# johnomotani/SharedMemSparseLU.jl

Hardware: AMD Instinct MI355X
Metric: nnz(L+U)/s + achieved HBM GB/s, 3D Poisson 128³ numeric LU, 1/2/4/8 GPU (higher is better)
Workload: dtype f64

## Files before the change

sharedmemsparselu.jl_amd/csrc/device.hpp:

```cpp
#pragma once
#include <cstdint>

namespace smlu {

struct SNode {
  int64_t first;
  int64_t Loff, Uoff, Foff;
  int64_t rowptr;
  int64_t voff;
  int32_t ns, nu;
  int32_t parent, nb;
  int32_t mode;
  int32_t chbeg, chend;
  int32_t level;
  int32_t cpair;
};

struct GemmTask {
  const double* A;
  const double* B;
  double* C;
  int32_t m, n, k;
  int32_t lda, ldb, ldc;
  int32_t tiles_m;
  int32_t gsid = -1;
  int64_t tile0;
};

constexpr int kUrowsCols = 32;
struct URowTask {
  int32_t s;
  int32_t ob0, ob1;
  int32_t slot0;
  int32_t ld;
  int32_t ncols;
  int64_t coff;
};

struct FrontTile {
  int32_t s;
  int32_t pad;
  int64_t wg0;
};

struct XContrib {
  int32_t child, pad;
  int64_t src;
};

struct alignas(8) AEnt {
  int32_t x, y;
};

struct SegDesc {
  uint64_t src, dst;
  int64_t n4;
};

struct XCol {
  int32_t p, tj;
  int64_t off;
  int32_t cnt, acnt;
  int64_t aoff;
};

struct SwapTask {
  int32_t s, kb0, nsub, slot0;
  int32_t a, b, c_lo, c_hi;
  int64_t wg0;
};

struct Rhs {
  int32_t n;
  int64_t ldx, ldv;
};
constexpr int kMultiRhs = 16;
#ifndef SMLU_SWEEP_WK
#define SMLU_SWEEP_WK 4
#endif
constexpr int kSweepWK = SMLU_SWEEP_WK;
constexpr int kSweepXB = 64;
struct ChunkDesc {
  int64_t c0, s, r0, nr, tri, rect;
};

}
```

sharedmemsparselu.jl_amd/csrc/factor.cpp:

```cpp
#include "handle.hpp"

static hipError_t run_launch(smlu_handle* h, const Launch& L, double diag_tol, double piv_tol, hipStream_t st) {
  switch (L.kind) {
    case K_EXTADD:
      return launch_assemble(st, L.cnt, h->xcols.p + L.off, h->xtasks.p, h->aents.p, h->sn.p, h->relmap.p,
                             h->A.p, h->Arow.p, h->Rs.p, h->store.p, h->scratch.p);
    case K_FRONT_LDS:
      return launch_front_small(st, (int)L.cnt, (int)L.aux, h->ilist.p + L.off, h->sn.p, h->chlist.p,
                                h->relmap.p, h->aents.p, h->A.p, h->Arow.p, h->Rs.p, h->store.p, h->scratch.p,
                                h->rowperm.p, h->info.p, h->growth.p, diag_tol, piv_tol);
    case K_STEPTRSM:
      return launch_step_trsm(st, (int)L.aux, h->ftiles.p + L.off, (int)L.cnt, L.nwg, h->ftiles.p + L.off2,
                              (int)L.cnt2, L.nwg2, L.step, h->sch.ob, h->sn.p, h->store.p, h->scratch.p, h->info.p,
                              h->growth.p, piv_tol);
    case K_LASWP:
      return launch_laswp(st, L.nwg, h->stasks.p + L.off, (int)L.cnt, h->sn.p, h->store.p, h->scratch.p,
                          h->swaps.p, kSwapStride);
    case K_PANEL:
      return launch_panel1(st, (int)L.cnt, (int)L.aux, (int)L.nwg, (int)L.aux2, L.step,
                           h->ilist.p + L.off, h->sn.p,
                          h->store.p, h->scratch.p, h->rowperm.p, h->swaps.p, kSwapStride, h->info.p,
                          h->growth.p, diag_tol, (int)L.cnt2, h->tinv.p, (int)h->sch.ob);
    case K_TRSMU:
      return launch_trsm_u(st, L.nwg, h->ftiles.p + L.off, (int)L.cnt, h->sch.ob, (int)L.aux, h->sn.p,
                           h->store.p, h->scratch.p, h->swaps.p, kSwapStride);
    case K_GEMM:
    case K_GEMMU:
    case K_GEMMO:
    case K_GEMM22:
      return launch_gemm(st, L.nwg, h->gtasks.p + L.off, (int)L.cnt, (int)L.aux, 0);
    case K_TRSML:
      return launch_gemm_g(st, L.nwg, h->gtasks.p + L.off, (int)L.cnt, (int)L.aux, 0, h->info.p,
                           h->growth.p, piv_tol);
    case K_UROWS:
      return launch_urows(st, (int)L.cnt, h->urtasks.p + L.off, h->sn.p, h->store.p, h->tinv.p);
    case K_TRIINV:
      return launch_tri_inv(st, (int)L.cnt, L.step, h->ilist.p + L.off, h->sn.p, h->store.p, h->scratch.p,
                            h->tinv.p);
  }
  return hipErrorInvalidValue;
}

static int enqueue_factor(smlu_handle* h, Timer& tm, bool dbg, int seg) {
  Plan& P = h->plan;
  hipStream_t st = h->stream;
  const size_t lo = h->sch.fac_seg[seg];
  const size_t hi = (size_t)seg + 1 < h->sch.fac_seg.size() ? h->sch.fac_seg[seg + 1] : h->sch.fac.size();
  double diag_tol = P.given_order ? 0.0 : h->opts.diag_pivot_tol;
  double piv_tol = h->opts.pivot_tol;
  if (seg > 0) goto launches;
  HIPCHK(launch_factor_reset(st, h->sch.nnodes, h->info.p, h->growth.p, P.n, h->rowperm.p, h->rowperm0.p));
  if (!h->given_Rs) {
    if (h->opts.scale) HIPCHK(launch_rowscale(st, P.n, h->Arowptr.p, h->Arow_ent.p, h->A.p, h->Rs.p));
    else HIPCHK(launch_fill(st, P.n, h->Rs.p, 1.0));
  }
launches:
  auto group = [&](size_t i) { return h->sch.fac[i].kind == K_FRONT_LDS ? h->sch.fac[i].aux2 : 0; };
  int gi = 0;
  hipEvent_t gstop = nullptr;
  for (size_t li = lo; li < hi; ++li) {
    const Launch& L = h->sch.fac[li];
    const int64_t g = group(li);
    const bool cont = g > 0 && li > lo && group(li - 1) == g;
    const bool more = g > 0 && li + 1 < hi && group(li + 1) == g;
    gi = cont ? gi + 1 : 0;
    const bool grouped = cont || more;
    if (gi == 0 && more) {
      HIPCHK(tm.begin(L.kind, &gstop, st));
      HIPCHK(hipEventRecord(h->fork_ev, st));
    }
    if (gi == 1) HIPCHK(hipStreamWaitEvent(h->side, h->fork_ev, 0));
    hipStream_t ls = (gi & 1) ? h->side : st;
    hipEvent_t stop = nullptr;
    if (!grouped) HIPCHK(tm.begin(L.kind, &stop, ls));
    hipError_t e = run_launch(h, L, diag_tol, piv_tol, ls);
    if (e == hipSuccess && dbg) e = hipStreamSynchronize(ls);
    if (e != hipSuccess) {
      if (gi >= 1) {
        (void)hipEventRecord(h->join_ev, h->side);
        (void)hipStreamWaitEvent(st, h->join_ev, 0);
      }
      char buf[256];
      std::snprintf(buf, sizeof buf, "HIP error '%s' in launch kind=%d step=%d off=%lld cnt=%lld nwg=%lld aux=%lld aux2=%lld",
                    hipGetErrorString(e), L.kind, L.step, (long long)L.off, (long long)L.cnt,
                    (long long)L.nwg, (long long)L.aux, (long long)L.aux2);
      return fail(h, SMLU_ERR_HIP, buf);
    }
    if (!grouped) HIPCHK(tm.end(stop));
    if (gi >= 1 && !more) {
      HIPCHK(hipEventRecord(h->join_ev, h->side));
      HIPCHK(hipStreamWaitEvent(st, h->join_ev, 0));
      tm.st = st;
      HIPCHK(tm.end(gstop));
      gstop = nullptr;
    }
  }
  return SMLU_OK;
}

static int factor_segment(smlu_handle* h, Timer& tm, int seg) {
  hipStream_t st = h->stream;
  const Tune tn = tune();
  const bool dbg = tn.debug_sync, nograph = tn.no_graph;
  const int prof = h->opts.profile ? 1 : 0;
  const size_t nseg = h->sch.fac_seg.size();
  if (h->fac_execs.size() != nseg || (seg == 0 && h->fac_exec_profile != prof)) {
    for (auto& g : h->fac_execs)
      if (g) (void)hipGraphExecDestroy(g);
    h->fac_execs.assign(nseg, nullptr);
    h->seg_events.assign(nseg, {0, 0});
  }
  bool use_graph = !dbg && !nograph && !h->graph_failed && h->have_numeric;
  if (use_graph && !h->fac_execs[seg]) {
    hipGraph_t g = nullptr;
    const size_t ev0 = tm.used;
    HIPCHK(hipStreamBeginCapture(st, hipStreamCaptureModeRelaxed));
    int rc = enqueue_factor(h, tm, false, seg);
    hipError_t ec = hipStreamEndCapture(st, &g);
    if (rc == SMLU_OK && ec == hipSuccess && g) ec = hipGraphInstantiate(&h->fac_execs[seg], g, nullptr, nullptr, 0);
    if (g) (void)hipGraphDestroy(g);
    if (rc != SMLU_OK || ec != hipSuccess || !h->fac_execs[seg]) {
      (void)hipGetLastError();
      h->graph_failed = true;
      h->fac_execs[seg] = nullptr;
      use_graph = false;
      tm.used = ev0;
    } else {
      h->fac_exec_profile = prof;
      h->seg_events[seg] = {ev0, tm.used - ev0};
    }
  }
  if (use_graph) {
    tm.used = h->seg_events[seg].first + h->seg_events[seg].second;
    HIPCHK(hipGraphLaunch(h->fac_execs[seg], st));
    return SMLU_OK;
  }
  return enqueue_factor(h, tm, dbg, seg);
}

int read_status(smlu_handle* h, const int32_t* info, int64_t nnodes, const int32_t* words, int nwords,
                long long out[16]) {
  hipStream_t st = h->stream;
  const long long seq = ++h->rb_seq;
  HIPCHK(launch_status(st, info, nnodes, info ? h->sn.p : nullptr, words, nwords, h->rb.p, seq));
  HIPCHK(hipStreamSynchronize(st));
  for (int attempt = 0; attempt < 4; ++attempt) {
    HIPCHK(hipMemcpy(out, h->rb.p, 16 * sizeof(long long), hipMemcpyDeviceToHost));
    if (out[0] == seq && out[15] == seq) return SMLU_OK;
    ++h->status_copy_retries;
  }
  return fail(h, SMLU_ERR_HIP, "status record read back with a wrong sequence stamp (device-to-host copy)");
}

static int finish_factor(smlu_handle* h, Timer& tm, std::chrono::steady_clock::time_point t0) {
  Plan& P = h->plan;
  long long rec[16];
  int rs = read_status(h, h->info.p, h->sch.nnodes, reinterpret_cast<const int32_t*>(h->growth.p), 4, rec);
  if (rs != SMLU_OK) return rs;
  h->dom_words = rec[7];
  if (rec[10] > 0) {
    h->bad_info_node = rec[8];
    h->bad_info_word = (int32_t)rec[9];
    h->bad_info_count += rec[10];
    return fail(h, SMLU_ERR_STATE, "factorization status: " + std::to_string(rec[10]) +
                " front info words outside the legal code set (first: node " + std::to_string(rec[8]) +
                ", word " + std::to_string(rec[9]) + ")");
  }
  tm.collect();
  h->refactor_ms = std::chrono::duration<double, std::milli>(std::chrono::steady_clock::now() - t0).count();
  double g;
  std::memcpy(&g, &rec[6], sizeof g);
  h->growth_max = g;
  h->have_numeric = true;
  ++h->nfactor;
  h->weak = rec[1];
  h->errcol = -1;
  h->flag_node = rec[4];
  h->flag_info = (int32_t)rec[5];
  int rc = SMLU_OK;
  if (rec[2] >= 0) {
    const int32_t v = (int32_t)rec[3];
    rc = SMLU_SINGULAR;
    h->errcol = P.s_first[h->sch.node_front[rec[2]]] + ((v >> 2) > 0 ? (v >> 2) - 1 : 0);
  }
  if (h->nranks > 1) {
    double red[3] = {rc == SMLU_SINGULAR ? 1.0 : 0.0, (double)h->errcol, (double)h->weak};
    if (h->tr.allreduce_max(h->tr.ctx, red, 3) != 0) return fail(h, SMLU_ERR_HIP, "transport allreduce failed");
    rc = red[0] > 0 ? SMLU_SINGULAR : SMLU_OK;
    h->errcol = (int64_t)red[1];
    h->weak = (int64_t)red[2];
  }
  if (rc == SMLU_SINGULAR) h->err = "matrix is singular (zero pivot column)";
  return rc;
}

static int run_factor_once(smlu_handle* h) {
  HIPCHK(hipSetDevice(h->device));
  auto t0 = std::chrono::steady_clock::now();
  for (auto& v : h->kind_ms) v = 0;
  h->comm_sent_fac = h->comm_recv_fac = 0;
  Timer tm(h);
  for (size_t seg = 0; seg < h->sch.fac_seg.size(); ++seg) {
    if (seg > 0) {
      int rc = exec_comm(h, h->sch.fac_comm[seg - 1]);
      if (rc != SMLU_OK) return rc;
    }
    int rc = factor_segment(h, tm, (int)seg);
    if (rc != SMLU_OK) return rc;
  }
  return finish_factor(h, tm, t0);
}

static int apply_dominance(smlu_handle* h, bool dom, bool* rebuilt);
static int launch_device_dominance(smlu_handle* h);

int run_factor(smlu_handle* h, bool redecide) {
  if (redecide) {
    int rc = launch_device_dominance(h);
    if (rc != SMLU_OK) return rc;
  }
  int rc = run_factor_once(h);
  if (rc < 0) return rc;
  if (redecide) {
    const bool dom = (h->dom_words & 0xffffffffll) != 0 || (h->dom_words >> 32) != 0;
    bool rebuilt = false;
    int r2 = apply_dominance(h, dom, &rebuilt);
    if (r2 != SMLU_OK) return r2;
    if (rebuilt) {
      ++h->mode_refactors;
      return run_factor(h, false);
    }
  }
  const bool off = tune().no_repivot;
  if ((rc == SMLU_SINGULAR || h->weak > 0) && h->pivmode == 0 && !off && has_tile_fronts(h) &&
      h->opts.pivot_tol > 0 && !h->plan.given_order && h->nranks == 1) {
    h->repivot_node = h->flag_node;
    h->repivot_info = h->flag_info;
    h->repivot_sn = h->flag_node >= 0 && h->flag_node < (int64_t)h->sch.hsn.size() ? h->sch.hsn[h->flag_node] : SNode{};
    h->repivot_growth = h->growth_max;
    h->pivmode = 1;
    int r2 = rebuild_schedule(h);
    if (r2 != SMLU_OK) return r2;
    ++h->repivots;
    rc = run_factor_once(h);
  }
  return rc;
}


static int apply_dominance(smlu_handle* h, bool dom, bool* rebuilt) {
  *rebuilt = false;
  if (h->nranks > 1) {
    double nd = dom ? 0.0 : 1.0;
    if (h->tr.allreduce_max(h->tr.ctx, &nd, 1) != 0) return fail(h, SMLU_ERR_HIP, "transport allreduce failed (dominance)");
    dom = nd == 0.0;
  }
  bool changed = false;
  if (dom != h->dominant) {
    h->dominant = dom;
    changed = h->pivmode == 0;
  }
  if (dom && h->pivmode == 1) {
    h->pivmode = 0;
    changed = true;
  }
  *rebuilt = changed;
  return changed ? rebuild_schedule(h) : SMLU_OK;
}

static int launch_device_dominance(smlu_handle* h) {
  const Plan& P = h->plan;
  hipStream_t st = h->stream;
  if (!h->Acolp.p) HIPCHK(h->Acolp.upload(P.Acolptr.data(), P.Acolptr.size(), st));
  int rc = ensure_residual(h);
  if (rc != SMLU_OK) return rc;
  HIPCHK(launch_dominance(st, P.n, h->Acolp.p, h->Arow.p, h->Arowptr.p, h->Arow_ent.p, h->Acol.p, h->A.p,
                          reinterpret_cast<int32_t*>(h->growth.p + 1)));
  return SMLU_OK;
}

int refactor_resident(smlu_handle* h) {
  return run_factor(h, !h->plan.given_order && !h->plan.matched);
}

int smlu_refactor(smlu_handle* h, const double* nzval) {
  if (!h || !nzval) return fail(h, SMLU_ERR_ARG, "NULL argument");
  HIPCHK(hipSetDevice(h->device));
  HIPCHK(hipMemcpyAsync(h->A.p, nzval, sizeof(double) * h->plan.nnzA, hipMemcpyHostToDevice, h->stream));
  return refactor_resident(h);
}

hipError_t after_caller(smlu_handle* h) {
  if (!h->ev_caller) {
    hipError_t e = hipEventCreateWithFlags(&h->ev_caller, hipEventDisableTiming);
    if (e != hipSuccess) return e;
  }
  hipError_t e = hipEventRecord(h->ev_caller, h->caller);
  return e != hipSuccess ? e : hipStreamWaitEvent(h->stream, h->ev_caller, 0);
}

int smlu_dev_front_hash(smlu_handle* h, unsigned long long* out) {
  if (!h || !out) return fail(h, SMLU_ERR_ARG, "NULL argument");
  if (h->nranks > 1) return fail(h, SMLU_ERR_STATE, "one-GPU handles only");
  const int64_t ns = h->plan.nsup;
  DBuf<unsigned long long> d;
  HIPCHK(d.alloc((size_t)std::max<int64_t>(2 * ns, 1)));
  HIPCHK(launch_front_hash(h->stream, ns, h->sn.p, h->store.p, h->rowperm.p, d.p));
  HIPCHK(hipStreamSynchronize(h->stream));
  hipError_t e = hipMemcpy(out, d.p, sizeof(unsigned long long) * 2 * ns, hipMemcpyDeviceToHost);
  d.free();
  HIPCHK(e);
  return SMLU_OK;
}

int smlu_dev_front_values(smlu_handle* h, int64_t s, double* out) {
  if (!h || !out || s < 0 || s >= h->plan.nsup) return fail(h, SMLU_ERR_ARG, "invalid arguments");
  if (h->nranks > 1) return fail(h, SMLU_ERR_STATE, "one-GPU handles only");
  const SNode& r = h->sch.hsn[s];
  const int64_t M = (int64_t)r.ns + r.nu;
  HIPCHK(hipStreamSynchronize(h->stream));
  HIPCHK(hipMemcpy(out, h->store.p + r.Loff, sizeof(double) * M * r.ns, hipMemcpyDeviceToHost));
  if (r.nu > 0)
    HIPCHK(hipMemcpy(out + M * r.ns, h->store.p + r.Uoff, sizeof(double) * r.ns * r.nu, hipMemcpyDeviceToHost));
  return SMLU_OK;
}

int smlu_dev_copy(smlu_handle* h, int which, int64_t off, int64_t cnt, double* out, int64_t* len) {
  if (!h || which < 0 || which > 1) return fail(h, SMLU_ERR_ARG, "invalid arguments");
  const DBuf<double>& b = which == 0 ? h->store : h->scratch;
  if (cnt < 0) {
    if (len) *len = (int64_t)b.n;
    return SMLU_OK;
// ... 83 lines not shown
```

sharedmemsparselu.jl_amd/csrc/handle.hpp:

```cpp
#pragma once
#include <dlfcn.h>
#include <hip/hip_runtime.h>
#include <rccl/rccl.h>

#include <algorithm>
#include <chrono>
#include <cmath>
#include <cstdio>
#include <cstdlib>
#include <cstring>
#include <limits>
#include <map>
#include <memory>
#include <unordered_map>
#include <string>
#include <vector>

#include "../../include/smlu.h"
#include "device.hpp"
#include "plan.hpp"
#include "schedule.hpp"

namespace smlu {
hipError_t launch_rowscale(hipStream_t, int64_t, const int64_t*, const int32_t*, const double*, double*);
hipError_t launch_fill(hipStream_t, int64_t, double*, double);
hipError_t launch_factor_reset(hipStream_t, int64_t, int32_t*, double*, int64_t, int32_t*, const int32_t*);
hipError_t launch_assemble(hipStream_t, int64_t, const XCol*, const XContrib*, const int2*, const SNode*,
                           const int32_t*, const double*, const int32_t*, const double*, double*, double*);
hipError_t launch_front_small(hipStream_t, int, int, const int32_t*, const SNode*, const int32_t*, const int32_t*,
                              const int2*, const double*, const int32_t*, const double*, double*, double*,
                            int32_t*, int32_t*, double*, double, double);
hipError_t init_kernel_attributes();
hipError_t launch_panel1(hipStream_t, int, int, int, int, int, const int32_t*, const SNode*, double*, double*,
                         int32_t*, int32_t*, int64_t, int32_t*, double*, double, int, double*, int);
hipError_t launch_step_trsm(hipStream_t, int, const FrontTile*, int, int64_t, const FrontTile*, int, int64_t,
                            int, int, const SNode*, double*, double*, int32_t*, double*, double);
hipError_t launch_laswp(hipStream_t, int64_t, const SwapTask*, int, const SNode*, double*, double*, const int32_t*,
                        int64_t);
hipError_t launch_trsm_u(hipStream_t, int64_t, const FrontTile*, int, int, int, const SNode*, double*,
                         double*, const int32_t*, int64_t);
hipError_t launch_gemm(hipStream_t, int64_t, const GemmTask*, int, int, int64_t);
hipError_t launch_gemm_g(hipStream_t, int64_t, const GemmTask*, int, int, int64_t, int32_t*, double*, double);
hipError_t launch_tri_inv(hipStream_t, int, int, const int32_t*, const SNode*, double*, double*, double*);
hipError_t launch_urows(hipStream_t, int, const URowTask*, const SNode*, double*, const double*);
hipError_t launch_fwd_tiny(hipStream_t, int, const int32_t*, const SNode*, const int32_t*, const int32_t*,
                           const int32_t*, const double*, double*, double*, Rhs, int);
hipError_t launch_bwd_tiny(hipStream_t, int, const int32_t*, const SNode*, const int32_t*, const double*, double*,
                           double*, Rhs, int);
hipError_t launch_fwd_pull(hipStream_t, int64_t, const FrontTile*, int, const SNode*, const int32_t*,
                           const int32_t*, const int32_t*, const double*, double*, Rhs);
hipError_t launch_fwd_gather(hipStream_t, int, const int32_t*, const SNode*, const int32_t*, const int32_t*,
                             const int32_t*, double*, double*, Rhs);
hipError_t launch_tri_block(hipStream_t, bool, int64_t, const FrontTile*, int, int, const SNode*,
                            const double*, double*, double*, Rhs);
hipError_t launch_bwd_u12(hipStream_t, int64_t, const FrontTile*, int, const SNode*, const int32_t*,
                          const double*, const double*, double*, Rhs);
hipError_t launch_tri_sweep(hipStream_t, bool, int64_t, const FrontTile*, int, unsigned long long*, int32_t*, double*,
                            int32_t*, const SNode*, const double*, double*, double*, Rhs, int);
hipError_t launch_fwd(hipStream_t, int, const int32_t*, const SNode*, const int32_t*, const int32_t*,
                      const int32_t*, const double*, double*, double*, Rhs);
hipError_t launch_bwd(hipStream_t, int, const int32_t*, const SNode*, const int32_t*, const double*,
                      double*, double*, Rhs);
hipError_t launch_residual(hipStream_t, int64_t, const int64_t*, const int32_t*, const int32_t*,
                           const double*, const double*, const double*, double*, double*);
hipError_t launch_axpy1(hipStream_t, int64_t, const double*, double*);
hipError_t launch_dominance(hipStream_t, int64_t, const int64_t*, const int32_t*, const int64_t*, const int32_t*,
                            const int32_t*, const double*, int32_t*);
hipError_t launch_status(hipStream_t, const int32_t*, int64_t, const SNode*, const int32_t*, int, long long*, long long);
hipError_t launch_front_hash(hipStream_t, int64_t, const SNode*, const double*, const int32_t*, unsigned long long*);
hipError_t launch_expand_z(hipStream_t, int64_t, const double*, const int64_t*, const int32_t*, double*);
hipError_t launch_perm_in(hipStream_t, int64_t, const int64_t*, const double*, const double*, double*, int,
                          int64_t, int64_t);
hipError_t launch_perm_out(hipStream_t, int64_t, const int64_t*, const double*, double*, int, int64_t, int64_t);
hipError_t launch_chunked_solve(hipStream_t, bool, int64_t, const ChunkDesc*, const double*, double*);
hipError_t launch_segcopy(hipStream_t, const SegDesc*, int64_t);
hipError_t launch_bwd_u12_cols(hipStream_t, const SNode*, int, int64_t, int64_t, int64_t, int, const int32_t*,
                               const double*, const double*, double*);
hipError_t launch_vcopy(hipStream_t, const SNode*, int, int64_t, const double*, double*);
hipError_t launch_unswap(hipStream_t, int64_t, const int64_t*, const int32_t*, const double*, double*);
hipError_t launch_ut_tiny(hipStream_t, int, const int32_t*, const SNode*, const int32_t*, const int32_t*, const double*,
                          double*, double*, int);
hipError_t launch_lt_tiny(hipStream_t, int, const int32_t*, const SNode*, const int32_t*, const int32_t*, const double*,
                          double*, int);
hipError_t launch_ut_front(hipStream_t, int, const int32_t*, const SNode*, const int32_t*, const int32_t*,
                           const double*, double*, double*);
hipError_t launch_lt_front(hipStream_t, int, const int32_t*, const SNode*, const int32_t*, const int32_t*,
                           const double*, double*, double*);
hipError_t launch_pull_t(hipStream_t, int64_t, const FrontTile*, int, const SNode*, const int32_t*, const int32_t*,
                         const double*, double*);
hipError_t launch_tri_t(hipStream_t, bool, int64_t, const FrontTile*, int, int, const SNode*, const int32_t*,
                        const double*, double*, double*);
hipError_t launch_bwdu_t(hipStream_t, int64_t, const FrontTile*, int, const SNode*, const int32_t*, const double*,
                         const double*, double*);
hipError_t launch_perm_in_t(hipStream_t, int64_t, const int64_t*, const double*, double*, int);
hipError_t launch_perm_out_t(hipStream_t, int64_t, const int64_t*, const double*, const double*, double*, int);
hipError_t launch_residual_t(hipStream_t, int64_t, const int64_t*, const int32_t*, const double*, const double*,
                             const double*, double*, double*, int);
}

using namespace smlu;

namespace smlu {

extern thread_local std::string g_last_error;

template <class T>
struct DBuf {
  T* p = nullptr;
  size_t n = 0;
  hipError_t alloc(size_t cnt) {
    n = cnt;
    if (cnt == 0) return hipSuccess;
    return hipMalloc((void**)&p, cnt * sizeof(T));
  }
  hipError_t upload(const T* h, size_t cnt, hipStream_t st) {
    hipError_t e = alloc(cnt);
    if (e != hipSuccess || cnt == 0) return e;
    return hipMemcpyAsync(p, h, cnt * sizeof(T), hipMemcpyHostToDevice, st);
  }
  void free() {
    if (p) (void)hipFree(p);
    p = nullptr;
    n = 0;
  }
};

struct RcclApi {
  void* lib = nullptr;
  ncclResult_t (*GetUniqueId)(ncclUniqueId*);
  ncclResult_t (*CommInitRank)(ncclComm_t*, int, ncclUniqueId, int);
  ncclResult_t (*CommDestroy)(ncclComm_t);
  ncclResult_t (*Send)(const void*, size_t, ncclDataType_t, int, ncclComm_t, hipStream_t);
  ncclResult_t (*Recv)(void*, size_t, ncclDataType_t, int, ncclComm_t, hipStream_t);
  ncclResult_t (*GroupStart)();
  ncclResult_t (*GroupEnd)();
  ncclResult_t (*AllReduce)(const void*, void*, size_t, ncclDataType_t, ncclRedOp_t, ncclComm_t, hipStream_t);
  ncclResult_t (*CommCount)(const ncclComm_t, int*);
};

RcclApi* rccl_api();

struct RcclState {
  ncclComm_t comm = nullptr;
  int rank = 0;
  int comm_count = 0;
  hipStream_t stream = nullptr;
  double* dbuf = nullptr;
};

int rccl_exchange(void* ctx, int32_t npeer, const int32_t* peer, void* const* sbuf, const int64_t* sbytes,
                  void* const* rbuf, const int64_t* rbytes, void* stream);
int rccl_bcast(void* ctx, void* buf, int64_t bytes, int32_t root, int32_t gsize, const int32_t* group, void* stream);
int rccl_allreduce_max(void* ctx, double* buf, int32_t count);

}

struct smlu_plan {
  Plan plan;
};

struct smlu_handle {
  smlu_opts opts{};
  Plan plan;
  int device = 0;
  hipStream_t stream = nullptr;
  hipStream_t side = nullptr;
  hipEvent_t fork_ev = nullptr, join_ev = nullptr;
  std::string err;
  int64_t errcol = -1;
  bool have_numeric = false;
  bool given_Rs = false;
  DBuf<double> A, Rs, store, scratch, wrk, wrk2, vbuf, growth;
  DBuf<double> vbufm, wrkm, wrk2m;
  DBuf<double> tinv;
  DBuf<double> ch_data;
  DBuf<ChunkDesc> ch_desc;
  DBuf<int64_t> ch_p, ch_q;
  int64_t ch_T = 0, ch_size = 0, ch_version = -1;
  int64_t nfactor = 0;
  DBuf<double> ref_b, ref_r, ref_d, ref_nrm;
  DBuf<int32_t> Acol;
  DBuf<int64_t> Acolp;
  int refine_steps = 0;
  double refine_berr = -1;
  double refine_resid = -1;
  DBuf<int64_t> Arowptr, p0, q, posfirst;
  DBuf<int32_t> Arow_ent, Arow, rows, relmap, chlist, ilist, rowperm, rowperm0, info, swaps;
  DBuf<SNode> sn;
  DBuf<XContrib> xtasks;
  DBuf<int2> aents;
  DBuf<FrontTile> ftiles;
  DBuf<int32_t> gptr, gent;
  DBuf<int32_t> ssync, sstatus;
  DBuf<unsigned long long> stick;
  DBuf<double> sxh;
  DBuf<GemmTask> gtasks;
  DBuf<SwapTask> stasks;
  DBuf<URowTask> urtasks;
  DBuf<XCol> xcols;
  Schedule sch;
  double refactor_ms = 0, solve_ms = 0, growth_max = 0;
  int64_t weak = 0;
  double kind_ms[K_NKIND] = {0};
  std::vector<std::pair<hipEvent_t, hipEvent_t>> ev_pool;
  std::vector<int> ev_kind;
  hipStream_t caller = nullptr;
  hipEvent_t ev_caller = nullptr;
  DBuf<long long> rb;
  std::vector<int64_t> gLp, gLi, gUp, gUi;
  bool given_pattern = false;
  int64_t pattern_dropped = 0;
  long long rb_seq = 0;
  int64_t status_copy_retries = 0;
  int64_t bad_info_node = -1, bad_info_count = 0;
  int32_t bad_info_word = 0;
  int64_t sweep_timeouts = 0;
  int sweep_spin = 1 << 22;
  DBuf<double> bstash;
  std::vector<std::pair<int, hipGraphExec_t>> sol_execs;
  std::vector<hipGraphExec_t> fac_execs;
  int fac_exec_profile = -1;
  std::vector<std::pair<size_t, size_t>> seg_events;
  int rank = 0, nranks = 1;
  RankLayout lay;
  smlu_transport tr{};
  void* rccl = nullptr;
  DBuf<double> stage_s, stage_r, bcbuf, d_red;
  DBuf<SegDesc> segdesc;
  char* hstage_s = nullptr;
  char* hstage_r = nullptr;
  int64_t stage_bytes_s = 0, stage_bytes_r = 0;
  double comm_sent = 0, comm_recv = 0, comm_sent_fac = 0, comm_recv_fac = 0;
  int64_t comm_calls = 0;
  size_t fac_graph_events = 0;
  bool graph_failed = false;
  bool dominant = false;
  int pivmode = 0;
  int64_t repivots = 0;
  int64_t mode_refactors = 0;
  long long dom_words = 0;
  int64_t flag_node = -1;
  int32_t flag_info = 0;
  int64_t repivot_node = -1;
  int32_t repivot_info = 0;
  double repivot_growth = 0;
  SNode repivot_sn{};
  bool zc = false;
  bool cpair = false;
  int64_t zn = 0, znnz = 0;
  std::vector<int64_t> zdst;
  std::vector<int32_t> zoff;
  std::vector<int64_t> zcolptr, zrowval;
  DBuf<int64_t> d_zdst;
  DBuf<int32_t> d_zoff;
  ~smlu_handle() { release_all(); }
  void release_buffers() {
    if (stream) (void)hipSetDevice(device);
    release_graphs();
    DBuf<double>* d[] = {&A, &Rs, &store, &scratch, &wrk, &wrk2, &vbuf, &vbufm, &wrkm, &wrk2m, &growth, &ref_b, &ref_r, &ref_d, &ref_nrm,
                         &tinv, &ch_data, &bstash};
    ch_desc.free();
    ch_p.free();
    ch_q.free();
    ch_version = -1;
    Acol.free();
    Acolp.free();
    for (auto* b : d) b->free();
    DBuf<int64_t>* l[] = {&Arowptr, &p0, &q, &posfirst};
    for (auto* b : l) b->free();
    DBuf<int32_t>* i[] = {&Arow_ent, &Arow, &rows, &relmap, &chlist, &ilist, &rowperm, &rowperm0, &info, &swaps};
    for (auto* b : i) b->free();
    sn.free();
    d_zdst.free();
    d_zoff.free();
    xtasks.free();
    aents.free();
    ftiles.free();
    gptr.free();
    gent.free();
    ssync.free();
    sstatus.free();
    stick.free();
    sxh.free();
    gtasks.free();
    stasks.free();
    urtasks.free();
    xcols.free();
    stage_s.free();
    stage_r.free();
    bcbuf.free();
    segdesc.free();
    d_red.free();
    if (hstage_s) (void)hipHostFree(hstage_s);
    if (hstage_r) (void)hipHostFree(hstage_r);
    hstage_s = hstage_r = nullptr;
  }
  void release_graphs() {
    for (auto& g : fac_execs)
      if (g) (void)hipGraphExecDestroy(g);
    fac_execs.clear();
    for (auto& g : sol_execs)
      if (g.second) (void)hipGraphExecDestroy(g.second);
    sol_execs.clear();
    fac_exec_profile = -1;
  }
  void release_all() {
    release_graphs();
    release_buffers();
    if (rccl) {
      if (RcclApi* R = rccl_api()) (void)R->CommDestroy(static_cast<RcclState*>(rccl)->comm);
      delete static_cast<RcclState*>(rccl);
      rccl = nullptr;
    }
    for (auto& e : ev_pool) {
      (void)hipEventDestroy(e.first);
      (void)hipEventDestroy(e.second);
    }
    ev_pool.clear();
    ev_kind.clear();
    rb.free();
    if (ev_caller) (void)hipEventDestroy(ev_caller);
    if (fork_ev) (void)hipEventDestroy(fork_ev);
    if (join_ev) (void)hipEventDestroy(join_ev);
    fork_ev = join_ev = nullptr;
    if (side) (void)hipStreamDestroy(side);
    side = nullptr;
    if (stream) (void)hipStreamDestroy(stream);
    stream = nullptr;
  }
};

#define HIPCHK2(hh, expr)                                                            \
  do {                                                                               \
    hipError_t _e = (expr);                                                          \
    if (_e != hipSuccess) {                                                          \
      (hh)->err = std::string("HIP error: ") + hipGetErrorString(_e) + " at " #expr; \
      g_last_error = (hh)->err;                                                      \
      return SMLU_ERR_HIP;                                                           \
    }                                                                                \
  } while (0)

#define HIPCHK(expr)                                                                 \
  do {                                                                               \
    hipError_t _e = (expr);                                                          \
    if (_e != hipSuccess) {                                                          \
      h->err = std::string("HIP error: ") + hipGetErrorString(_e) + " at " #expr;    \
      g_last_error = h->err;                                                         \
      return SMLU_ERR_HIP;                                                           \
    }                                                                                \
  } while (0)

inline int fail(smlu_handle* h, int code, const std::string& msg) {
  if (h) h->err = msg;
  g_last_error = msg;
  return code;
}

inline PlanOptions plan_opts(const smlu_opts& o) {
  PlanOptions p;
  p.ordering = o.ordering;
  for (int i = 0; i < 3; ++i) p.grid[i] = o.grid[i];
  p.relax = o.relax;
  p.leaf_size = o.leaf_size > 0 ? o.leaf_size : 64;
  return p;
}

inline bool valid_opts(const smlu_opts* o) { return o && (o->index_base == 0 || o->index_base == 1); }

template <class RI>
bool diagonally_dominant(int64_t n, const int64_t* colptr, const RI* rowval, const double* a,
                                int64_t base) {
  std::vector<double> rdiag(n, 0.0), roff(n, 0.0);
  bool col_dom = true;
  for (int64_t j = 0; j < n; ++j) {
    double d = 0.0, off = 0.0;
    for (int64_t e = colptr[j] - base; e < colptr[j + 1] - base; ++e) {
      const int64_t i = rowval[e] - base;
      const double v = std::fabs(a[e]);
      if (i == j) { d += v; rdiag[i] += v; }
      else { off += v; roff[i] += v; }
    }
    if (!(d > 0.0 && d >= off)) col_dom = false;
  }
  if (col_dom) return true;
  for (int64_t i = 0; i < n; ++i)
    if (!(rdiag[i] > 0.0 && rdiag[i] >= roff[i])) return false;
  return true;
}

struct Timer {
  smlu_handle* h;
  size_t used = 0;
  explicit Timer(smlu_handle* hh) : h(hh) {}
  hipStream_t st = nullptr;
  hipError_t begin(int kind, hipEvent_t* stop, hipStream_t s) {
    st = s;
    if (!h->opts.profile) { *stop = nullptr; return hipSuccess; }
    if (used == h->ev_pool.size()) {
      hipEvent_t a, b;
      hipError_t e = hipEventCreate(&a);
      if (e != hipSuccess) return e;
      e = hipEventCreate(&b);
      if (e != hipSuccess) return e;
      h->ev_pool.push_back({a, b});
      h->ev_kind.push_back(kind);
    }
    h->ev_kind[used] = kind;
    *stop = h->ev_pool[used].second;
    hipError_t e = hipEventRecord(h->ev_pool[used].first, st);
    ++used;
    return e;
  }
  hipError_t end(hipEvent_t stop) { return stop ? hipEventRecord(stop, st) : hipSuccess; }
  void collect() {
    for (size_t i = 0; i < used; ++i) {
      float ms = 0;
      if (hipEventElapsedTime(&ms, h->ev_pool[i].first, h->ev_pool[i].second) == hipSuccess)
        h->kind_ms[h->ev_kind[i]] += ms;
      else
        (void)hipGetLastError();
    }
  }
};

int create_impl(int64_t n, const int64_t* colptr, const int64_t* rowval, const double* nzval, const int64_t* p,
                const int64_t* q, const double* Rs, const smlu_opts* opts, smlu_handle** out, int rank = 0,
                int nranks = 1, const smlu_transport* tr = nullptr, RcclState* rccl = nullptr,
                const std::vector<int64_t>* preorder = nullptr);
std::vector<int64_t> diagonal_match(int64_t n, const int64_t* colptr, const int64_t* rowval, const double* a,
                                    int64_t base);
int setup_device(smlu_handle* h);
void schedule_bytes(const Plan& P, const RankLayout& lay, const Schedule& S, int rank, int nranks, double out[5]);
int rebuild_schedule(smlu_handle* h);
bool has_tile_fronts(const smlu_handle* h);
int run_factor(smlu_handle* h, bool redecide = false);
int read_status(smlu_handle* h, const int32_t* info, int64_t nnodes, const int32_t* words, int nwords,
                long long out[16]);
hipError_t after_caller(smlu_handle* h);
int refactor_resident(smlu_handle* h);
int refactor_csc_impl(smlu_handle* h, int64_t n, const int64_t* colptr, const int64_t* rowval,
                      const double* nzval, const std::vector<int64_t>* preorder);
int exec_comm(smlu_handle* h, int id);
int ensure_residual(smlu_handle* h);


struct Exported {
  std::vector<int64_t> Lp, Li, Up, Ui, p, q;
  std::vector<double> Lx, Ux;
};

int export_factors(smlu_handle* h, Exported& X, bool values);
```

sharedmemsparselu.jl_amd/csrc/kernels_front.hip:

```cpp
#include "kernels_common.hpp"

namespace smlu {

__global__ void k_rowscale(int64_t n, const int64_t* __restrict__ rowptr,
                           const int32_t* __restrict__ ent, const double* __restrict__ a,
                           double* __restrict__ Rs) {
  int64_t i = (int64_t)blockIdx.x * blockDim.x + threadIdx.x;
  if (i >= n) return;
  double s = 0.0;
  const int64_t e1 = rowptr[i + 1];
  for (int64_t e0 = rowptr[i]; e0 < e1; e0 += 8) {
    int32_t id[8];
#pragma unroll
    for (int k = 0; k < 8; ++k) id[k] = e0 + k < e1 ? ent[e0 + k] : -1;
    double v[8];
#pragma unroll
    for (int k = 0; k < 8; ++k) v[k] = id[k] >= 0 ? a[id[k]] : 0.0;
#pragma unroll
    for (int k = 0; k < 8; ++k)
      if (id[k] >= 0) s += fabs(v[k]);
  }
  Rs[i] = s > 0.0 ? 1.0 / s : 1.0;
}

__global__ void k_fill(int64_t n, double* __restrict__ x, double v) {
  int64_t i = (int64_t)blockIdx.x * blockDim.x + threadIdx.x;
  if (i < n) x[i] = v;
}

__global__ void k_factor_reset(int64_t nnodes, int32_t* __restrict__ info, double* __restrict__ growth, int64_t n,
                               int32_t* __restrict__ rowperm, const int32_t* __restrict__ rowperm0) {
  const int64_t i = (int64_t)blockIdx.x * blockDim.x + threadIdx.x;
  if (i < nnodes) info[i] = 0;
  if (i < n) rowperm[i] = rowperm0[i];
  if (i == 0) growth[0] = 0.0;
}

__global__ __launch_bounds__(256) void k_assemble(int64_t ntasks, const XCol* __restrict__ cols,
                                                  const XContrib* __restrict__ contrib,
                                                  const int2* __restrict__ aents,
                                                  const SNode* __restrict__ sn,
                                                  const int32_t* __restrict__ relmap,
                                                  const double* __restrict__ a,
                                                  const int32_t* __restrict__ arow,
                                                  const double* __restrict__ Rs,
                                                  double* __restrict__ store, double* __restrict__ scratch) {
  __shared__ double sbuf[4][256];
  const int64_t w = ((int64_t)blockIdx.x * blockDim.x + threadIdx.x) >> 6;
  const int lane = threadIdx.x & 63;
  if (w >= ntasks) return;
  double* b = sbuf[threadIdx.x >> 6];
  const XCol t = cols[w];
  const SNode p = sn[t.p];
  FrontPtrs P = front_ptrs(p, store, scratch);
  const int64_t len = P.M;
  const int64_t tj = t.tj;
  gdbl* colL = tj < P.ns ? P.L + tj * P.M : nullptr;
  gdbl* colU = tj < P.ns ? nullptr : P.U + (tj - P.ns) * P.ns;
  gdbl* colF = (tj < P.ns || P.nu == 0) ? nullptr : P.F + (tj - P.ns) * P.nu - P.ns;
  int cur = 0;
  int64_t q_src = 0, q_rm = 0;
  int q_nu = 0;
  if (lane < t.cnt) {
    const XContrib ck = contrib[t.off + lane];
    const SNode c = sn[ck.child];
    q_src = ck.src;
    q_rm = c.rowptr;
    q_nu = c.nu;
  }
  int64_t ap = 0;
  for (int64_t r0 = 0; r0 < len; r0 += 256) {
    const int64_t r1 = min<int64_t>(len, r0 + 256);
#pragma unroll
    for (int u = 0; u < 4; ++u) b[lane + 64 * u] = 0.0;
    wave_lds_sync();
    while (ap < t.acnt) {
      const int64_t i = ap + lane;
      int2 en = make_int2(0, 0x7fffffff);
      if (i < t.acnt) en = aents[t.aoff + i];
      const bool take = en.y < r1;
      const unsigned long long m = __ballot(take);
      if (take) b[en.y - r0] = Rs[arow[en.x]] * a[en.x];
      const int c = __popcll(m);
      ap += c;
      if (c < 64) break;
    }
    wave_lds_sync();
    for (int q = 0; q < t.cnt; ++q) {
      int64_t srco, rmo, nuc, pos;
      if (q < 64) {
        srco = ((int64_t)__builtin_amdgcn_readlane((int)(q_src >> 32), q) << 32) |
               (uint32_t)__builtin_amdgcn_readlane((int)(q_src & 0xffffffff), q);
        rmo = ((int64_t)__builtin_amdgcn_readlane((int)(q_rm >> 32), q) << 32) |
              (uint32_t)__builtin_amdgcn_readlane((int)(q_rm & 0xffffffff), q);
        nuc = __builtin_amdgcn_readlane(q_nu, q);
        pos = __builtin_amdgcn_readlane(cur, q);
      } else {
        const XContrib ck = contrib[t.off + q];
        const SNode c = sn[ck.child];
        srco = ck.src;
        rmo = c.rowptr;
        nuc = c.nu;
        const int32_t* rmq = relmap + rmo;
        int64_t lo = 0, hi = nuc;
        while (lo < hi) {
          const int64_t mid = (lo + hi) >> 1;
          if (rmq[mid] < r0) lo = mid + 1;
          else hi = mid;
        }
        pos = lo;
      }
      const double* src = srco >= 0 ? scratch + srco : store + (-1 - srco);
      const int32_t* rm = relmap + rmo;
      int32_t rv[4];
      double sv[4];
#pragma unroll
      for (int k = 0; k < 4; ++k) {
        const int64_t i = pos + lane + 64 * k;
        rv[k] = i < nuc ? rm[i] : 0x7fffffff;
        sv[k] = i < nuc ? src[i] : 0.0;
      }
      int cn = 0;
#pragma unroll
      for (int k = 0; k < 4; ++k) {
        const bool take = rv[k] < r1;
        if (take) b[rv[k] - r0] += sv[k];
        cn += __popcll(__ballot(take));
      }
      pos += cn;
      if (q < 64 && lane == q) cur = (int)pos;
      wave_lds_sync();
    }
#pragma unroll
    for (int u = 0; u < 4; ++u) {
      const int64_t r = r0 + lane + 64 * u;
      if (r < r1) {
        const double v = b[lane + 64 * u];
        if (colL) colL[r] = v;
        else if (r < P.ns) colU[r] = v;
        else colF[r] = v;
      }
    }
    wave_lds_sync();
  }
}

__device__ __forceinline__ int choose_pivot(double akk, double amax, int arg, int k,
                                            double diag_tol) {
  if (amax == 0.0) return k;
  if (fabs(akk) >= diag_tol * amax && akk != 0.0) return k;
  return arg;
}

typedef double f64x4 __attribute__((ext_vector_type(4)));
template <int NW>
__global__ __launch_bounds__(64 * NW) void k_front_small(const int32_t* __restrict__ list,
                                                         const SNode* __restrict__ sn,
                                                         const int32_t* __restrict__ chlist,
                                                         const int32_t* __restrict__ relmap,
                                                         const int2* __restrict__ aents,
                                                         const double* __restrict__ a,
                                                         const int32_t* __restrict__ arow,
                                                         const double* __restrict__ Rs,
                                                         double* __restrict__ store,
                                                         double* __restrict__ scratch,
                                                         int32_t* __restrict__ rowperm,
                                                         int32_t* __restrict__ info,
                                                         double* __restrict__ growth, double diag_tol,
                                                         double piv_tol) {
  constexpr int NT = 64 * NW;
  extern __shared__ __attribute__((aligned(16))) double lds[];
  __shared__ int s_perm[128];
  __shared__ int s_piv;
  const int sid = list[3 * blockIdx.x];
  const int64_t a0 = list[3 * blockIdx.x + 1];
  const int acnt = list[3 * blockIdx.x + 2];
  const SNode s = sn[sid];
  FrontPtrs f = front_ptrs(s, store, scratch);
  const int M = (int)f.M, ns = (int)f.ns;
  const int ld = M | 1;
  const int tid = threadIdx.x, lane = tid & 63, wv = tid >> 6;
  for (int e = tid; e < M * ld; e += NT) lds[e] = 0.0;
  for (int i = tid; i < ns; i += NT) s_perm[i] = i;
  __syncthreads();
  for (int e = tid; e < acnt; e += NT) {
    const int2 en = aents[a0 + e];
    lds[(en.y >> 16) * ld + (en.y & 0xffff)] = Rs[arow[en.x]] * a[en.x];
  }
  __syncthreads();
  for (int q = s.chbeg; q < s.chend; ++q) {
    const SNode c = sn[chlist[q]];
    const int nuc = c.nu;
    if (nuc == 0) continue;
    const int32_t* rm = relmap + c.rowptr;
    const gdbl* src = gbl(scratch + c.Foff);
    const bool h0 = lane < nuc, h1 = lane + 64 < nuc;
    const int ri0 = h0 ? rm[lane] : 0, ri1 = h1 ? rm[lane + 64] : 0;
    for (int jc0 = wv; jc0 < nuc; jc0 += 8 * NW) {
      int cj[8];
      double v0[8], v1[8];
#pragma unroll
      for (int u = 0; u < 8; ++u) {
        const int jc = jc0 + u * NW;
        const bool on = jc < nuc;
        cj[u] = on ? rm[jc] : 0;
        v0[u] = (on && h0) ? src[(int64_t)jc * nuc + lane] : 0.0;
        v1[u] = (on && h1) ? src[(int64_t)jc * nuc + lane + 64] : 0.0;
      }
#pragma unroll
      for (int u = 0; u < 8; ++u) {
        if (jc0 + u * NW >= nuc) break;
        double* col = lds + cj[u] * ld;
        if (h0) col[ri0] += v0[u];
        if (h1) col[ri1] += v1[u];
      }
    }
    __syncthreads();
  }
  int flag = 0, err = -1;
  double gmax = 0.0, glane = 0.0;
  __shared__ int s_second;
  for (int k = 0; k < ns; ++k) {
    if (s.cpair && wv == 0) {
      if ((k & 1) == 0) {
        double am = -1.0, amo = 0.0;
        int ai = k;
        for (int e = k + 2 * lane; e < M; e += 128) {
          const double x = lds[k * ld + e], y = lds[k * ld + e + 1];
          const double v = fma(x, x, y * y);
          if (e < ns) {
            if (v > am) { am = v; ai = e; }
          } else if (v > amo) {
            amo = v;
          }
        }
        am = wave_max_idx(am, ai);
        amo = wave_max(amo);
        if (lane == 0) {
          const double x = lds[k * ld + k], y = lds[k * ld + k + 1];
          const double d2 = fma(x, x, y * y);
          int pc = k;
          if (am <= 0.0) {
            flag |= 1;
            if (err < 0) err = k;
          } else if (!(d2 >= diag_tol * diag_tol * am && d2 != 0.0)) {
            pc = ai;
          }
          const int r1 = fabs(lds[k * ld + pc + 1]) > fabs(lds[k * ld + pc]) ? pc + 1 : pc;
          const int r2 = 2 * pc + 1 - r1;
          if (am > 0.0) {
            const double a = lds[k * ld + pc], b = lds[k * ld + pc + 1];
            const double pm = fma(a, a, b * b);
            if (pm < piv_tol * piv_tol * fmax(am, amo)) flag |= 2;
            gmax = fmax(gmax, sqrt(fmax(am, amo) / pm));
          }
          s_piv = r1;
          s_second = r2 == k ? r1 : r2;
        }
      } else if (lane == 0) {
        s_piv = s_second;
        if (lds[k * ld + s_second] == 0.0) {
          flag |= 1;
          if (err < 0) err = k;
        }
      }
    } else if (wv == 0) {
      double am = -1.0, amo = 0.0;
      int ai = k;
      bool beats = false, weak = false;
      const double akk = lds[k * ld + k], pk = fabs(akk);
      for (int i = k + lane; i < M; i += 64) {
        double v = fabs(lds[k * ld + i]);
        if (i < ns) {
          if (v > am) { am = v; ai = i; }
          beats |= diag_tol * v > pk;
        } else if (v > amo) {
          amo = v;
        }
        weak |= piv_tol * v > pk;
      }
      if (akk != 0.0 && __ballot(beats) == 0ull) {
        const double ml = fmax(am, amo);
        if (ml > 0.0) glane = fmax(glane, ml / pk);
        const bool anyweak = __ballot(weak) != 0ull;
        if (lane == 0) {
          if (anyweak) flag |= 2;
          s_piv = k;
        }
        goto searched;
      }
      am = wave_max_idx(am, ai);
      amo = wave_max(amo);
      if (lane == 0) {
        int piv = choose_pivot(lds[k * ld + k], am, ai, k, diag_tol);
        double pv = fabs(lds[k * ld + piv]);
        if (am <= 0.0) {
          flag |= 1;
          if (err < 0) err = k;
        } else {
          if (pv < piv_tol * fmax(am, amo)) flag |= 2;
          gmax = fmax(gmax, fmax(am, amo) / pv);
        }
        s_piv = piv;
      }
    }
  searched:
    __syncthreads();
    const int piv = s_piv;
    if (piv != k) {
      for (int j = tid; j < M; j += NT) {
        double t = lds[j * ld + k];
        lds[j * ld + k] = lds[j * ld + piv];
        lds[j * ld + piv] = t;
      }
      if (tid == 0) {
        int t = s_perm[k];
        s_perm[k] = s_perm[piv];
        s_perm[piv] = t;
      }
      __syncthreads();
    }
    const double pinv = recip(lds[k * ld + k]);
    for (int i = k + 1 + tid; i < M; i += NT) lds[k * ld + i] = lds[k * ld + i] * pinv;
    __syncthreads();
    const int nb = (M - ns + 63) / 64, nl = ns - k - 1;
    for (int q = wv; q < nb + nl; q += NW) {
      if (q < nb) {
        const int j = ns + 64 * q + lane;
        if (j < M) {
          double* cj = lds + j * ld;
          const double u = cj[k];
          if (u != 0.0) {
            int i = k + 1;
            for (; i + 4 <= ns; i += 4) {
              const double a0 = cj[i], a1 = cj[i + 1], a2 = cj[i + 2], a3 = cj[i + 3];
              const double l0 = lds[k * ld + i], l1 = lds[k * ld + i + 1], l2 = lds[k * ld + i + 2],
                           l3 = lds[k * ld + i + 3];
              cj[i] = fma(-l0, u, a0);
              cj[i + 1] = fma(-l1, u, a1);
              cj[i + 2] = fma(-l2, u, a2);
              cj[i + 3] = fma(-l3, u, a3);
            }
            for (; i < ns; ++i) cj[i] = fma(-lds[k * ld + i], u, cj[i]);
          }
        }
      } else {
        const int j = k + 1 + (q - nb);
        const double u = lds[j * ld + k];
        if (u != 0.0)
          for (int i = k + 1 + lane; i < M; i += 64)
            lds[j * ld + i] = fma(-lds[k * ld + i], u, lds[j * ld + i]);
      }
    }
    __syncthreads();
  }
  if (M > ns) {
    const int nu = M - ns, nt = (nu + 15) / 16;
    const int li = lane & 15, lg = lane >> 4;
    for (int t = wv; t < nt * nt; t += NW) {
// ... 1269 lines not shown
```

sharedmemsparselu.jl_amd/csrc/kernels_gemm.hip:

```cpp
#include "kernels_common.hpp"

namespace smlu {

__device__ __forceinline__ int find_gemm_task(const GemmTask* __restrict__ t, int cnt, int64_t b) {
  int lo = 0, hi = cnt - 1;
  while (lo < hi) {
    int mid = (lo + hi + 1) >> 1;
    if (t[mid].tile0 <= b) lo = mid;
    else hi = mid - 1;
  }
  return lo;
}


__device__ __forceinline__ int64_t xcd_remap(int64_t b, int64_t nwg) {
  const int64_t q = nwg >> 3, r = nwg & 7, x = b & 7;
  return (x < r ? x * (q + 1) : r * (q + 1) + (x - r) * q) + (b >> 3);
}
__device__ __forceinline__ int64_t xcd_window_remap(int64_t b, int64_t nwg) {
  constexpr int64_t W = 512;
  if (b >= (nwg / W) * W) return b;
  const int64_t w0 = b - b % W, i = b % W;
  return w0 + (i & 7) * (W / 8) + (i >> 3);
}
template <int TS>
__device__ __forceinline__ void tile_rc(const GemmTask& t, int64_t tl, int& tm, int& tn) {
  constexpr int GM = 8;
  const int64_t tiles_n = (t.n + TS - 1) / TS;
  const int64_t g = tl / (GM * tiles_n);
  const int first = (int)(g * GM);
  const int gm = min(GM, t.tiles_m - first);
  const int64_t in = tl - g * GM * tiles_n;
  tm = first + (int)(in % gm);
  tn = (int)(in / gm);
}

struct GrowthArgs {
  int32_t* info;
  double* growth;
  double piv_tol;
};
__device__ __forceinline__ void tile_growth(const GrowthArgs& ga, int sid, double g) {
  g = wave_max(g);
  if ((threadIdx.x & 63) == 0 && g > 0.0) {
    atomic_max_pos(&ga.growth[0], g);
    if (g > 1.0 / ga.piv_tol) atomicOr(&ga.info[sid], 2);
  }
}

#define GBM 64
#define GBN 64
#define GBK 16
template <bool TRSM>
__global__ __launch_bounds__(256) void k_gemm(const GemmTask* __restrict__ tasks, int ntask, GrowthArgs ga) {
  __shared__ double As[2][GBK][GBM + 2];
  __shared__ double Bs[2][GBK][GBN + 2];
  const int64_t b = xcd_remap(blockIdx.x, gridDim.x);
  const GemmTask t = tasks[find_gemm_task(tasks, ntask, b)];
  const gdbl* gA = gbl(t.A);
  const gdbl* gB = gbl(t.B);
  gdbl* gC = gbl(t.C);
  int tm, tn;
  tile_rc<GBM>(t, b - t.tile0, tm, tn);
  const int m0 = tm * GBM, n0 = tn * GBN;
  const int tid = threadIdx.x;
  const int tx = tid & 15, ty = tid >> 4;
  double acc[4][4];
#pragma unroll
  for (int j = 0; j < 4; ++j) {
    const int col = n0 + ty + 16 * j;
#pragma unroll
    for (int i = 0; i < 4; ++i) {
      const int row = m0 + tx + 16 * i;
      acc[i][j] = (col < t.n && row < t.m) ? gC[(int64_t)col * t.ldc + row] : 0.0;
    }
  }
  const int ar = tid & 63, ak = tid >> 6;
  const int bk = tid & 15, bc = tid >> 4;
  double ra[4], rb[4];
  const int K = t.k;
  auto gload = [&](int k0) {
#pragma unroll
    for (int r = 0; r < 4; ++r) {
      int kk = ak + 4 * r;
      int row = m0 + ar;
      ra[r] = (row < t.m && k0 + kk < K) ? gA[(int64_t)(k0 + kk) * t.lda + row] : 0.0;
      int col = n0 + bc + 16 * r;
      rb[r] = (col < t.n && k0 + bk < K) ? gB[(int64_t)col * t.ldb + k0 + bk] : 0.0;
    }
  };
  auto sstore = [&](int buf) {
#pragma unroll
    for (int r = 0; r < 4; ++r) {
      As[buf][ak + 4 * r][ar] = ra[r];
      Bs[buf][bk][bc + 16 * r] = -rb[r];
    }
  };
  int nk = (K + GBK - 1) / GBK;
  gload(0);
  sstore(0);
  __syncthreads();
  for (int kt = 0; kt < nk; ++kt) {
    const int cur = kt & 1;
    if (kt + 1 < nk) gload((kt + 1) * GBK);
#pragma unroll 4
    for (int kk = 0; kk < GBK; ++kk) {
      double a[4], bb[4];
#pragma unroll
      for (int i = 0; i < 4; ++i) a[i] = As[cur][kk][tx + 16 * i];
#pragma unroll
      for (int j = 0; j < 4; ++j) bb[j] = Bs[cur][kk][ty + 16 * j];
#pragma unroll
      for (int i = 0; i < 4; ++i)
#pragma unroll
        for (int j = 0; j < 4; ++j) acc[i][j] = fma(a[i], bb[j], acc[i][j]);
    }
    if (kt + 1 < nk) sstore(cur ^ 1);
    __syncthreads();
  }
  double gmax = 0.0;
#pragma unroll
  for (int j = 0; j < 4; ++j) {
    const int col = n0 + ty + 16 * j;
#pragma unroll
    for (int i = 0; i < 4; ++i) {
      const int row = m0 + tx + 16 * i;
      if (col < t.n && row < t.m) {
        gC[(int64_t)col * t.ldc + row] = acc[i][j];
        gmax = fmax(gmax, fabs(acc[i][j]));
      }
    }
  }
  if (TRSM && t.gsid >= 0) tile_growth(ga, t.gsid, gmax);
}

typedef double v4d __attribute__((ext_vector_type(4)));
template <bool TRSM>
__global__ __launch_bounds__(256) void k_gemm64_mfma(const GemmTask* __restrict__ tasks, int ntask, GrowthArgs ga) {
  __shared__ double As[2][GBK][GBM + 2];
  __shared__ double Bs[2][GBK][GBN + 2];
  const int64_t b = xcd_remap(blockIdx.x, gridDim.x);
  const GemmTask t = tasks[find_gemm_task(tasks, ntask, b)];
  const gdbl* gA = gbl(t.A);
  const gdbl* gB = gbl(t.B);
  gdbl* gC = gbl(t.C);
  int tm, tn;
  tile_rc<GBM>(t, b - t.tile0, tm, tn);
  const int m0 = tm * GBM, n0 = tn * GBN;
  const int tid = threadIdx.x, lane = tid & 63;
  const int wv = __builtin_amdgcn_readfirstlane(tid >> 6);
  const int wr = (wv & 1) * 32, wc = (wv >> 1) * 32;
  const int li = lane & 15, lk = lane >> 4;
  v4d acc[2][2];
#pragma unroll
  for (int i = 0; i < 2; ++i) {
    const int row = m0 + wr + 16 * i + li;
#pragma unroll
    for (int j = 0; j < 2; ++j)
#pragma unroll
      for (int r = 0; r < 4; ++r) {
        const int col = n0 + wc + 16 * j + lk + 4 * r;
        acc[i][j][r] = (col < t.n && row < t.m) ? gC[(int64_t)col * t.ldc + row] : 0.0;
      }
  }
  const int ar = tid & 63, ak = tid >> 6;
  const int bk = tid & 15, bc = tid >> 4;
  double ra[4], rb[4];
  const int K = t.k;
  auto gload = [&](int k0) {
#pragma unroll
    for (int r = 0; r < 4; ++r) {
      const int kk = ak + 4 * r;
      const int row = m0 + ar;
      ra[r] = (row < t.m && k0 + kk < K) ? gA[(int64_t)(k0 + kk) * t.lda + row] : 0.0;
      const int col = n0 + bc + 16 * r;
      rb[r] = (col < t.n && k0 + bk < K) ? gB[(int64_t)col * t.ldb + k0 + bk] : 0.0;
    }
  };
  auto sstore = [&](int buf) {
#pragma unroll
    for (int r = 0; r < 4; ++r) {
      As[buf][ak + 4 * r][ar] = ra[r];
      Bs[buf][bk][bc + 16 * r] = -rb[r];
    }
  };
  const int nk = (K + GBK - 1) / GBK;
  gload(0);
  sstore(0);
  __syncthreads();
  for (int kt = 0; kt < nk; ++kt) {
    const int cur = kt & 1;
    if (kt + 1 < nk) gload((kt + 1) * GBK);
#pragma unroll
    for (int kq = 0; kq < GBK / 4; ++kq) {
      const int k = 4 * kq + lk;
      double fa[2], fb[2];
#pragma unroll
      for (int i = 0; i < 2; ++i) fa[i] = As[cur][k][wr + 16 * i + li];
#pragma unroll
      for (int j = 0; j < 2; ++j) fb[j] = Bs[cur][k][wc + 16 * j + li];
#pragma unroll
      for (int i = 0; i < 2; ++i)
#pragma unroll
        for (int j = 0; j < 2; ++j) acc[i][j] = __builtin_amdgcn_mfma_f64_16x16x4f64(fb[j], fa[i], acc[i][j], 0, 0, 0);
    }
    if (kt + 1 < nk) sstore(cur ^ 1);
    __syncthreads();
  }
  double gmax = 0.0;
#pragma unroll
  for (int i = 0; i < 2; ++i) {
    const int row = m0 + wr + 16 * i + li;
#pragma unroll
    for (int j = 0; j < 2; ++j)
#pragma unroll
      for (int r = 0; r < 4; ++r) {
        const int col = n0 + wc + 16 * j + lk + 4 * r;
        if (col < t.n && row < t.m) {
          gC[(int64_t)col * t.ldc + row] = acc[i][j][r];
          gmax = fmax(gmax, fabs(acc[i][j][r]));
        }
      }
  }
  if (TRSM && t.gsid >= 0) tile_growth(ga, t.gsid, gmax);
}

__device__ __forceinline__ double k64_tile_mfma(const gdbl* gA, int lda, const gdbl* gB, int ldb, gdbl* gC, int ldc,
                                                int m, int n, int K, int m0, int n0,
                                                double (&As)[64][GBM + 2], double (&Bs)[64][GBN + 2]) {
  const int tid = threadIdx.x, lane = tid & 63;
  const int wv = __builtin_amdgcn_readfirstlane(tid >> 6);
  const int wr = (wv & 1) * 32, wc = (wv >> 1) * 32;
  const int li = lane & 15, lk = lane >> 4;
  v4d acc[2][2];
#pragma unroll
  for (int i = 0; i < 2; ++i) {
    const int row = m0 + wr + 16 * i + li;
#pragma unroll
    for (int j = 0; j < 2; ++j)
#pragma unroll
      for (int r = 0; r < 4; ++r) {
        const int col = n0 + wc + 16 * j + lk + 4 * r;
        acc[i][j][r] = (col < n && row < m) ? gC[(int64_t)col * ldc + row] : 0.0;
      }
  }
  const int ar = tid & 63, ak = tid >> 6;
  double ra[16], rb[16];
#pragma unroll
  for (int r = 0; r < 16; ++r) {
    const int kk = ak + 4 * r, row = m0 + ar;
    ra[r] = (row < m && kk < K) ? gA[(int64_t)kk * lda + row] : 0.0;
    const int col = n0 + ak + 4 * r;
    rb[r] = (col < n && ar < K) ? gB[(int64_t)col * ldb + ar] : 0.0;
  }
#pragma unroll
  for (int r = 0; r < 16; ++r) {
    As[ak + 4 * r][ar] = ra[r];
    Bs[ar][ak + 4 * r] = -rb[r];
  }
  __syncthreads();
  auto kquad = [&](int kq) {
    const int k = 4 * kq + lk;
    double fa[2], fb[2];
#pragma unroll
    for (int i = 0; i < 2; ++i) fa[i] = As[k][wr + 16 * i + li];
#pragma unroll
    for (int j = 0; j < 2; ++j) fb[j] = Bs[k][wc + 16 * j + li];
#pragma unroll
    for (int i = 0; i < 2; ++i)
#pragma unroll
      for (int j = 0; j < 2; ++j) acc[i][j] = __builtin_amdgcn_mfma_f64_16x16x4f64(fb[j], fa[i], acc[i][j], 0, 0, 0);
  };
  if (K == 64) {
#pragma unroll
    for (int kq = 0; kq < 16; ++kq) kquad(kq);
  } else {
    const int nkq = (K + 3) >> 2;
    for (int kq = 0; kq < nkq; ++kq) kquad(kq);
  }
  double gmax = 0.0;
#pragma unroll
  for (int i = 0; i < 2; ++i) {
    const int row = m0 + wr + 16 * i + li;
#pragma unroll
    for (int j = 0; j < 2; ++j)
#pragma unroll
      for (int r = 0; r < 4; ++r) {
        const int col = n0 + wc + 16 * j + lk + 4 * r;
        if (col < n && row < m) {
          gC[(int64_t)col * ldc + row] = acc[i][j][r];
          gmax = fmax(gmax, fabs(acc[i][j][r]));
        }
      }
  }
  return gmax;
}

template <bool TRSM>
__global__ __launch_bounds__(256) void k_gemm_k64(const GemmTask* __restrict__ tasks, int ntask, GrowthArgs ga) {
  __shared__ double As[64][GBM + 2];
  __shared__ double Bs[64][GBN + 2];
  const int64_t b = xcd_remap(blockIdx.x, gridDim.x);
  const GemmTask t = tasks[find_gemm_task(tasks, ntask, b)];
  int tm, tn;
  tile_rc<GBM>(t, b - t.tile0, tm, tn);
  const double gmax = k64_tile_mfma(gbl(t.A), t.lda, gbl(t.B), t.ldb, gbl(t.C), t.ldc, t.m, t.n, t.k, tm * GBM,
                                    tn * GBN, As, Bs);
  if (TRSM && t.gsid >= 0) tile_growth(ga, t.gsid, gmax);
}

#define HBM_ 128
#define HBK_ 16
#define HLDB_ (HBM_ + 2)
template <bool TRSM, bool FULL>
__device__ __forceinline__ void gemm128_mfma_body(const GemmTask& t, int m0, int n0,
                                                double (&As)[2][HBK_][HBM_], double (&Bs)[2][HBK_][HLDB_],
                                                const GrowthArgs& ga) {
  const gdbl* gA = gbl(t.A);
  const gdbl* gB = gbl(t.B);
  gdbl* gC = gbl(t.C);
  const int tid = threadIdx.x, lane = tid & 63, wv = tid >> 6;
  const int wr = (wv & 1) * 64, wc = (wv >> 1) * 64;
  const int li = lane & 15, lk = lane >> 4;
  v4d acc[4][4];
#pragma unroll
  for (int i = 0; i < 4; ++i) {
    const int row = m0 + wr + 16 * i + li;
#pragma unroll
    for (int j = 0; j < 4; ++j)
#pragma unroll
      for (int r = 0; r < 4; ++r) {
        const int col = n0 + wc + 16 * j + lk + 4 * r;
        acc[i][j][r] = (FULL || (row < t.m && col < t.n)) ? gC[(int64_t)col * t.ldc + row] : 0.0;
      }
  }
  const int ar = tid & 127, ak = tid >> 7;
  const int bk = tid & 15, bc = tid >> 4;
  const int K = t.k;
  const int arow = m0 + ar;
  const bool arow_ok = FULL || arow < t.m;
  const gdbl* Ap = gA + arow;
  const gdbl* Bp = gB + (int64_t)(n0 + bc) * t.ldb + bk;
  double ra[8], rb[8];
  auto gload = [&](int k0, bool kguard) {
#pragma unroll
    for (int r = 0; r < 8; ++r) {
      const int kk = k0 + ak + 2 * r;
      if (!kguard && FULL) ra[r] = Ap[(int64_t)kk * t.lda];
      else ra[r] = (arow_ok && kk < K) ? Ap[(int64_t)kk * t.lda] : 0.0;
      const int col = n0 + bc + 16 * r;
      if (!kguard && FULL) rb[r] = Bp[(int64_t)16 * r * t.ldb + k0];
      else rb[r] = ((FULL || col < t.n) && k0 + bk < K) ? Bp[(int64_t)16 * r * t.ldb + k0] : 0.0;
    }
  };
  auto sstore = [&](int buf) {
#pragma unroll
    for (int r = 0; r < 8; ++r) {
      As[buf][ak + 2 * r][ar] = ra[r];
      Bs[buf][bk][bc + 16 * r] = -rb[r];
    }
  };
  const int nk = (K + HBK_ - 1) / HBK_;
  const int nfull = K / HBK_;
  gload(0, nfull == 0);
  sstore(0);
  __syncthreads();
  for (int kt = 0; kt < nk; ++kt) {
    const int cur = kt & 1;
    if (kt + 1 < nk) gload((kt + 1) * HBK_, kt + 1 >= nfull);
#pragma unroll
    for (int kq = 0; kq < HBK_ / 4; ++kq) {
      const int k = kq * 4 + lk;
      double fa[4], fb[4];
#pragma unroll
      for (int i = 0; i < 4; ++i) fa[i] = As[cur][k][wr + 16 * i + li];
#pragma unroll
      for (int j = 0; j < 4; ++j) fb[j] = Bs[cur][k][wc + 16 * j + li];
#pragma unroll
      for (int i = 0; i < 4; ++i)
#pragma unroll
        for (int j = 0; j < 4; ++j)
          acc[i][j] = __builtin_amdgcn_mfma_f64_16x16x4f64(fb[j], fa[i], acc[i][j], 0, 0, 0);
    }
    if (kt + 1 < nk) sstore(cur ^ 1);
    __syncthreads();
  }
  double gmax = 0.0;
#pragma unroll
  for (int i = 0; i < 4; ++i) {
    const int row = m0 + wr + 16 * i + li;
#pragma unroll
    for (int j = 0; j < 4; ++j)
#pragma unroll
      for (int r = 0; r < 4; ++r) {
        const int col = n0 + wc + 16 * j + lk + 4 * r;
        if (FULL || (row < t.m && col < t.n)) {
          gC[(int64_t)col * t.ldc + row] = acc[i][j][r];
          if (TRSM) gmax = fmax(gmax, fabs(acc[i][j][r]));
        }
      }
  }
  if (TRSM && t.gsid >= 0) tile_growth(ga, t.gsid, gmax);
}


typedef double v2du __attribute__((ext_vector_type(2), aligned(8)));
typedef double v2d __attribute__((ext_vector_type(2)));
__device__ __forceinline__ v2d ldu2(const char* ubase, uint32_t off) {
  return *(const __attribute__((address_space(1))) v2du*)(ubase + off);
}
__device__ __forceinline__ void stu2(char* ubase, uint32_t off, v2d v) {
  *(__attribute__((address_space(1))) v2du*)(ubase + off) = v;
}

struct Mfma3Lds {
  double A[2][HBK_][HBM_];
  double B[2][HBM_][HBK_];
};
static_assert(sizeof(Mfma3Lds) == 65536, "v3 tile LDS image");
typedef __attribute__((address_space(3))) void lds_void;

__device__ __forceinline__ void glds16(const void* src, void* lds_dst) {
  __builtin_amdgcn_global_load_lds((const __attribute__((address_space(1))) void*)src, (lds_void*)lds_dst, 16, 0, 0);
}


template <bool TRSM, bool EB>
__device__ __forceinline__ void gemm128_mfma3_interior(const GemmTask& t, int m0, int n0, Mfma3Lds& S,
                                                       const GrowthArgs& ga) {
  const int tid = threadIdx.x, lane = tid & 63;
  const int wv = __builtin_amdgcn_readfirstlane(tid >> 6);
  const int wr = (wv & 1) * 64, wc = (wv >> 1) * 64;
  const int li = lane & 15, lk = lane >> 4;
  const int K = t.k;
  const int64_t lda = t.lda, ldb = t.ldb, ldc = t.ldc;
  const uint32_t c_lo = (uint32_t)(((int64_t)lk * ldc + 2 * li) * 8);
  auto cbase = [&](int ip, int j, int r) {
    return reinterpret_cast<char*>(t.C) + ((int64_t)(n0 + wc + 16 * j + 4 * r) * ldc + m0 + wr + 32 * ip) * 8;
  };
  const int bpair = (lane & 7) ^ ((4 * wv + (lane >> 4)) & 7);
  const char* asrc = reinterpret_cast<const char*>(t.A) + ((int64_t)wv * lda + m0 + 2 * lane) * 8;
  const char* bsrc = reinterpret_cast<const char*>(t.B) + ((int64_t)(n0 + 8 * wv + (lane >> 3)) * ldb + 2 * bpair) * 8;
  auto issue = [&](int k0, int buf) {
#pragma unroll
    for (int q = 0; q < 4; ++q) {
      glds16(asrc + ((int64_t)(k0 + 4 * q) * lda) * 8, &S.A[buf][wv + 4 * q][0]);
      glds16(bsrc + ((int64_t)32 * q * ldb + k0) * 8, &S.B[buf][8 * (wv + 4 * q)][0]);
    }
  };
  auto stage_tail = [&](int k0, int buf) {
#pragma unroll
    for (int q = 0; q < 4; ++q) {
      const int ka = k0 + wv + 4 * q;
      const v2d a = ka < K ? ldu2(asrc + ((int64_t)(k0 + 4 * q) * lda) * 8, 0) : v2d{0.0, 0.0};
      *reinterpret_cast<v2d*>(&S.A[buf][wv + 4 * q][2 * lane]) = a;
      const gdbl* bp = gbl(reinterpret_cast<const double*>(bsrc + ((int64_t)32 * q * ldb + k0) * 8));
      const int kb = k0 + 2 * bpair;
      v2d b;
      b.x = kb < K ? bp[0] : 0.0;
      b.y = kb + 1 < K ? bp[1] : 0.0;
      *reinterpret_cast<v2d*>(&S.B[buf][8 * (wv + 4 * q)][2 * lane]) = b;
    }
  };
  v4d acc[4][4];
#pragma unroll
  for (int ip = 0; ip < 2; ++ip)
#pragma unroll
    for (int j = 0; j < 4; ++j)
#pragma unroll
      for (int r = 0; r < 4; ++r) {
        const v2d c = ldu2(cbase(ip, j, r), c_lo);
        acc[2 * ip][j][r] = c.x;
        acc[2 * ip + 1][j][r] = c.y;
      }
  const int a_off = (lk * HBM_ + wr + 2 * li);
  int b_off[4];
#pragma unroll
  for (int kq = 0; kq < 4; ++kq) b_off[kq] = (wc + li) * HBK_ + (((2 * kq + (lk >> 1)) ^ (li >> 1)) << 1) + (lk & 1);
  auto frags = [&](int cur, int kq, v2d (&fa)[2], double (&fb)[4]) {
    const double* As = &S.A[cur][0][0] + a_off + kq * 4 * HBM_;
    const double* Bs = &S.B[cur][0][0] + b_off[kq];
#pragma unroll
    for (int ip = 0; ip < 2; ++ip) fa[ip] = *reinterpret_cast<const v2d*>(As + 32 * ip);
#pragma unroll
    for (int j = 0; j < 4; ++j) fb[j] = Bs[16 * HBK_ * j];
  };
  auto quad = [&](const v2d (&fa)[2], const double (&fb)[4]) {
#pragma unroll
    for (int ip = 0; ip < 2; ++ip)
#pragma unroll
      for (int j = 0; j < 4; ++j) {
        acc[2 * ip][j] = __builtin_amdgcn_mfma_f64_16x16x4f64(fb[j], fa[ip].x, acc[2 * ip][j], 0, 0, 1);
        acc[2 * ip + 1][j] = __builtin_amdgcn_mfma_f64_16x16x4f64(fb[j], fa[ip].y, acc[2 * ip + 1][j], 0, 0, 1);
      }
  };
  auto slice = [&](int cur) {
    v2d fa0[2], fa1[2];
    double fb0[4], fb1[4];
    frags(cur, 0, fa0, fb0);
    frags(cur, 1, fa1, fb1);
    quad(fa0, fb0);
    frags(cur, 2, fa0, fb0);
    quad(fa1, fb1);
    frags(cur, 3, fa1, fb1);
    quad(fa0, fb0);
    quad(fa1, fb1);
  };
  const int nk = (K + HBK_ - 1) / HBK_;
  const int nfull = K / HBK_;
  if (nfull > 0) issue(0, 0);
  else stage_tail(0, 0);
  __syncthreads();
  if (!EB) {
    for (int kt = 0; kt < nk; ++kt) {
      const int cur = kt & 1;
      const bool next = kt + 1 < nk;
      const bool next_full = kt + 1 < nfull;
      if (next_full) issue((kt + 1) * HBK_, cur ^ 1);
      if (next && !next_full) stage_tail((kt + 1) * HBK_, cur ^ 1);
      slice(cur);
      if (next) __syncthreads();
    }
  } else {
    v2d fa0[2], fa1[2];
    double fb0[4], fb1[4];
    frags(0, 0, fa0, fb0);
    for (int kt = 0; kt < nk; ++kt) {
      const int cur = kt & 1;
      const bool next = kt + 1 < nk;
      const bool next_full = kt + 1 < nfull;
      if (next_full) issue((kt + 1) * HBK_, cur ^ 1);
      if (next && !next_full) stage_tail((kt + 1) * HBK_, cur ^ 1);
      frags(cur, 1, fa1, fb1);
      quad(fa0, fb0);
      frags(cur, 2, fa0, fb0);
      quad(fa1, fb1);
      frags(cur, 3, fa1, fb1);
      quad(fa0, fb0);
      if (next) {
        __syncthreads();
        frags(cur ^ 1, 0, fa0, fb0);
      }
      quad(fa1, fb1);
    }
  }
  double gmax = 0.0;
#pragma unroll
  for (int ip = 0; ip < 2; ++ip)
#pragma unroll
    for (int j = 0; j < 4; ++j)
#pragma unroll
      for (int r = 0; r < 4; ++r) {
        const v2d c = v2d{acc[2 * ip][j][r], acc[2 * ip + 1][j][r]};
        stu2(cbase(ip, j, r), c_lo, c);
        if (TRSM) gmax = fmax(gmax, fmax(fabs(c.x), fabs(c.y)));
      }
  if (TRSM && t.gsid >= 0) tile_growth(ga, t.gsid, gmax);
}

#ifdef SMLU_CLOCK_PROBE
__device__ unsigned long long* g_clock_probe = nullptr;
struct ClockMark {
  unsigned long long t0, r0;
  __device__ __forceinline__ ClockMark() : t0(__builtin_amdgcn_s_memtime()), r0(__builtin_amdgcn_s_memrealtime()) {}
  __device__ __forceinline__ void done(int form) const {
    const unsigned long long t1 = __builtin_amdgcn_s_memtime(), r1 = __builtin_amdgcn_s_memrealtime();
    unsigned long long* p = g_clock_probe;
    if (p && threadIdx.x == 0) {
      atomicAdd(p + 4 * form, t1 - t0);
      atomicAdd(p + 4 * form + 1, r1 - r0);
      atomicAdd(p + 4 * form + 2, 1ull);
    }
  }
};
#endif
template <bool TRSM, bool EB = false>
__global__ __launch_bounds__(256, 2) void k_gemm128_mfma3(const GemmTask* __restrict__ tasks, int ntask,
                                                          GrowthArgs ga) {
#ifdef SMLU_CLOCK_PROBE
  const ClockMark mark;
#endif
  __shared__ __attribute__((aligned(16))) double lds[sizeof(Mfma3Lds) / sizeof(double)];
  const int64_t b = xcd_window_remap(blockIdx.x, gridDim.x);
  const GemmTask t = tasks[find_gemm_task(tasks, ntask, b)];
  int tm, tn;
  tile_rc<HBM_>(t, b - t.tile0, tm, tn);
  const int m0 = tm * HBM_, n0 = tn * HBM_;
  if (m0 + HBM_ <= t.m && n0 + HBM_ <= t.n) {
    gemm128_mfma3_interior<TRSM, EB>(t, m0, n0, *reinterpret_cast<Mfma3Lds*>(lds), ga);
  } else {
    auto& As = *reinterpret_cast<double(*)[2][HBK_][HBM_]>(lds);
    auto& Bs = *reinterpret_cast<double(*)[2][HBK_][HLDB_]>(lds + 2 * HBK_ * HBM_);
    gemm128_mfma_body<TRSM, false>(t, m0, n0, As, Bs, ga);
  }
#ifdef SMLU_CLOCK_PROBE
  mark.done(EB ? 0 : 1);
#endif
}

#define UR_NC 32
#define UR_RB 6
#define UR_LD 36
__device__ __forceinline__ double sel0(bool c, double x) {
  return __longlong_as_double(__double_as_longlong(x) & (c ? -1LL : 0LL));
}
__global__ __launch_bounds__(256, 2) void k_urows(const URowTask* __restrict__ tasks, const SNode* __restrict__ sn,
                                                  double* __restrict__ store, const double* __restrict__ tinv) {
  __shared__ double Bs[64 * UR_LD];
  const URowTask t = tasks[blockIdx.x];
  const SNode s = sn[t.s];
  const int64_t M = (int64_t)s.ns + s.nu;
  const int64_t ld = t.ld;
  const int nc = t.ncols;
  const int nrows = t.ob1 - t.ob0;
  const int tid = threadIdx.x, lane = tid & 63, li = lane & 15, lk = lane >> 4;
  const int wv = __builtin_amdgcn_readfirstlane(tid >> 6);
  gdbl* const C = gbl(store + t.coff);
  const gdbl* const Lp = gbl(store + s.Loff);
  v4d acc[UR_RB][2];
#pragma unroll
  for (int i = 0; i < UR_RB; ++i) {
    const int lr = 16 * (wv + 4 * i) + li;
    const bool rin = lr < nrows;
    const int row = t.ob0 + (rin ? lr : 0);
#pragma unroll
    for (int cb = 0; cb < 2; ++cb)
#pragma unroll
      for (int r = 0; r < 4; ++r) {
        const int col = 16 * cb + lk + 4 * r;
        const bool in = rin && col < nc;
        acc[i][cb][r] = sel0(in, C[(int64_t)(in ? col : 0) * ld + row]);
      }
  }
  auto publish = [&](int i) {
#pragma unroll
    for (int cb = 0; cb < 2; ++cb)
#pragma unroll
      for (int r = 0; r < 4; ++r) Bs[(16 * wv + li) * UR_LD + 16 * cb + lk + 4 * r] = -acc[i][cb][r];
  };
  const int nsub = (nrows + 63) >> 6;
#pragma unroll 1
  for (int u = 0; u < nsub; ++u) {
    const int kbu = t.ob0 + 64 * u;
    const int wu = min(64, t.ob1 - kbu);
    const int nkq = (wu + 3) >> 2;
    v4d tc[2];
#pragma unroll
    for (int i = 0; i < UR_RB; ++i)
      if (i == u) {
        publish(i);
        tc[0] = acc[i][0];
        tc[1] = acc[i][1];
      }
    double na[16];
    {
      const gdbl* pn = gbl(tinv + (int64_t)(t.slot0 + u) * 8192) + lk * 64 + 16 * wv + li;
#pragma unroll
      for (int kq = 0; kq < 16; ++kq) na[kq] = sel0(16 * wv + li < wu && 4 * kq + lk < wu, pn[256 * kq]);
    }
    __syncthreads();
#pragma unroll
    for (int kq = 0; kq < 16; ++kq) {
      if (kq >= nkq) continue;
      const int k = 4 * kq + lk;
#pragma unroll
      for (int cb = 0; cb < 2; ++cb)
        tc[cb] = __builtin_amdgcn_mfma_f64_16x16x4f64(Bs[k * UR_LD + 16 * cb + li], na[kq], tc[cb], 0, 0, 0);
    }
    __syncthreads();
#pragma unroll
    for (int i = 0; i < UR_RB; ++i)
      if (i == u) {
        acc[i][0] = tc[0];
        acc[i][1] = tc[1];
        publish(i);
      }
    __syncthreads();
    double fa[16], fn[16];
    auto lfrag = [&](int i, double (&f)[16]) {
      const int lr = 16 * (wv + 4 * i) + li;
      const bool rin = lr < nrows;
      const gdbl* pa = Lp + (int64_t)(kbu + lk) * M + t.ob0 + (rin ? lr : 0);
#pragma unroll
      for (int kq = 0; kq < 16; ++kq) {
        const bool kin = 4 * kq + lk < wu;
        f[kq] = sel0(rin && kin, pa[kin ? (int64_t)4 * kq * M : 0]);
      }
    };
    if (u + 1 < UR_RB && 16 * (wv + 4 * (u + 1)) < nrows) lfrag(u + 1, fa);
#pragma unroll
    for (int i = 1; i < UR_RB; ++i) {
      if (i <= u || 16 * (wv + 4 * i) >= nrows) continue;
      const bool more = i + 1 < UR_RB && 16 * (wv + 4 * (i + 1)) < nrows;
      if (more) lfrag(i + 1, fn);
#pragma unroll
      for (int kq = 0; kq < 16; ++kq) {
        if (kq >= nkq) continue;
        const int k = 4 * kq + lk;
#pragma unroll
        for (int cb = 0; cb < 2; ++cb)
          acc[i][cb] = __builtin_amdgcn_mfma_f64_16x16x4f64(Bs[k * UR_LD + 16 * cb + li], fa[kq], acc[i][cb], 0, 0, 0);
      }
      if (more)
#pragma unroll
        for (int kq = 0; kq < 16; ++kq) fa[kq] = fn[kq];
    }
    __syncthreads();
  }
#pragma unroll
  for (int i = 0; i < UR_RB; ++i) {
    const int lr = 16 * (wv + 4 * i) + li;
    if (16 * (wv + 4 * i) >= nrows) continue;
#pragma unroll
    for (int cb = 0; cb < 2; ++cb)
#pragma unroll
      for (int r = 0; r < 4; ++r) {
        const int col = 16 * cb + lk + 4 * r;
        if (lr < nrows && col < nc) C[(int64_t)col * ld + t.ob0 + lr] = acc[i][cb][r];
      }
  }
}

__global__ __launch_bounds__(256) void k_tri_inv(const int32_t* __restrict__ list, int step,
                                                 const SNode* __restrict__ sn,
                                                 double* __restrict__ store,
                                                 double* __restrict__ scratch,
                                                 double* __restrict__ tinv) {
  __shared__ double sD[64 * 65];
  const int item = blockIdx.x >> 3, part = blockIdx.x & 7;
  const int sid = list[2 * item];
  const int64_t slot = list[2 * item + 1];
  const SNode s = sn[sid];
  FrontPtrs f = front_ptrs(s, store, scratch);
  const int64_t M = f.M;
  const int kb = step * s.nb;
  const int w = min(s.nb, (int)f.ns - kb);
  const gdbl* D = f.L + (int64_t)kb * M + kb;
  {
    double v[16];
#pragma unroll
    for (int u = 0; u < 16; ++u) {
      const int idx = threadIdx.x + 256 * u, i = idx & 63, j = idx >> 6;
      v[u] = (i < w && j < w) ? D[(int64_t)j * M + i] : (i == j ? 1.0 : 0.0);
    }
#pragma unroll
    for (int u = 0; u < 16; ++u) {
      const int idx = threadIdx.x + 256 * u, i = idx & 63, j = idx >> 6;
      sD[j * 65 + i] = v[u];
    }
  }
  __syncthreads();
  const int lane = threadIdx.x & 63, wv = threadIdx.x >> 6;
  const bool upper = part >= 4;
  const int c0 = ((part & 3) * 4 + wv) * 4;
  double z[4];
#pragma unroll
  for (int r = 0; r < 4; ++r) z[r] = lane == c0 + r ? 1.0 : 0.0;
  double* out = tinv + slot * 8192 + (upper ? 4096 : 0);
  if (!upper) {
#pragma unroll 4
    for (int j = 0; j < 63; ++j) {
      const double lij = sD[j * 65 + lane];
#pragma unroll
      for (int r = 0; r < 4; ++r) {
        const double zj = readlane_f64(z[r], j);
        if (lane > j) z[r] = fma(-lij, zj, z[r]);
      }
    }
#pragma unroll
    for (int r = 0; r < 4; ++r) out[(int64_t)(c0 + r) * 64 + lane] = lane > c0 + r ? -z[r] : 0.0;
  } else {
    const double rd = recip(sD[lane * 65 + lane]);
#pragma unroll 4
    for (int j = 63; j >= 0; --j) {
      const double uij = sD[j * 65 + lane];
#pragma unroll
      for (int r = 0; r < 4; ++r) {
        if (lane == j) z[r] *= rd;
        const double yj = readlane_f64(z[r], j);
        if (lane < j) z[r] = fma(-uij, yj, z[r]);
      }
    }
#pragma unroll
    for (int r = 0; r < 4; ++r) {
      const int c = c0 + r;
      out[(int64_t)c * 64 + lane] = lane == c ? 1.0 - z[r] : (lane < c ? -z[r] : 0.0);
    }
  }
}

#ifdef SMLU_CLOCK_PROBE
extern "C" int smlu_dev_gemm_clock(int arm, unsigned long long* out) {
  static unsigned long long* buf = nullptr;
  if (!buf && hipMalloc(&buf, 8 * sizeof(unsigned long long)) != hipSuccess) return -1;
  unsigned long long* p = nullptr;
  if (arm) {
    if (hipMemset(buf, 0, 8 * sizeof(unsigned long long)) != hipSuccess) return -1;
    p = buf;
  } else {
    if (hipDeviceSynchronize() != hipSuccess) return -1;
    if (out && hipMemcpy(out, buf, 8 * sizeof(unsigned long long), hipMemcpyDeviceToHost) != hipSuccess) return -1;
  }
  return hipMemcpyToSymbol(HIP_SYMBOL(g_clock_probe), &p, sizeof p) == hipSuccess ? 0 : -1;
}
#endif

hipError_t launch_gemm_g(hipStream_t st, int64_t ntiles, const GemmTask* tasks, int ntask, int tile,
                         int64_t maxwg, int32_t* info, double* growth, double piv_tol) {
  if (ntiles <= 0) return hipSuccess;
  const GrowthArgs ga{info, growth, piv_tol};
  const bool trsm = info != nullptr;
  if (tile == 135 && trsm) k_gemm128_mfma3<true, true><<<(unsigned)ntiles, 256, 0, st>>>(tasks, ntask, ga);
  else if (tile == 135) k_gemm128_mfma3<false, true><<<(unsigned)ntiles, 256, 0, st>>>(tasks, ntask, ga);
  else if (tile == 131 && trsm) k_gemm128_mfma3<true><<<(unsigned)ntiles, 256, 0, st>>>(tasks, ntask, ga);
  else if (tile == 131) k_gemm128_mfma3<false><<<(unsigned)ntiles, 256, 0, st>>>(tasks, ntask, ga);
  else if (tile == 65 && trsm) k_gemm_k64<true><<<(unsigned)ntiles, 256, 0, st>>>(tasks, ntask, ga);
  else if (tile == 65) k_gemm_k64<false><<<(unsigned)ntiles, 256, 0, st>>>(tasks, ntask, ga);
  else if (tile == 66 && trsm) k_gemm64_mfma<true><<<(unsigned)ntiles, 256, 0, st>>>(tasks, ntask, ga);
  else if (tile == 66) k_gemm64_mfma<false><<<(unsigned)ntiles, 256, 0, st>>>(tasks, ntask, ga);
  else if (trsm) k_gemm<true><<<(unsigned)ntiles, 256, 0, st>>>(tasks, ntask, ga);
  else k_gemm<false><<<(unsigned)ntiles, 256, 0, st>>>(tasks, ntask, ga);
  return hipGetLastError();
}
hipError_t launch_gemm(hipStream_t st, int64_t ntiles, const GemmTask* tasks, int ntask, int tile,
                       int64_t maxwg) {
  return launch_gemm_g(st, ntiles, tasks, ntask, tile, maxwg, nullptr, nullptr, 1.0);
}
hipError_t launch_urows(hipStream_t st, int cnt, const URowTask* tasks, const SNode* sn, double* store,
                        const double* tinv) {
  if (cnt <= 0) return hipSuccess;
  k_urows<<<(unsigned)cnt, 256, 0, st>>>(tasks, sn, store, tinv);
  return hipGetLastError();
}
hipError_t launch_tri_inv(hipStream_t st, int cnt, int step, const int32_t* list, const SNode* sn,
                          double* store, double* scratch, double* tinv) {
  if (cnt <= 0) return hipSuccess;
  k_tri_inv<<<(unsigned)cnt * 8, 256, 0, st>>>(list, step, sn, store, scratch, tinv);
  return hipGetLastError();
}

}
```

sharedmemsparselu.jl_amd/csrc/plan.hpp:

```cpp
#pragma once
#include <algorithm>
#include <cstdint>
#include <string>
#include <vector>

namespace smlu {

struct Tune {
  int ob = 0;
  int64_t t128_min = 512;
  bool small_k = true;
  int64_t fullpiv_ns = -1;
  int sweep_spin = 1 << 22;
  bool solve_steps = false;
  bool no_graph = false;
  bool debug_sync = false;
  bool no_repivot = false;
  int host_threads = 0;
};
Tune tune();


struct PlanOptions {
  int ordering = 0;
  int64_t grid[3] = {0, 0, 0};
  int relax = 1;
  int64_t leaf_size = 64;
  std::vector<int64_t> preorder;
};

struct Graph {
  int64_t n = 0;
  std::vector<int64_t> ptr;
  std::vector<int32_t> adj;
};

Graph build_sym_graph(int64_t n, const int64_t* colptr, const int32_t* rowval);
std::vector<int64_t> order_geometric_nd(int64_t nx, int64_t ny, int64_t nz, int64_t leaf);
std::vector<int64_t> order_graph_nd(const Graph& g, int64_t leaf);
std::vector<int64_t> order_amd(const Graph& g);
std::vector<int64_t> compute_order(int64_t n, const int64_t* colptr, const int32_t* rowval,
                                   const PlanOptions& opt, std::string& err);
std::vector<int64_t> zero_free_diagonal(int64_t n, const int64_t* colptr, const int32_t* rowval,
                                        const double* a);

struct Plan {
  int64_t n = 0, nnzA = 0;
  std::vector<int64_t> Acolptr;
  std::vector<int32_t> Arow;
  bool sym_pattern = false;

  std::vector<int64_t> q, qinv;
  std::vector<int64_t> p0, p0inv;
  bool given_order = false;
  bool matched = false;

  int64_t ntsup = 0;
  std::vector<int64_t> t_first;
  std::vector<int64_t> t_rowptr;
  std::vector<int32_t> t_rows;
  std::vector<int32_t> col2t;

  int64_t nsup = 0;
  std::vector<int64_t> s_first;
  std::vector<int64_t> s_parent;
  std::vector<int64_t> s_rowptr;
  std::vector<int32_t> s_rows;
  std::vector<int32_t> col2s;
  std::vector<int32_t> s_level;
  std::vector<int64_t> ch_ptr;
  std::vector<int32_t> ch_list;
  std::vector<int32_t> child_rank;
  std::vector<int32_t> relmap;
  int nlevels = 0;
  std::vector<int64_t> lev_ptr;
  std::vector<int32_t> lev_sup;

  std::vector<int64_t> Loff, Uoff;
  std::vector<int64_t> lev_foff;
  int64_t factor_size = 0;
  std::vector<int64_t> Foff;
  std::vector<int64_t> lev_soff, lev_ssize;
  int64_t scratch_size = 0;

  std::vector<int64_t> Adest;
  std::vector<int32_t> A_s, A_li, A_lj;
  std::vector<int64_t> Alev_ptr;
  std::vector<int32_t> Alev_ent;
  std::vector<int64_t> Arowptr;
  std::vector<int32_t> Arow_ent;

  double nnzL = 0, nnzU = 0;
  double upd = 0;
  double flops = 0;
  double stored = 0;
  int64_t front_max = 0, ns_max = 0, nu_max = 0;
  double analysis_ms = 0;
  double phase_ms[12] = {0};

  int nparts = 1;
  int64_t dob = 384;
  std::vector<int32_t> owner;
  std::vector<std::vector<int32_t>> group;
  std::vector<double> front_flops;
  void compute_owners(int nparts, int64_t block = 384);
  bool dist(int64_t s) const { return !group.empty() && group[s].size() > 1; }
  int64_t npblk(int64_t s) const { return (ns(s) + dob - 1) / dob; }
  int64_t nublk(int64_t s) const { return (nu(s) + dob - 1) / dob; }
  int32_t blk_owner(int64_t s, int64_t b) const { return group[s][b % group[s].size()]; }
  int64_t blk_c0(int64_t s, int64_t b) const {
    const int64_t np = npblk(s);
    return b < np ? b * dob : ns(s) + (b - np) * dob;
  }
  int64_t blk_c1(int64_t s, int64_t b) const {
    const int64_t np = npblk(s);
    return b < np ? std::min(ns(s), (b + 1) * dob) : std::min(M(s), ns(s) + (b - np + 1) * dob);
  }
  int32_t col_owner(int64_t s, int64_t c) const {
    if (!dist(s)) return owner[s];
    return c < ns(s) ? blk_owner(s, c / dob) : blk_owner(s, npblk(s) + (c - ns(s)) / dob);
  }

  std::string build(int64_t n, const int64_t* colptr, const int64_t* rowval, int index_base,
                    const PlanOptions& opt, const int64_t* pgiven = nullptr,
                    const int64_t* qgiven = nullptr, const int64_t* rowmatch = nullptr);

  int64_t ns(int64_t s) const { return s_first[s + 1] - s_first[s]; }
  int64_t nu(int64_t s) const { return s_rowptr[s + 1] - s_rowptr[s]; }
  int64_t M(int64_t s) const { return ns(s) + nu(s); }
  int64_t local_index(int64_t s, int64_t g) const;
};

struct RankLayout {
  int rank = 0;
  std::vector<int64_t> Loff, Uoff, Foff;
  struct Blk {
    int32_t s;
    int32_t b;
    int64_t c0, c1;
    int64_t loff;
    int64_t foff;
  };
  std::vector<Blk> blocks;
  std::vector<int64_t> recv_off, recv_size;
  int64_t store_size = 0, scratch_size = 0;
  int64_t stage_size = 0;
};
void rank_layout(const Plan& P, int rank, RankLayout& out);
double project_partition(const Plan& P, double tflops, double gbs, double lat_us, double* t1);

}
```

sharedmemsparselu.jl_amd/csrc/schedule.cpp:

```cpp
#include <cstddef>

#include "handle.hpp"

static void stage_sizes(const Schedule& S, int64_t& ss, int64_t& rs, int64_t& hs, int64_t& hr) {
  ss = rs = hs = hr = 0;
  for (const CommOp& op : S.comm) {
    int64_t a = 0, b = 0, sa = 0, sb = 0;
    for (size_t i = 0; i < op.peer.size(); ++i) {
      if (op.sbase[i] == 4) a = std::max(a, op.soff[i] + op.sbytes[i]);
      if (op.rbase[i] == 5) b = std::max(b, op.roff[i] + op.rbytes[i]);
      sa += op.sbytes[i];
      sb += op.rbytes[i];
    }
    if (op.type == 1 && op.bbase == 4) a = std::max(a, op.bytes);
    ss = std::max(ss, a);
    rs = std::max(rs, b);
    hs = std::max(hs, std::max(sa, op.type == 1 ? op.bytes : 0));
    hr = std::max(hr, std::max(sb, op.type == 1 ? op.bytes : 0));
  }
}

struct Sizes {
  int64_t store, scratch, bcbuf;
};
static Sizes sizes_of(const Plan& P, const RankLayout& lay, int rank, int nranks) {
  Sizes z{};
  int64_t maxM = 1;
  for (int64_t s = 0; s < P.nsup; ++s) maxM = std::max<int64_t>(maxM, P.M(s));
  z.store = std::max<int64_t>(lay.store_size, 1) + 64 * maxM + 4096;
  z.scratch = std::max<int64_t>(lay.scratch_size, 1);
  z.bcbuf = 0;
  if (nranks > 1) {
    z.bcbuf = 1;
    for (int64_t s = 0; s < P.nsup; ++s)
      if (P.dist(s) && std::binary_search(P.group[s].begin(), P.group[s].end(), rank))
        z.bcbuf = std::max<int64_t>(z.bcbuf, P.M(s) * P.dob + (P.dob / 64) * 8192 + (P.dob / 64) * kSwapStride / 2 + P.dob / 2 + 64);
  }
  return z;
}

static int upload_schedule(smlu_handle* h) {
  Schedule& S = h->sch;
  hipStream_t st = h->stream;
  static_assert(sizeof(AEnt) == sizeof(int2) && alignof(AEnt) == alignof(int2) && offsetof(AEnt, y) == offsetof(int2, y),
                "the kernels read the A-entry lists as int2");
  HIPCHK(h->sn.upload(S.hsn.data(), S.hsn.size(), st));
  HIPCHK(h->ilist.upload(S.ilist.data(), S.ilist.size(), st));
  HIPCHK(h->xtasks.upload(S.xt.data(), S.xt.size(), st));
  HIPCHK(h->aents.upload(reinterpret_cast<const int2*>(S.ae.data()), S.ae.size(), st));
  HIPCHK(h->ftiles.upload(S.ft.data(), S.ft.size(), st));
  if (!S.gptr.empty()) {
    HIPCHK(h->gptr.upload(S.gptr.data(), S.gptr.size(), st));
    HIPCHK(h->gent.upload(S.gent.data(), S.gent.size(), st));
  }
  if (S.ssync_n > 0) {
    HIPCHK(h->ssync.alloc((size_t)S.ssync_n));
    HIPCHK(h->stick.alloc((size_t)S.ntick));
    HIPCHK(h->sxh.alloc((size_t)S.ssync_n * 64 * kMultiRhs));
    {
      const long long sent = 0x7ff4dead5eed0001ll;
      double sv;
      std::memcpy(&sv, &sent, sizeof sv);
      HIPCHK(launch_fill(st, S.ssync_n * 64 * kMultiRhs, h->sxh.p, sv));
    }
    HIPCHK(hipMemsetAsync(h->ssync.p, 0, sizeof(int32_t) * S.ssync_n, st));
    HIPCHK(hipMemsetAsync(h->stick.p, 0, sizeof(unsigned long long) * S.ntick, st));
    HIPCHK(hipStreamSynchronize(st));
  }
  if (!h->sstatus.p) {
    HIPCHK(h->sstatus.alloc(1));
    HIPCHK(hipMemsetAsync(h->sstatus.p, 0, sizeof(int32_t), st));
  }
  h->sweep_spin = tune().sweep_spin;
  if (S.uses_tinv || h->nranks > 1) HIPCHK(h->tinv.alloc((size_t)S.max_list * 8192));
  std::vector<GemmTask> gt(S.gt.size());
  {
    double* base[8] = {h->store.p, h->scratch.p, nullptr, nullptr, nullptr, nullptr, h->bcbuf.p, h->tinv.p};
    auto addr = [&](const Operand& o) { return o.buf < 0 ? nullptr : base[o.buf] + o.off; };
    for (size_t i = 0; i < gt.size(); ++i) {
      const GemmRec& r = S.gt[i];
      gt[i] = GemmTask{addr(r.A), addr(r.B), addr(r.C), r.m, r.n, r.k, r.lda, r.ldb, r.ldc, r.tiles_m, r.gsid, r.tile0};
    }
  }
  HIPCHK(h->gtasks.upload(gt.data(), gt.size(), st));
  HIPCHK(h->stasks.upload(S.st_tasks.data(), S.st_tasks.size(), st));
  HIPCHK(h->urtasks.upload(S.ur_tasks.data(), S.ur_tasks.size(), st));
  HIPCHK(h->xcols.upload(S.xc.data(), S.xc.size(), st));
  HIPCHK(h->swaps.alloc((size_t)S.max_list * kSwapStride));
  HIPCHK(h->vbuf.alloc((size_t)std::max<int64_t>(S.voff, 1)));
  if (!S.comm.empty()) {
    int64_t ss, rs, hs, hr;
    stage_sizes(S, ss, rs, hs, hr);
    h->stage_bytes_s = ss;
    h->stage_bytes_r = rs;
    HIPCHK(h->stage_s.alloc((size_t)(ss + 7) / 8 + 1));
    HIPCHK(h->stage_r.alloc((size_t)(rs + 7) / 8 + 1));
    if (!h->tr.device_memory) {
      HIPCHK(hipHostMalloc((void**)&h->hstage_s, (size_t)std::max<int64_t>(hs, 8), 0));
      HIPCHK(hipHostMalloc((void**)&h->hstage_r, (size_t)std::max<int64_t>(hr, 8), 0));
    }
    char* base[10] = {(char*)h->store.p, (char*)h->scratch.p, (char*)h->vbuf.p, (char*)h->wrk.p,
                      (char*)h->stage_s.p, (char*)h->stage_r.p, (char*)h->bcbuf.p, (char*)h->tinv.p,
                      (char*)h->swaps.p, (char*)h->rowperm.p};
    std::vector<SegDesc> d;
    for (CommOp& op : S.comm) {
      auto emit = [&](const std::vector<HSeg>& v, int64_t& at) {
        at = (int64_t)d.size();
        for (const HSeg& g : v)
          d.push_back(SegDesc{(uint64_t)(base[g.sb] + g.so), (uint64_t)(base[g.db] + g.dof), g.bytes / 4});
      };
      emit(op.pack, op.pack0);
      emit(op.unpack, op.unpack0);
    }
    HIPCHK(h->segdesc.upload(d.data(), d.size(), st));
  }
  HIPCHK(hipStreamSynchronize(st));
  S.ilist = {}; S.xt = {}; S.ae = {}; S.xc = {}; S.ft = {}; S.gptr = {}; S.gent = {};
  S.gt = {}; S.st_tasks = {}; S.ur_tasks = {};
  return SMLU_OK;
}

void schedule_bytes(const Plan& P, const RankLayout& lay, const Schedule& S, int rank, int nranks, double out[5]) {
  const Sizes z = sizes_of(P, lay, rank, nranks);
  const double n = (double)P.n, nnzA = (double)P.nnzA;
  const int64_t nnodes = P.nsup + (int64_t)lay.blocks.size();
  int64_t ss, rs, hs, hr;
  stage_sizes(S, ss, rs, hs, hr);
  int64_t nseg = 0;
  for (const CommOp& op : S.comm) nseg += (int64_t)(op.pack.size() + op.unpack.size());
  out[1] = 8.0 * z.store;
  out[2] = 8.0 * z.scratch;
  out[3] = 8.0 * z.bcbuf + (nranks > 1 ? 64.0 : 0.0) + 8.0 * ((ss + 7) / 8 + 1) + 8.0 * ((rs + 7) / 8 + 1);
  out[4] = (double)hs + (double)hr;
  out[0] = out[1] + out[2] + 8.0 * nnzA + 8.0 * n * 3 + 8.0 + 8.0 * (n + 1) + 4.0 * nnzA * 2 + 8.0 * n * 3 +
           4.0 * (double)(P.s_rows.size() + P.relmap.size() + P.ch_list.size()) + 4.0 * n * 2 + 4.0 * (double)nnodes +
           8.0 * (16 + 5 * 512) + out[3];
  out[0] += sizeof(SNode) * (double)S.hsn.size() + 4.0 * S.ilist.size() + sizeof(XContrib) * (double)S.xt.size() +
            sizeof(AEnt) * (double)S.ae.size() + sizeof(FrontTile) * (double)S.ft.size() +
            4.0 * (S.gptr.size() + S.gent.size()) + 4.0 * S.ssync_n + 8.0 * S.ntick +
            8.0 * 64 * kMultiRhs * S.ssync_n + 4.0 + ((S.uses_tinv || nranks > 1) ? 8.0 * 8192 * S.max_list : 0.0) +
            sizeof(GemmTask) * (double)S.gt.size() + sizeof(SwapTask) * (double)S.st_tasks.size() +
            sizeof(URowTask) * (double)S.ur_tasks.size() + sizeof(XCol) * (double)S.xc.size() +
            4.0 * kSwapStride * S.max_list + 8.0 * std::max<int64_t>(S.voff, 1) + sizeof(SegDesc) * (double)nseg;
}

static int build_and_upload(smlu_handle* h) {
  ScheduleInput in;
  in.plan = &h->plan;
  in.lay = &h->lay;
  in.tn = tune();
  in.rank = h->rank;
  in.nranks = h->nranks;
  in.dominant = h->dominant;
  in.pivmode = h->pivmode;
  in.cpair = h->cpair;
  in.use_mfma = h->opts.use_mfma != 0;
  in.ob = h->sch.ob;
  const std::string e = build_schedule(in, h->sch);
  static_assert(kSchedErrArg == SMLU_ERR_ARG && kSchedErrAlloc == SMLU_ERR_ALLOC && kSchedErrState == SMLU_ERR_STATE,
                "the builder's error codes are smlu.h's");
  if (!e.empty()) return fail(h, h->sch.err_code, e);
  return upload_schedule(h);
}

int setup_device(smlu_handle* h) {
  Plan& P = h->plan;
  HIPCHK(hipSetDevice(h->device));
  int prio_lo = 0, prio_hi = 0;
  HIPCHK(hipDeviceGetStreamPriorityRange(&prio_lo, &prio_hi));
  if (!h->stream) HIPCHK(hipStreamCreateWithPriority(&h->stream, hipStreamNonBlocking, prio_hi));
  if (!h->side) HIPCHK(hipStreamCreateWithPriority(&h->side, hipStreamNonBlocking, prio_hi));
  if (!h->fork_ev) HIPCHK(hipEventCreateWithFlags(&h->fork_ev, hipEventDisableTiming));
  if (!h->join_ev) HIPCHK(hipEventCreateWithFlags(&h->join_ev, hipEventDisableTiming));
  hipStream_t st = h->stream;
  rank_layout_of(P, h->rank, h->nranks, h->lay);
  const Sizes z = sizes_of(P, h->lay, h->rank, h->nranks);
  HIPCHK(h->A.alloc((size_t)std::max<int64_t>(P.nnzA, 1)));
  HIPCHK(h->Rs.alloc((size_t)P.n));
  HIPCHK(h->store.alloc((size_t)z.store));
  HIPCHK(h->scratch.alloc((size_t)z.scratch));
  if (h->nranks > 1) {
    HIPCHK(h->bcbuf.alloc((size_t)z.bcbuf));
    HIPCHK(h->d_red.alloc(8));
  }
  HIPCHK(h->wrk.alloc((size_t)P.n));
  HIPCHK(h->wrk2.alloc((size_t)P.n));
  HIPCHK(h->growth.alloc(2));
  HIPCHK(h->Arowptr.upload(P.Arowptr.data(), P.Arowptr.size(), st));
  HIPCHK(h->Arow_ent.upload(P.Arow_ent.data(), P.Arow_ent.size(), st));
  HIPCHK(h->Arow.upload(P.Arow.data(), P.Arow.size(), st));
  HIPCHK(h->p0.upload(P.p0.data(), P.p0.size(), st));
  HIPCHK(h->q.upload(P.q.data(), P.q.size(), st));
  HIPCHK(h->rows.upload(P.s_rows.data(), P.s_rows.size(), st));
  HIPCHK(h->relmap.upload(P.relmap.data(), P.relmap.size(), st));
  HIPCHK(h->chlist.upload(P.ch_list.data(), P.ch_list.size(), st));
  std::vector<int64_t> pf(P.n);
  for (int64_t s = 0; s < P.nsup; ++s)
    for (int64_t j = P.s_first[s]; j < P.s_first[s + 1]; ++j) pf[j] = P.s_first[s];
  HIPCHK(h->posfirst.upload(pf.data(), pf.size(), st));
  HIPCHK(h->rowperm.alloc((size_t)P.n));
  {
    std::vector<int32_t> id(P.n);
    for (int64_t j = 0; j < P.n; ++j) id[j] = (int32_t)(j - pf[j]);
    HIPCHK(h->rowperm0.upload(id.data(), id.size(), st));
  }
  const int64_t nnodes = P.nsup + (int64_t)h->lay.blocks.size();
  HIPCHK(h->info.alloc((size_t)std::max<int64_t>(nnodes, 1)));
  HIPCHK(init_kernel_attributes());
  if (!h->rb.p) HIPCHK(h->rb.alloc(16 + 5 * 512));
  return build_and_upload(h);
}

static void release_schedule(smlu_handle* h) {
  h->release_graphs();
  h->sn.free();
  h->ilist.free();
  h->xtasks.free();
  h->aents.free();
  h->ftiles.free();
  h->gptr.free();
  h->gent.free();
  h->ssync.free();
  h->stick.free();
  h->sxh.free();
  h->gtasks.free();
  h->stasks.free();
  h->urtasks.free();
  h->xcols.free();
  h->swaps.free();
  h->vbuf.free();
  h->vbufm.free();
  h->tinv.free();
  h->stage_s.free();
  h->stage_r.free();
  h->segdesc.free();
  if (h->hstage_s) (void)hipHostFree(h->hstage_s);
  if (h->hstage_r) (void)hipHostFree(h->hstage_r);
  h->hstage_s = h->hstage_r = nullptr;
}

int rebuild_schedule(smlu_handle* h) {
  HIPCHK(hipSetDevice(h->device));
  HIPCHK(hipStreamSynchronize(h->stream));
  release_schedule(h);
  return build_and_upload(h);
}

bool has_tile_fronts(const smlu_handle* h) {
  for (const SNode& r : h->sch.hsn)
    if (r.mode == 2) return true;
  return false;
}
```

sharedmemsparselu.jl_amd/csrc/schedule.hpp:

```cpp
#pragma once
#include <algorithm>
#include <cstdint>
#include <string>
#include <vector>

#include "device.hpp"
#include "plan.hpp"

namespace smlu {

constexpr int kSmallM = 128;
constexpr int kFullPivNs = 512;
constexpr int kNbFull = 32;
constexpr int kNbTile = 64;
constexpr int kSwapStride = 1 + 2 * 64;
constexpr int kOBDefault = 384;

enum Kind : int {
  K_EXTADD, K_FRONT_LDS, K_PANEL, K_TRSMU, K_TRSML,
  K_GEMM, K_FWD, K_BWD, K_FWDG, K_TRIF, K_BWDU, K_TRIB, K_GEMM22, K_LASWP, K_STEPTRSM, K_GEMMU,
  K_GEMMO, K_TRIINV, K_BWDU12C, K_VCOPY, K_FWDT, K_BWDT, K_SWEEPF, K_SWEEPB, K_UROWS, K_FWDP, K_NKIND
};
inline const char* const kKindName[] = {"assemble", "small", "panel",
                                  "trsm", "trsm", "gemm", "solve", "solve", "solve", "solve",
                                  "solve", "solve", "gemm22", "trsm", "trsm", "gemmu", "gemmo", "trsm", "solve", "solve",
                                  "solve", "solve", "solve", "solve", "urows", "solve"};
static_assert(sizeof(kKindName) / sizeof(kKindName[0]) == K_NKIND, "one kKindName entry per launch kind");
constexpr int kSolveBigNs = 256;
constexpr int64_t kSolveBigWork = 1 << 16;
constexpr int kSolveMicroM = 8;
constexpr int kSolveTinyM = 128;

struct Launch {
  int kind = 0;
  int node = 0;
  int step = 0;
  int64_t off = 0, cnt = 0, nwg = 0, aux = 0, aux2 = 0;
  int64_t off2 = 0, cnt2 = 0, nwg2 = 0;
  double flops = 0;
  int grp = 0;
  bool side = false;
};

struct HSeg {
  int sb;
  int64_t so;
  int db;
  int64_t dof;
  int64_t bytes;
};

struct CommOp {
  int type = 0;
  std::vector<int32_t> peer;
  std::vector<int> sbase, rbase;
  std::vector<int64_t> soff, roff, sbytes, rbytes;
  int32_t root = -1;
  std::vector<int32_t> grp;
  int bbase = 4;
  int64_t bytes = 0;
  std::vector<HSeg> pack, unpack;
  int64_t pack0 = 0, unpack0 = 0;
  int at(int32_t p) {
    for (size_t i = 0; i < peer.size(); ++i)
      if (peer[i] == p) return (int)i;
    peer.push_back(p);
    sbase.push_back(4);
    rbase.push_back(5);
    soff.push_back(0);
    roff.push_back(0);
    sbytes.push_back(0);
    rbytes.push_back(0);
    return (int)peer.size() - 1;
  }
};

struct Operand {
  int buf = -1;
  int64_t off = 0;
  Operand operator+(int64_t d) const { return Operand{buf, off + d}; }
};
struct GemmRec {
  Operand A, B, C;
  int32_t m, n, k;
  int32_t lda, ldb, ldc;
  int32_t tiles_m = 0;
  int32_t gsid = -1;
  int64_t tile0 = 0;
};

struct ScheduleInput {
  const Plan* plan = nullptr;
  const RankLayout* lay = nullptr;
  Tune tn;
  int rank = 0, nranks = 1;
  bool dominant = false;
  int pivmode = 0;
  bool cpair = false;
  bool use_mfma = true;
  int ob = kOBDefault;
};

struct Schedule {
  std::vector<SNode> hsn;
  std::vector<int32_t> node_front;
  int64_t nnodes = 0;
  std::vector<Launch> fac, fwd, bwd;
  std::vector<Launch> fwdm, bwdm;
  std::vector<size_t> fac_seg, fwd_seg, bwd_seg;
  std::vector<size_t> fwdm_seg, bwdm_seg;
  std::vector<int> fac_comm, fwd_comm, bwd_comm;
  std::vector<CommOp> comm;
  std::vector<int32_t> ilist;
  std::vector<XContrib> xt;
  std::vector<AEnt> ae;
  std::vector<XCol> xc;
  std::vector<FrontTile> ft;
  std::vector<int32_t> gptr, gent;
  std::vector<GemmRec> gt;
  std::vector<SwapTask> st_tasks;
  std::vector<URowTask> ur_tasks;
  double gemm_flops = 0, gemm22_flops = 0;
  double gemm_bytes = 0;
  int64_t gemm_launches = 0, gemm128_launches = 0;
  int64_t nlaunch = 0;
  int64_t max_list = 1;
  int64_t ssync_n = 0, ntick = 0;
  int64_t voff = 0;
  bool uses_tinv = false;
  int ob = kOBDefault;
  int64_t t128_min = 512;
  bool small_k = true;
  bool trsm_gemm = true;
  int err_code = 0;
};
constexpr int kSchedErrArg = -1, kSchedErrAlloc = -3, kSchedErrState = -6;

std::string build_schedule(const ScheduleInput& in, Schedule& out);
void rank_layout_of(const Plan& P, int rank, int nranks, RankLayout& Y);
void schedule_digest(const Schedule& S, const double bytes[5], std::vector<uint64_t>& out);

}
```

sharedmemsparselu.jl_amd/csrc/schedule_build.cpp:

```cpp
#include "schedule.hpp"

#include <limits>
#include <unordered_map>
#include <utility>

namespace smlu {
namespace {

const Operand kStore{0, 0}, kScratch{1, 0}, kBlockBuf{6, 0}, kTinv{7, 0};

GemmRec gemm_task(Operand A, Operand B, Operand C, int64_t m, int64_t n, int64_t k, int64_t lda, int64_t ldb,
                  int64_t ldc, int32_t gsid = -1) {
  GemmRec g;
  g.A = A; g.B = B; g.C = C;
  g.m = (int32_t)m; g.n = (int32_t)n; g.k = (int32_t)k;
  g.lda = (int32_t)lda; g.ldb = (int32_t)ldb; g.ldc = (int32_t)ldc;
  g.gsid = gsid;
  return g;
}
void update(std::vector<GemmRec>& cand, double& fl, Operand A, Operand B, Operand C, int64_t m, int64_t n, int64_t k,
            int64_t lda, int64_t ldb, int64_t ldc) {
  if (m <= 0 || n <= 0 || k <= 0) return;
  cand.push_back(gemm_task(A, B, C, m, n, k, lda, ldb, ldc));
  fl += 2.0 * (double)m * (double)n * (double)k;
}
Operand tinv_at(int64_t slot, bool upper) { return kTinv + (slot * 8192 + (upper ? 4096 : 0)); }

int64_t tri_wg(bool upper, int64_t M, int64_t ns, int64_t jb) {
  if (upper) return std::max<int64_t>(1, (jb + 255) / 256);
  const int64_t bw = std::min<int64_t>(64, ns - jb);
  return std::max<int64_t>(1, (M - jb - bw + 255) / 256);
}

constexpr int kMfmaTile = 131;
constexpr bool kDistLookahead = false;

struct Builder {
  const ScheduleInput& in;
  const Plan& P;
  const RankLayout& Y;
  Schedule& S;
  const int rank, nranks;
  std::string err;
  std::vector<int32_t> blknode;
  std::unordered_map<int64_t, int32_t> blkmap;
  std::vector<int64_t> fr_ptr;
  std::vector<int32_t> fr_ent;
  std::vector<int64_t> LP;
  std::vector<int32_t> LS;
  std::vector<std::vector<int32_t>> dfront;
  std::vector<char> dlevel;
  int64_t dist_slots = 0;
  int64_t spf = 0;
  int fuse_mode = 0;
  bool fuse_panel = false, fuse_inv = false, fuse_urows = false;
  std::vector<int64_t> bidx;
  std::vector<int32_t> col_cnt, col_pos;
  std::vector<std::vector<Launch>> bwd_levels;

  Builder(const ScheduleInput& i, Schedule& s)
      : in(i), P(*i.plan), Y(*i.lay), S(s), rank(i.rank), nranks(i.nranks) {}

  static Launch launch(int kind, int step, size_t off) {
    Launch L;
    L.kind = kind;
    L.step = step;
    L.off = (int64_t)off;
    return L;
  }
  void fail(int code, const char* msg) {
    S.err_code = code;
    err = msg;
  }
  void add_comm(std::vector<Launch>& seq, std::vector<size_t>& seg, std::vector<int>& cm, CommOp&& op) {
    seg.push_back(seq.size());
    cm.push_back((int)S.comm.size());
    S.comm.push_back(std::move(op));
  }
  int32_t child_col(int64_t c, int64_t jc, int64_t* src) const {
    const int64_t nuc = P.nu(c);
    if (!P.dist(c)) {
      if (src && P.owner[c] == rank) *src = Y.Foff[c] + jc * nuc;
      return P.owner[c];
    }
    const int64_t b = P.npblk(c) + jc / P.dob;
    const int32_t o = P.blk_owner(c, b);
    if (src && o == rank) {
      const RankLayout::Blk& B = Y.blocks[blkmap.at((int64_t)c * 1048576 + b)];
      *src = B.foff + (P.ns(c) + jc - B.c0) * nuc;
    }
    return o;
  }
  int32_t node_of(int64_t s, int64_t b) const { return blknode[blkmap.at(s * 1048576 + b)]; }
  int32_t holder(int64_t c) const { return P.dist(c) ? P.blk_owner(c, P.npblk(c) - 1) : P.owner[c]; }
  bool gform(int64_t s) const { return S.trsm_gemm && S.hsn[s].nb == kNbTile; }
  int64_t slot_of(int64_t s, int64_t u) const { return dist_slots + bidx[s] * spf + u; }
  struct Step {
    int64_t kb, w, ostart, oend, R, M, slot;
  };
  Step geom(int64_t s, int64_t t) const {
    const SNode& r = S.hsn[s];
    Step g;
    g.M = (int64_t)r.ns + r.nu;
    g.kb = t * r.nb;
    g.w = std::min<int64_t>(r.nb, r.ns - g.kb);
    g.ostart = (g.kb / S.ob) * S.ob;
    g.oend = std::min<int64_t>(r.ns, g.ostart + S.ob);
    g.R = r.mode == 1 ? r.ns - g.kb : g.w;
    g.slot = slot_of(s, t % (S.ob / r.nb));
    return g;
  }
  void add_gemm_launch(std::vector<GemmRec>& cand, double fl, int step, int kind = K_GEMM) {
    if (cand.empty()) return;
    const bool count = kind != K_TRSML;
    int64_t t128 = 0;
    for (auto& g : cand) t128 += (int64_t)((g.m + 127) / 128) * ((g.n + 127) / 128);
    int tile = t128 >= S.t128_min && !(kind == K_TRSML && S.small_k) ? 128 : 64;
    if (tile == 128) tile = in.use_mfma ? kMfmaTile : 64;
    if (tile == 131 && step < 0) tile = 135;
    if (tile == 64 && S.small_k) {
      int kmax = 0;
      for (auto& g : cand) kmax = std::max(kmax, g.k);
      tile = kmax <= 64 ? 65 : in.use_mfma ? 66 : 64;
    }
    if (step < 0)
      std::stable_sort(cand.begin(), cand.end(), [](const GemmRec& a, const GemmRec& b) { return a.k > b.k; });
    Launch L = launch(step < 0 ? K_GEMM22 : kind, step, S.gt.size());
    L.aux = tile;
    int64_t tiles = 0;
    const int ts = tile >= 128 ? 128 : 64;
    for (GemmRec& g : cand) {
      if (count) S.gemm_bytes += 8.0 * ((double)g.m * g.k + (double)g.k * g.n + 2.0 * g.m * g.n);
      if (g.A.buf == kTinv.buf || g.B.buf == kTinv.buf) S.uses_tinv = true;
      g.tiles_m = (g.m + ts - 1) / ts;
      g.tile0 = tiles;
      tiles += (int64_t)g.tiles_m * ((g.n + ts - 1) / ts);
      S.gt.push_back(g);
    }
    L.cnt = (int64_t)cand.size();
    L.nwg = tiles;
    L.flops = fl;
    S.fac.push_back(L);
    if (!count) return;
    S.gemm_flops += fl;
    ++S.gemm_launches;
    if (tile >= 128) ++S.gemm128_launches;
    if (step < 0) S.gemm22_flops += fl;
  }

  void nodes() {
    const int64_t nsup = P.nsup;
    const int64_t full_piv_ns = (in.pivmode == 1 || in.cpair) ? std::numeric_limits<int64_t>::max()
                                : in.tn.fullpiv_ns >= 0 ? in.tn.fullpiv_ns
                                : in.dominant ? (int64_t)0 : (int64_t)kFullPivNs;
    S.hsn.resize(nsup);
    for (int64_t s = 0; s < nsup; ++s) {
      SNode r{};
      r.first = P.s_first[s];
      r.Loff = Y.Loff[s] >= 0 ? Y.Loff[s] : 0;
      r.Uoff = Y.Uoff[s] >= 0 ? Y.Uoff[s] : 0;
      r.Foff = Y.Foff[s];
      r.rowptr = P.s_rowptr[s];
      r.voff = S.voff;
      r.ns = (int32_t)P.ns(s);
      r.nu = (int32_t)P.nu(s);
      S.voff += P.M(s);
      r.parent = (int32_t)P.s_parent[s];
      if (P.M(s) <= kSmallM) { r.mode = 0; r.nb = 0; }
      else if (r.ns <= full_piv_ns) { r.mode = 1; r.nb = kNbFull; }
      else { r.mode = 2; r.nb = kNbTile; }
      r.chbeg = (int32_t)P.ch_ptr[s];
      r.chend = (int32_t)P.ch_ptr[s + 1];
      r.level = P.s_level[s];
      r.cpair = in.cpair ? 1 : 0;
      if (nranks > 1 && P.dist(s)) { r.mode = 2; r.nb = kNbTile; }
      S.hsn[s] = r;
    }
    S.node_front.resize(nsup);
    for (int64_t s = 0; s < nsup; ++s) S.node_front[s] = (int32_t)s;
    blknode.resize(Y.blocks.size());
    for (size_t i = 0; i < Y.blocks.size(); ++i) {
      const RankLayout::Blk& B = Y.blocks[i];
      SNode r = S.hsn[B.s];
      const int64_t ns = r.ns, nu = r.nu, M = ns + nu;
      if (B.c0 < ns) {
        r.Loff = B.loff - B.c0 * M;
      } else {
        r.Uoff = B.loff - (B.c0 - ns) * ns;
        r.Foff = B.foff - (B.c0 - ns) * nu;
      }
      blknode[i] = (int32_t)S.hsn.size();
      blkmap[(int64_t)B.s * 1048576 + B.b] = (int32_t)i;
      S.hsn.push_back(r);
      S.node_front.push_back(B.s);
    }
    S.nnodes = (int64_t)S.hsn.size();
  }

  void group_entries() {
    const int64_t nsup = P.nsup;
    fr_ptr.assign(nsup + 1, 0);
    fr_ent.resize((size_t)P.nnzA);
    for (int64_t e = 0; e < P.nnzA; ++e) ++fr_ptr[P.A_s[e] + 1];
    for (int64_t s = 0; s < nsup; ++s) fr_ptr[s + 1] += fr_ptr[s];
    std::vector<int64_t> fp(fr_ptr.begin(), fr_ptr.end() - 1);
    for (int64_t e = 0; e < P.nnzA; ++e) fr_ent[fp[P.A_s[e]]++] = (int32_t)e;
    for (int64_t s = 0; s < nsup; ++s) {
      if (nranks > 1 && !(P.dist(s) ? std::binary_search(P.group[s].begin(), P.group[s].end(), rank)
                                    : P.owner[s] == rank))
        continue;
      std::sort(fr_ent.begin() + fr_ptr[s], fr_ent.begin() + fr_ptr[s + 1], [&](int32_t a, int32_t b) {
        return P.A_lj[a] != P.A_lj[b] ? P.A_lj[a] < P.A_lj[b] : P.A_li[a] < P.A_li[b];
      });
    }
  }

  void levels() {
    LP.assign(P.nlevels + 1, 0);
    dfront.assign(P.nlevels, {});
    dlevel.assign(P.nlevels, 0);
    for (int l = 0; l < P.nlevels; ++l) {
      for (int64_t k = P.lev_ptr[l]; k < P.lev_ptr[l + 1]; ++k) {
        const int64_t s = P.lev_sup[k];
        if (nranks == 1) { LS.push_back((int32_t)s); continue; }
        if (!P.dist(s)) {
          if (P.owner[s] == rank) LS.push_back((int32_t)s);
          continue;
        }
        dlevel[l] = 1;
        if (std::binary_search(P.group[s].begin(), P.group[s].end(), rank)) dfront[l].push_back((int32_t)s);
      }
      LP[l + 1] = (int64_t)LS.size();
    }
    S.fac_seg.assign(1, 0);
    S.fwd_seg.assign(1, 0);
    S.bwd_seg.assign(1, 0);
    bidx.assign(P.nsup, 0);
    dist_slots = nranks > 1 ? S.ob / 32 : 0;
    spf = S.ob / 32;
    fuse_mode = !(S.trsm_gemm && S.ob <= 64 + 16 * 20) ? 0 : 2;
    fuse_panel = fuse_mode > 0;
    fuse_inv = fuse_mode == 2;
    fuse_urows = S.ob <= 384;
  }

  using RecvAt = std::unordered_map<int64_t, int64_t>;
  RecvAt f22_exchange(int l) {
    RecvAt recv_at;
    for (const int32_t t : dfront[l]) {
      CommOp op;
      std::vector<std::vector<std::pair<int64_t, int64_t>>> from(nranks);
      for (int64_t e = P.ch_ptr[t]; e < P.ch_ptr[t + 1]; ++e) {
        const int64_t c = P.ch_list[e];
        const int32_t* rm = P.relmap.data() + P.s_rowptr[c];
        const int64_t nuc = P.nu(c);
        for (int64_t jc = 0; jc < nuc; ++jc) {
          const int32_t dst = P.col_owner(t, rm[jc]);
          int64_t src = -1;
          const int32_t o = child_col(c, jc, &src);
          if (o == dst) continue;
          if (o == rank) {
            const int pi = op.at(dst);
            op.pack.push_back(HSeg{1, 8 * src, 4, 0, 8 * nuc});
            op.pack.back().db = 1000 + pi;
            op.sbytes[pi] += 8 * nuc;
          } else if (dst == rank) {
            from[o].push_back({c, jc});
          }
        }
      }
      int64_t ro = Y.recv_off[t];
      for (int32_t o = 0; o < nranks; ++o) {
        if (from[o].empty()) continue;
        const int pi = op.at(o);
        op.rbase[pi] = 1;
        op.roff[pi] = 8 * ro;
        for (auto& cj : from[o]) {
          recv_at[cj.first * 1048576 + cj.second] = ro;
          ro += P.nu(cj.first);
          op.rbytes[pi] += 8 * P.nu(cj.first);
        }
      }
      std::vector<int64_t> base(op.peer.size(), 0);
      int64_t acc = 0;
      for (size_t i = 0; i < op.peer.size(); ++i) {
        op.soff[i] = acc;
        base[i] = acc;
        acc += op.sbytes[i];
      }
      for (auto& g : op.pack) {
        const int pi = g.db - 1000;
        g.db = 4;
        g.dof = base[pi];
        base[pi] += g.bytes;
      }
      add_comm(S.fac, S.fac_seg, S.fac_comm, std::move(op));
    }
    return recv_at;
  }

  void front_columns(int64_t s, const std::vector<std::pair<int64_t, int64_t>>& ranges,
                     const std::vector<int32_t>& nodes, const RecvAt& recv_at) {
    std::vector<int32_t>&cnt = col_cnt, &pos = col_pos;
    const int64_t M = P.M(s);
    cnt.assign(M + 1, 0);
    for (int64_t ci = P.ch_ptr[s]; ci < P.ch_ptr[s + 1]; ++ci) {
      const int64_t c = P.ch_list[ci];
      const int32_t* rm = P.relmap.data() + S.hsn[c].rowptr;
      for (int64_t jc = 0; jc < P.nu(c); ++jc) ++cnt[rm[jc] + 1];
    }
    for (int64_t tj = 0; tj < M; ++tj) cnt[tj + 1] += cnt[tj];
    const int64_t base = (int64_t)S.xt.size();
    S.xt.resize(base + cnt[M]);
    pos.assign(cnt.begin(), cnt.end() - 1);
    for (int64_t ci = P.ch_ptr[s]; ci < P.ch_ptr[s + 1]; ++ci) {
      const int64_t c = P.ch_list[ci];
      const int32_t* rm = P.relmap.data() + S.hsn[c].rowptr;
      for (int64_t jc = 0; jc < P.nu(c); ++jc) {
        int64_t src = -1;
        if (nranks == 1) src = S.hsn[c].Foff + jc * P.nu(c);
        else if (P.col_owner(s, rm[jc]) == rank) {
          if (child_col(c, jc, &src) != rank) src = recv_at.at(c * 1048576 + jc);
        }
        S.xt[base + pos[rm[jc]]++] = XContrib{(int32_t)c, 0, src};
      }
    }
    int64_t ea = fr_ptr[s];
    const int64_t eb = fr_ptr[s + 1];
    for (size_t ri = 0; ri < ranges.size(); ++ri)
      for (int64_t tj = ranges[ri].first; tj < ranges[ri].second; ++tj) {
        while (ea < eb && P.A_lj[fr_ent[ea]] < tj) ++ea;
        const int64_t a0 = (int64_t)S.ae.size();
        while (ea < eb && P.A_lj[fr_ent[ea]] == tj) {
          S.ae.push_back(AEnt{fr_ent[ea], P.A_li[fr_ent[ea]]});
          ++ea;
        }
        S.xc.push_back(XCol{nodes[ri], (int32_t)tj, base + cnt[tj], cnt[tj + 1] - cnt[tj],
                            (int32_t)((int64_t)S.ae.size() - a0), a0});
      }
  }
  void assembly(int l, const RecvAt& recv_at) {
    Launch L = launch(K_EXTADD, 0, S.xc.size());
    for (int64_t k = LP[l]; k < LP[l + 1]; ++k) {
      const int64_t s = LS[k];
      if (S.hsn[s].mode != 0) front_columns(s, {{0, P.M(s)}}, {(int32_t)s}, recv_at);
    }
    for (const int32_t t : dfront[l]) {
      std::vector<std::pair<int64_t, int64_t>> ranges;
      std::vector<int32_t> nodes;
      for (size_t i = 0; i < Y.blocks.size(); ++i)
        if (Y.blocks[i].s == t) {
          ranges.push_back({Y.blocks[i].c0, Y.blocks[i].c1});
          nodes.push_back(blknode[i]);
        }
      front_columns(t, ranges, nodes, recv_at);
    }
    L.cnt = (int64_t)S.xc.size() - L.off;
    if (L.cnt > 0) S.fac.push_back(L);
  }

  void small_fronts(int l) {
    const int64_t cls[6] = {16, 32, 48, 64, 96, kSmallM};
    for (int c = 0; c < 6; ++c) {
      Launch L = launch(K_FRONT_LDS, 0, S.ilist.size());
      int64_t Mmax = 0;
      for (int64_t k = LP[l]; k < LP[l + 1]; ++k) {
        int64_t s = LS[k];
        if (S.hsn[s].mode != 0) continue;
        int64_t M = P.M(s);
        if (M > cls[c] || (c > 0 && M <= cls[c - 1])) continue;
        S.ilist.push_back((int32_t)s);
        S.ilist.push_back((int32_t)S.ae.size());
        S.ilist.push_back((int32_t)(fr_ptr[s + 1] - fr_ptr[s]));
        for (int64_t e = fr_ptr[s]; e < fr_ptr[s + 1]; ++e) {
          const int32_t id = fr_ent[e];
          S.ae.push_back(AEnt{id, (int32_t)((P.A_lj[id] << 16) | P.A_li[id])});
        }
        Mmax = std::max(Mmax, M);
      }
      L.cnt = ((int64_t)S.ilist.size() - L.off) / 3;
      L.aux = Mmax;
      L.aux2 = l + 1;
      if (L.cnt > 0) S.fac.push_back(L);
    }
    std::vector<std::pair<int64_t, int64_t>> wr, rd;
    for (int64_t k = LP[l]; k < LP[l + 1]; ++k) {
      const int64_t s = LS[k];
      if (S.hsn[s].mode != 0) continue;
      const int64_t nu = P.nu(s);
      if (nu > 0 && S.hsn[s].Foff >= 0) wr.push_back({S.hsn[s].Foff, S.hsn[s].Foff + nu * nu});
      for (int64_t e = P.ch_ptr[s]; e < P.ch_ptr[s + 1]; ++e) {
        const int64_t c = P.ch_list[e], nuc = P.nu(c);
        if (nuc > 0 && S.hsn[c].Foff >= 0) rd.push_back({S.hsn[c].Foff, S.hsn[c].Foff + nuc * nuc});
      }
    }
    std::sort(wr.begin(), wr.end());
    for (size_t i = 1; i < wr.size(); ++i)
      if (wr[i].first < wr[i - 1].second) {
        fail(kSchedErrState, "internal: overlapping F22 blocks in one level");
        return;
      }
    for (const auto& r : rd) {
      auto it = std::upper_bound(wr.begin(), wr.end(), std::make_pair(r.second, (int64_t)-1));
      if (it != wr.begin() && std::prev(it)->second > r.first) {
        fail(kSchedErrState, "internal: a level's F22 block overlaps a child's F22 it reads");
        return;
      }
    }
  }

  void blocked_fronts(int l) {
    std::vector<int64_t> big;
    int64_t maxsteps = 0;
    for (int64_t k = LP[l]; k < LP[l + 1]; ++k) {
      int64_t s = LS[k];
      const SNode& r = S.hsn[s];
      if (r.mode == 0) continue;
      bidx[s] = (int64_t)big.size();
      big.push_back(s);
      maxsteps = std::max<int64_t>(maxsteps, (r.ns + r.nb - 1) / r.nb);
    }
    S.max_list = std::max<int64_t>(S.max_list, dist_slots + (int64_t)big.size() * spf);
    for (int64_t t = 0; t < maxsteps; ++t) {
      std::vector<int64_t> act;
      for (auto s : big) {
        const SNode& r = S.hsn[s];
        if (t * r.nb < r.ns) act.push_back(s);
      }
      if (act.empty()) continue;
      step_panels(t, act);
      if (!err.empty()) return;
      step_solves(t, act);
      std::vector<int64_t> fin_all;
      for (auto s : act) {
        const Step g = geom(s, t);
        if (g.kb + g.w == g.oend) fin_all.push_back(s);
      }
      if (!fin_all.empty()) outer_block_end(t, fin_all);
    }
    std::vector<GemmRec> cand;
    double fl = 0;
    for (auto s : big) {
      const SNode& r = S.hsn[s];
      update(cand, fl, kStore + r.Loff + r.ns, kStore + r.Uoff, kScratch + r.Foff, r.nu, r.nu, r.ns,
             (int64_t)r.ns + r.nu, r.ns, r.nu);
    }
    add_gemm_launch(cand, fl, -1);
  }
  int pclass(int64_t s, int64_t t) const {
    const SNode& r = S.hsn[s];
    if (r.nb > 32) return 0;
    const int64_t R = r.mode == 1 ? r.ns - t * r.nb : std::min<int64_t>(r.nb, r.ns - t * r.nb);
    return R <= 64 ? 1 : R <= 128 ? 2 : R <= 256 ? 3 : R <= 512 ? 4 : 5;
  }
  void step_panels(int64_t t, std::vector<int64_t>& act) {
    std::stable_sort(act.begin(), act.end(), [&](int64_t a, int64_t b) { return pclass(a, t) < pclass(b, t); });
    size_t pos = 0;
    for (int c = 0; c < 6 && pos < act.size(); ++c) {
      Launch L = launch(K_PANEL, (int)t, S.ilist.size());
      int64_t rmax = 1, wmax = 1, cnt = 0;
      while (pos < act.size() && pclass(act[pos], t) == c) {
        const Step g = geom(act[pos], t);
        rmax = std::max(rmax, g.R);
        wmax = std::max<int64_t>(wmax, S.hsn[act[pos]].nb);
        S.ilist.push_back((int32_t)act[pos]);
        S.ilist.push_back((int32_t)g.slot);
        ++pos;
        ++cnt;
      }
      L.cnt = cnt;
      L.aux = 0;
      L.nwg = rmax;
      L.aux2 = wmax;
      L.cnt2 = c == 0 ? fuse_mode : 0;
      if (L.cnt > 0) S.fac.push_back(L);
    }
    if (pos != act.size()) fail(kSchedErrArg, "internal: panel classes");
  }
  void step_solves(int64_t t, const std::vector<int64_t>& act) {
    Launch L;
    L.kind = K_TRIINV;
    L.step = (int)t;
    L.off = (int64_t)S.ilist.size();
    for (auto s : act) {
      if (!gform(s) || fuse_inv) continue;
      S.ilist.push_back((int32_t)s);
      S.ilist.push_back((int32_t)geom(s, t).slot);
    }
    L.cnt = ((int64_t)S.ilist.size() - L.off) / 2;
    if (L.cnt > 0) S.fac.push_back(L);
    L = launch(K_LASWP, (int)t, S.st_tasks.size());
    int64_t wg = 0;
    for (auto s : act) {
      const Step g = geom(s, t);
      const int64_t ncol = g.oend - g.ostart - g.w;
      if (ncol <= 0 || (fuse_panel && gform(s))) continue;
      S.st_tasks.push_back(SwapTask{(int32_t)s, (int32_t)g.kb, 1, (int32_t)g.slot, (int32_t)g.ostart,
                                    (int32_t)g.oend, (int32_t)g.kb, (int32_t)(g.kb + g.w), wg});
      wg += (ncol + 63) / 64;
    }
    L.cnt = (int64_t)S.st_tasks.size() - L.off;
    L.nwg = wg;
    if (wg > 0) S.fac.push_back(L);
    Launch T = launch(K_STEPTRSM, (int)t, S.ft.size());
    int64_t wgU = 0, W = 32, ntri = 0;
    for (auto s : act) {
      if (gform(s)) continue;
      ++ntri;
      const Step g = geom(s, t);
      S.ft.push_back(FrontTile{(int32_t)s, (int32_t)g.kb, wgU});
      wgU += (g.oend - g.kb - g.w + 255) / 256;
      W = std::max<int64_t>(W, g.w);
    }
    T.cnt = ntri;
    T.nwg = wgU;
    T.off2 = (int64_t)S.ft.size();
    int64_t wgL = 0;
    for (auto s : act) {
      if (gform(s)) continue;
      const Step g = geom(s, t);
      S.ft.push_back(FrontTile{(int32_t)s, (int32_t)g.kb, wgL});
      wgL += (g.M - g.kb - g.R + 255) / 256;
    }
    T.cnt2 = ntri;
    T.nwg2 = wgL;
    T.aux = W;
    if (wgU + wgL > 0) S.fac.push_back(T);
    std::vector<GemmRec> tri, cand;
    double fl = 0;
    for (auto s : act) {
      const Step g = geom(s, t);
      const Operand F = kStore + S.hsn[s].Loff;
      if (gform(s)) {
        if (g.oend - g.kb - g.w > 0) {
          const Operand X = F + (g.kb + g.w) * g.M + g.kb;
          tri.push_back(gemm_task(tinv_at(g.slot, false), X, X, g.w, g.oend - g.kb - g.w, g.w, 64, g.M, g.M));
        }
        if (g.M - g.kb - g.R > 0) {
          const Operand X = F + g.kb * g.M + g.kb + g.R;
          tri.push_back(gemm_task(X, tinv_at(g.slot, true), X, g.M - g.kb - g.R, g.w, g.w, g.M, 64, g.M, (int32_t)s));
        }
      }
      update(cand, fl, F + g.kb * g.M + g.kb + g.w, F + (g.kb + g.w) * g.M + g.kb,
             F + (g.kb + g.w) * g.M + g.kb + g.w, g.M - g.kb - g.w, g.oend - g.kb - g.w, g.w, g.M, g.M, g.M);
    }
    add_gemm_launch(tri, 0.0, (int)t, K_TRSML);
    add_gemm_launch(cand, fl, (int)t);
  }
  void outer_block_end(int64_t t, const std::vector<int64_t>& fin_all) {
    Launch L = launch(K_LASWP, (int)t, S.st_tasks.size());
    int64_t wg = 0;
    for (auto s : fin_all) {
      const SNode& r = S.hsn[s];
      const Step g = geom(s, t);
      const int64_t ncol = g.M - (g.oend - g.ostart);
      if (ncol <= 0) continue;
      S.st_tasks.push_back(SwapTask{(int32_t)s, (int32_t)g.ostart, (int32_t)((g.oend - g.ostart + r.nb - 1) / r.nb),
                                    (int32_t)slot_of(s, (g.ostart % S.ob) / r.nb), 0, (int32_t)g.M,
                                    (int32_t)g.ostart, (int32_t)g.oend, wg});
      wg += (ncol + 63) / 64;
    }
    L.cnt = (int64_t)S.st_tasks.size() - L.off;
    L.nwg = wg;
    if (wg > 0) S.fac.push_back(L);
    std::vector<URows> items;
    std::vector<GemmRec> c1;
    double fl1 = 0;
    for (auto s : fin_all) {
      const SNode& r = S.hsn[s];
      const Step g = geom(s, t);
      if (g.oend == g.M) continue;
      items.push_back(URows{s, g.ostart, g.oend, g.oend, r.ns, true});
      rank_update(s, g.oend, g.M, g.oend, r.ns, false, g.ostart, g.oend, c1, fl1);
      rank_update(s, g.oend, r.ns, g.oend, g.oend, true, g.ostart, g.oend, c1, fl1);
    }
    urows(t, items);
    add_gemm_launch(c1, fl1, (int)t, K_GEMMO);
  }
  struct URows {
    int64_t s, ob0, ob1, c0, c1;
    bool u12;
  };
  void urows(int64_t t, const std::vector<URows>& all_items) {
    std::vector<URows> items;
    Launch L = launch(K_UROWS, (int)t, S.ur_tasks.size());
    for (auto& it : all_items) {
      const SNode& r = S.hsn[it.s];
      if (!(fuse_urows && gform(it.s))) {
        items.push_back(it);
        continue;
      }
      const int64_t M = (int64_t)r.ns + r.nu;
      const int32_t slot0 = (int32_t)slot_of(it.s, (it.ob0 % S.ob) / r.nb);
      for (int64_t c = it.c0; c < it.c1; c += kUrowsCols)
        S.ur_tasks.push_back(URowTask{(int32_t)it.s, (int32_t)it.ob0, (int32_t)it.ob1, slot0, (int32_t)M,
                                      (int32_t)std::min<int64_t>(kUrowsCols, it.c1 - c), r.Loff + c * M});
      if (it.u12)
        for (int64_t c = 0; c < r.nu; c += kUrowsCols)
          S.ur_tasks.push_back(URowTask{(int32_t)it.s, (int32_t)it.ob0, (int32_t)it.ob1, slot0, r.ns,
                                        (int32_t)std::min<int64_t>(kUrowsCols, r.nu - c), r.Uoff + c * r.ns});
    }
    L.cnt = (int64_t)S.ur_tasks.size() - L.off;
    if (L.cnt > 0) S.fac.push_back(L);
    int64_t nsub = 0;
    for (auto& it : items) nsub = std::max<int64_t>(nsub, (it.ob1 - it.ob0 + S.hsn[it.s].nb - 1) / S.hsn[it.s].nb);
    for (int64_t u = 0; u < nsub; ++u) {
      L = Launch();
      L.kind = K_TRSMU;
      L.step = (int)t;
      L.aux = 1;
      L.off = (int64_t)S.ft.size();
      int64_t wg = 0, cnt = 0;
      std::vector<GemmRec> cand, ctri;
      double fl = 0;
      for (auto& it : items) {
        const int64_t s = it.s;
        const SNode& r = S.hsn[s];
        const int64_t M = (int64_t)r.ns + r.nu;
        const int64_t kbu = it.ob0 + u * r.nb;
        if (kbu >= it.ob1) continue;
        const int64_t wu = std::min<int64_t>(r.nb, it.ob1 - kbu);
        const int64_t n1 = it.c1 - it.c0;
        const Operand F = kStore + r.Loff, U = kStore + r.Uoff;
        const bool u12 = it.u12 && r.nu > 0;
        if (gform(s)) {
          const Operand Ti = tinv_at(slot_of(s, (kbu % S.ob) / r.nb), false);
          if (n1 > 0) ctri.push_back(gemm_task(Ti, F + it.c0 * M + kbu, F + it.c0 * M + kbu, wu, n1, wu, 64, M, M));
          if (u12) ctri.push_back(gemm_task(Ti, U + kbu, U + kbu, wu, r.nu, wu, 64, r.ns, r.ns));
        } else {
          S.ft.push_back(FrontTile{(int32_t)s, (int32_t)kbu, wg});
          wg += (M - it.c0 + 255) / 256;
          ++cnt;
        }
        const int64_t m = it.ob1 - kbu - wu;
        update(cand, fl, F + kbu * M + kbu + wu, F + it.c0 * M + kbu, F + it.c0 * M + kbu + wu, m, n1, wu, M, M, M);
        if (u12) update(cand, fl, F + kbu * M + kbu + wu, U + kbu, U + kbu + wu, m, r.nu, wu, M, r.ns, r.ns);
      }
      L.cnt = cnt;
      L.nwg = wg;
      if (wg > 0) S.fac.push_back(L);
      add_gemm_launch(ctri, 0.0, (int)t, K_TRSML);
      add_gemm_launch(cand, fl, (int)t, K_GEMMU);
    }
  }
  void rank_update(int64_t s, int64_t r0, int64_t r1, int64_t c0, int64_t c1, bool u12, int64_t k0, int64_t k1,
                   std::vector<GemmRec>& cand, double& fl) {
    const SNode& r = S.hsn[s];
    const int64_t M = (int64_t)r.ns + r.nu;
    const Operand F = kStore + r.Loff, U = kStore + r.Uoff;
    update(cand, fl, F + k0 * M + r0, F + c0 * M + k0, F + c0 * M + r0, r1 - r0, c1 - c0, k1 - k0, M, M, M);
    const int64_t ru1 = std::min<int64_t>(r1, r.ns);
    if (u12) update(cand, fl, F + k0 * M + r0, U + k0, U + r0, ru1 - r0, r.nu, k1 - k0, M, r.ns, r.ns);
  }

  void shared_front(int32_t t) {
    const int64_t np = P.npblk(t);
    std::vector<size_t> mine;
    for (size_t i = 0; i < Y.blocks.size(); ++i)
      if (Y.blocks[i].s == t) mine.push_back(i);
    std::vector<Launch> pending;
    for (int64_t b = 0; b < np; ++b) {
      const bool own = P.blk_owner(t, b) == rank;
      const int32_t bn = own ? node_of(t, b) : -1;
      if (own) shared_block_factor(t, b, bn);
      shared_block_bcast(t, b, bn);
      for (auto& q : pending) S.fac.push_back(q);
      pending.clear();
      shared_block_apply(t, b, bn, mine, pending);
    }
    for (auto& q : pending) S.fac.push_back(q);
  }
  void shared_block_factor(int32_t t, int64_t b, int32_t bn) {
    const int64_t M = P.M(t), ob = P.blk_c0(t, b), oe = P.blk_c1(t, b);
    const Operand Lb = kStore + S.hsn[bn].Loff;
    for (int64_t kb = ob; kb < oe; kb += 64) {
      const int64_t wk = std::min<int64_t>(64, oe - kb);
      const int step = (int)(kb / 64);
      const int32_t u = (int32_t)((kb - ob) / 64);
      Launch Q = launch(K_PANEL, step, S.ilist.size());
      S.ilist.push_back(bn);
      S.ilist.push_back(u);
      Q.cnt = 1;
      Q.nwg = wk;
      Q.aux2 = 64;
      S.fac.push_back(Q);
      Q = launch(K_TRIINV, step, S.ilist.size());
      S.ilist.push_back(bn);
      S.ilist.push_back(u);
      Q.cnt = 1;
      S.fac.push_back(Q);
      if (oe - ob - wk > 0) {
        Q = launch(K_LASWP, step, S.st_tasks.size());
        S.st_tasks.push_back(SwapTask{bn, (int32_t)kb, 1, u, (int32_t)ob, (int32_t)oe, (int32_t)kb,
                                      (int32_t)(kb + wk), 0});
        Q.cnt = 1;
        Q.nwg = (oe - ob - wk + 63) / 64;
        S.fac.push_back(Q);
      }
      std::vector<GemmRec> tri, cand;
      double fl = 0;
      if (oe - kb - wk > 0) {
        const Operand X = Lb + (kb + wk) * M + kb;
        tri.push_back(gemm_task(tinv_at(u, false), X, X, wk, oe - kb - wk, wk, 64, M, M));
      }
      if (M - kb - wk > 0) {
        const Operand X = Lb + kb * M + kb + wk;
        tri.push_back(gemm_task(X, tinv_at(u, true), X, M - kb - wk, wk, wk, M, 64, M, bn));
      }
      add_gemm_launch(tri, 0.0, step, K_TRSML);
      update(cand, fl, Lb + kb * M + kb + wk, Lb + (kb + wk) * M + kb, Lb + (kb + wk) * M + kb + wk, M - kb - wk,
             oe - kb - wk, wk, M, M, M);
      add_gemm_launch(cand, fl, step);
    }
  }
  void shared_block_bcast(int32_t t, int64_t b, int32_t bn) {
    const SNode& fr = S.hsn[t];
    const int64_t M = P.M(t), ob = P.blk_c0(t, b), oe = P.blk_c1(t, b), w = oe - ob, nsub = (w + 63) / 64;
    const int64_t lbytes = 8 * (M - ob) * w, tbytes = 8 * nsub * 8192;
    const int64_t swbytes = 4 * nsub * kSwapStride, rpbytes = 4 * w;
    CommOp op;
    op.type = 1;
    op.root = P.blk_owner(t, b);
    op.grp = P.group[t];
    op.bytes = lbytes + tbytes + swbytes + rpbytes;
    if (op.root == rank) {
      op.bbase = 4;
      for (int64_t c = ob; c < oe; ++c)
        op.pack.push_back(HSeg{0, 8 * (S.hsn[bn].Loff + c * M + ob), 4, 8 * (c - ob) * (M - ob), 8 * (M - ob)});
      op.pack.push_back(HSeg{7, 0, 4, lbytes, tbytes});
      op.pack.push_back(HSeg{8, 0, 4, lbytes + tbytes, swbytes});
      op.pack.push_back(HSeg{9, 4 * (fr.first + ob), 4, lbytes + tbytes + swbytes, rpbytes});
    } else {
      op.bbase = 6;
      op.unpack.push_back(HSeg{6, lbytes + tbytes, 8, 0, swbytes});
      op.unpack.push_back(HSeg{6, lbytes + tbytes + swbytes, 9, 4 * (fr.first + ob), rpbytes});
    }
    add_comm(S.fac, S.fac_seg, S.fac_comm, std::move(op));
  }
  void shared_block_apply(int32_t t, int64_t b, int32_t bn, const std::vector<size_t>& mine,
                          std::vector<Launch>& pending) {
    const SNode& fr = S.hsn[t];
    const int64_t ns = fr.ns, nu = fr.nu, M = ns + nu, np = P.npblk(t);
    const int64_t ob = P.blk_c0(t, b), oe = P.blk_c1(t, b), w = oe - ob, nsub = (w + 63) / 64;
    const bool own = bn >= 0;
    const Operand Lb = own ? kStore + S.hsn[bn].Loff : Operand{};
    const int64_t ldL = own ? M : M - ob;
    auto Lsrc = [&](int64_t row, int64_t col) {
      return own ? Lb + col * M + row : kBlockBuf + ((col - ob) * (M - ob) + (row - ob));
// ... 147 lines not shown
    solve_gather(bigs);
    if (!err.empty()) return;
    Launch U = launch(K_BWDU, 0, S.ft.size());
    int64_t wg = 0;
    for (auto s : bigs) {
      S.ft.push_back(FrontTile{(int32_t)s, 0, wg});
      wg += (S.hsn[s].ns + 63) / 64;
    }
    U.cnt = (int64_t)bigs.size();
    U.nwg = wg;
    bl.push_back(U);
    if (!in.tn.solve_steps) {
      for (int upper = 0; upper < 2; ++upper) {
        Launch F = launch(upper ? K_SWEEPB : K_SWEEPF, 0, S.ft.size());
        F.aux = S.ssync_n;
        F.aux2 = S.ntick++;
        int64_t w = 0;
        int32_t fb = 0;
        for (auto s : bigs) {
          const SNode& r = S.hsn[s];
          const int64_t nbs = (r.ns + 63) / 64;
          S.ft.push_back(FrontTile{(int32_t)s, fb, w});
          w += upper ? (nbs + kSweepWK - 1) / kSweepWK
                     : ((int64_t)r.ns + r.nu + 64 * kSweepWK - 1) / (64 * kSweepWK);
          fb += (int32_t)nbs;
        }
        F.cnt = (int64_t)bigs.size();
        F.nwg = w;
        S.ssync_n += fb;
        (upper ? bl : S.fwd).push_back(F);
      }
      return;
    }
    int64_t nb = 0;
    for (auto s : bigs) nb = std::max<int64_t>(nb, (S.hsn[s].ns + 63) / 64);
    for (int64_t t = 0; t < nb; ++t)
      for (int upper = 0; upper < 2; ++upper) {
        Launch F = launch(upper ? K_TRIB : K_TRIF, (int)t, S.ft.size());
        int64_t w = 0, cnt = 0;
        for (auto s : bigs) {
          const SNode& r = S.hsn[s];
          const int64_t nbs = (r.ns + 63) / 64;
          if (t >= nbs) continue;
          S.ft.push_back(FrontTile{(int32_t)s, 0, w});
          w += tri_wg(upper, (int64_t)r.ns + r.nu, r.ns, (upper ? nbs - 1 - t : t) * 64);
          ++cnt;
        }
        F.cnt = cnt;
        F.nwg = w;
        (upper ? bl : S.fwd).push_back(F);
      }
  }
  void tri_steps(bool upper, int32_t node, int64_t ob, int64_t oe, std::vector<Launch>& out) {
    const SNode& r = S.hsn[node];
    const int64_t M = (int64_t)r.ns + r.nu, nbs = (r.ns + 63) / 64;
    std::vector<int64_t> jbs;
    for (int64_t jb = ob; jb < oe; jb += 64) jbs.push_back(jb);
    if (upper) std::reverse(jbs.begin(), jbs.end());
    for (int64_t jb : jbs) {
      Launch F = launch(upper ? K_TRIB : K_TRIF, (int)(upper ? nbs - 1 - jb / 64 : jb / 64), S.ft.size());
      S.ft.push_back(FrontTile{node, 0, 0});
      F.cnt = 1;
      F.nwg = tri_wg(upper, M, r.ns, jb);
      out.push_back(F);
    }
  }
  void vhop(std::vector<Launch>& seq, std::vector<size_t>& seg, std::vector<int>& cm, int32_t a, int32_t b,
            int64_t off, int64_t cnt) {
    if (a == b || cnt <= 0 || (rank != a && rank != b)) return;
    CommOp op;
    const int pi = op.at(rank == a ? b : a);
    if (rank == a) { op.sbase[pi] = 2; op.soff[pi] = 8 * off; op.sbytes[pi] = 8 * cnt; }
    else { op.rbase[pi] = 2; op.roff[pi] = 8 * off; op.rbytes[pi] = 8 * cnt; }
    add_comm(seq, seg, cm, std::move(op));
  }

  void shared_forward(int32_t t) {
    const int64_t np = P.npblk(t), M = P.M(t);
    const int64_t tv = S.hsn[t].voff;
    const int32_t o0 = P.blk_owner(t, 0);
    {
      CommOp op;
      std::vector<std::vector<int64_t>> kids(nranks);
      for (int64_t e = P.ch_ptr[t]; e < P.ch_ptr[t + 1]; ++e) kids[holder(P.ch_list[e])].push_back(P.ch_list[e]);
      for (int32_t q = 0; q < nranks; ++q) {
        if (q == o0 || kids[q].empty()) continue;
        if (rank != q && rank != o0) continue;
        const int pi = op.at(rank == q ? o0 : q);
        int64_t acc = 0;
        for (int64_t c : kids[q]) {
          const int64_t off = 8 * (S.hsn[c].voff + P.ns(c)), nb8 = 8 * P.nu(c);
          if (rank == q) op.pack.push_back(HSeg{2, off, 4, acc, nb8});
          else op.unpack.push_back(HSeg{5, acc, 2, off, nb8});
          acc += nb8;
        }
        if (rank == q) op.sbytes[pi] = acc;
        else op.rbytes[pi] = acc;
      }
      int64_t racc = 0;
      for (size_t i = 0; i < op.peer.size(); ++i) {
        op.roff[i] = racc;
        racc += op.rbytes[i];
      }
      if (rank == o0) {
        size_t k = 0;
        for (int32_t q = 0; q < nranks; ++q) {
          if (q == o0 || kids[q].empty()) continue;
          int64_t shift = 0;
          for (size_t i = 0; i < op.peer.size(); ++i)
            if (op.peer[i] == q) shift = op.roff[i];
          for (size_t j = 0; j < kids[q].size(); ++j) op.unpack[k++].so += shift;
        }
      }
      if (!op.peer.empty()) add_comm(S.fwd, S.fwd_seg, S.fwd_comm, std::move(op));
    }
    if (rank == o0) {
      Launch L = launch(K_FWDG, 0, S.ilist.size());
      S.ilist.push_back(t);
      L.cnt = 1;
      S.fwd.push_back(L);
    }
    for (int64_t b = 0; b < np; ++b) {
      const int32_t o = P.blk_owner(t, b);
      const int64_t ob = P.blk_c0(t, b), oe = P.blk_c1(t, b);
      if (rank == o) tri_steps(false, node_of(t, b), ob, oe, S.fwd);
      if (b + 1 < np) vhop(S.fwd, S.fwd_seg, S.fwd_comm, o, P.blk_owner(t, b + 1), tv + oe, M - oe);
    }
  }

  using Rows = std::vector<std::pair<int64_t, int64_t>>;
  void backward() {
    std::vector<Rows> pending_rows(nranks);
    Rows myrows;
    for (int l = P.nlevels - 1; l >= 0; --l) {
      for (auto& L : bwd_levels[l]) S.bwd.push_back(L);
      if (nranks == 1) continue;
      for (int64_t k = P.lev_ptr[l]; k < P.lev_ptr[l + 1]; ++k) {
        const int64_t s = P.lev_sup[k];
        if (!P.dist(s)) {
          pending_rows[P.owner[s]].push_back({P.s_first[s], P.ns(s)});
          continue;
        }
        for (int64_t b = 0; b < P.npblk(s); ++b)
          pending_rows[P.blk_owner(s, b)].push_back({P.s_first[s] + P.blk_c0(s, b), P.blk_c1(s, b) - P.blk_c0(s, b)});
      }
      for (const int32_t t : dfront[l]) shared_backward(t);
      for (auto& rg : pending_rows[rank]) myrows.push_back(rg);
      pending_rows[rank].clear();
      if (dlevel[l] || l == 0) xbwd(pending_rows, myrows);
    }
  }
  void xbwd(std::vector<Rows>& pending_rows, Rows& myrows) {
    CommOp op;
    int64_t mine = 0;
    for (auto& rg : myrows) {
      op.pack.push_back(HSeg{3, 8 * rg.first, 4, 8 * mine, 8 * rg.second});
      mine += rg.second;
    }
    std::vector<Rows> theirs(nranks);
    theirs.swap(pending_rows);
    int64_t racc = 0;
    for (int32_t q = 0; q < nranks; ++q) {
      if (q == rank) continue;
      const int pi = op.at(q);
      op.soff[pi] = 0;
      op.sbytes[pi] = 8 * mine;
      op.roff[pi] = racc;
      int64_t cnt = 0;
      for (auto& rg : theirs[q]) {
        op.unpack.push_back(HSeg{5, racc + 8 * cnt, 3, 8 * rg.first, 8 * rg.second});
        cnt += rg.second;
      }
      op.rbytes[pi] = 8 * cnt;
      racc += 8 * cnt;
    }
    myrows.clear();
    add_comm(S.bwd, S.bwd_seg, S.bwd_comm, std::move(op));
  }
  void shared_backward(int32_t t) {
    const int64_t np = P.npblk(t), nbk = np + P.nublk(t), ns = P.ns(t);
    const int64_t tv = S.hsn[t].voff;
    const int32_t cs = nbk > np ? P.blk_owner(t, np) : P.blk_owner(t, np - 1);
    {
      CommOp op;
      const int64_t f0 = P.s_first[t];
      for (int32_t q = 0; q < nranks; ++q) {
        if (q == cs || (rank != q && rank != cs)) continue;
        int64_t acc = 0;
        std::vector<HSeg> segs;
        for (int64_t b = 0; b < np; ++b) {
          if (P.blk_owner(t, b) != q) continue;
          const int64_t o8 = 8 * (f0 + P.blk_c0(t, b)), nb8 = 8 * (P.blk_c1(t, b) - P.blk_c0(t, b));
          segs.push_back(rank == q ? HSeg{3, o8, 4, acc, nb8} : HSeg{5, acc, 3, o8, nb8});
          acc += nb8;
        }
        if (acc == 0) continue;
        const int pi = op.at(rank == q ? cs : q);
        if (rank == q) {
          op.sbytes[pi] = acc;
          for (auto& g : segs) op.pack.push_back(g);
        } else {
          op.rbytes[pi] = acc;
          for (auto& g : segs) op.unpack.push_back(g);
        }
      }
      if (rank == cs) {
        int64_t racc = 0;
        size_t k = 0;
        for (size_t i = 0; i < op.peer.size(); ++i) {
          op.roff[i] = racc;
          int64_t left = op.rbytes[i];
          while (left > 0 && k < op.unpack.size()) {
            op.unpack[k].so += racc;
            left -= op.unpack[k].bytes;
            ++k;
          }
          racc += op.rbytes[i];
        }
      }
      if (!op.peer.empty()) add_comm(S.bwd, S.bwd_seg, S.bwd_comm, std::move(op));
    }
    int32_t prev = -1;
    bool first = true;
    for (int64_t ub = np; ub < nbk; ++ub) {
      const int32_t o = P.blk_owner(t, ub);
      if (prev >= 0) vhop(S.bwd, S.bwd_seg, S.bwd_comm, prev, o, tv, ns);
      if (rank == o) {
        Launch L;
        L.kind = K_BWDU12C;
        L.node = node_of(t, ub);
        L.aux = P.blk_c0(t, ub);
        L.aux2 = P.blk_c1(t, ub);
        L.cnt = first ? 1 : 0;
        S.bwd.push_back(L);
      }
      prev = o;
      first = false;
    }
    if (first) {
      prev = P.blk_owner(t, np - 1);
      if (rank == prev) {
        Launch L;
        L.kind = K_VCOPY;
        L.node = t;
        S.bwd.push_back(L);
      }
    }
    for (int64_t b = np - 1; b >= 0; --b) {
      const int32_t o = P.blk_owner(t, b);
      const int64_t ob = P.blk_c0(t, b), oe = P.blk_c1(t, b);
      vhop(S.bwd, S.bwd_seg, S.bwd_comm, prev, o, tv, oe);
      if (rank == o) tri_steps(true, node_of(t, b), ob, oe, S.bwd);
      prev = o;
    }
  }

  void expand(const Launch& Sw, bool upper, std::vector<Launch>& out) {
    std::vector<int32_t> fr;
    for (int64_t i = Sw.off; i < Sw.off + Sw.cnt; ++i) fr.push_back(S.ft[i].s);
    int64_t nb = 0;
    for (auto s : fr) nb = std::max<int64_t>(nb, (S.hsn[s].ns + 63) / 64);
    for (int64_t t = 0; t < nb; ++t) {
      Launch F;
      F.kind = upper ? K_TRIB : K_TRIF;
      F.grp = Sw.grp;
      F.step = (int)t;
      F.off = (int64_t)S.ft.size();
      int64_t w = 0, cnt = 0;
      for (auto s : fr) {
        const SNode& r = S.hsn[s];
        const int64_t nbs = (r.ns + 63) / 64;
        if (t >= nbs) continue;
        S.ft.push_back(FrontTile{s, 0, w});
        w += tri_wg(upper, (int64_t)r.ns + r.nu, r.ns, (upper ? nbs - 1 - t : t) * 64);
        ++cnt;
      }
      F.cnt = cnt;
      F.nwg = w;
      out.push_back(F);
    }
  }
  void expand_all(const std::vector<Launch>& seq, const std::vector<size_t>& seg, bool upper,
                  std::vector<Launch>& out, std::vector<size_t>& oseg) {
    std::vector<size_t> at(seq.size() + 1);
    for (size_t i = 0; i < seq.size(); ++i) {
      at[i] = out.size();
      if (seq[i].kind == (upper ? K_SWEEPB : K_SWEEPF)) expand(seq[i], upper, out);
      else out.push_back(seq[i]);
    }
    at[seq.size()] = out.size();
    oseg.clear();
    for (size_t k : seg) oseg.push_back(at[std::min(k, seq.size())]);
  }

  std::string run() {
    S = Schedule();
    S.ob = in.tn.ob > 0 ? in.tn.ob : in.ob;
    S.t128_min = in.tn.t128_min;
    S.small_k = in.tn.small_k;
    S.trsm_gemm = in.use_mfma;
    nodes();
    group_entries();
    levels();
    for (int l = 0; l < P.nlevels && err.empty(); ++l) {
      assembly(l, f22_exchange(l));
      small_fronts(l);
      if (err.empty()) blocked_fronts(l);
      if (!err.empty()) break;
      for (const int32_t t : dfront[l]) shared_front(t);
    }
    for (int l = 0; l < P.nlevels && err.empty(); ++l) {
      solve_level(l);
      for (const int32_t t : dfront[l]) shared_forward(t);
    }
    if (!err.empty()) return err;
    backward();
    S.nlaunch = (int64_t)S.fac.size();
    expand_all(S.fwd, S.fwd_seg, false, S.fwdm, S.fwdm_seg);
    expand_all(S.bwd, S.bwd_seg, true, S.bwdm, S.bwdm_seg);
    if (nranks > 1) S.max_list = std::max<int64_t>(S.max_list, dist_slots);
    return err;
  }
};

}

std::string build_schedule(const ScheduleInput& in, Schedule& out) { return Builder(in, out).run(); }

void rank_layout_of(const Plan& P, int rank, int nranks, RankLayout& Y) {
  if (nranks > 1) {
    rank_layout(P, rank, Y);
    return;
  }
  Y = RankLayout();
  Y.Loff = P.Loff;
  Y.Uoff = P.Uoff;
  Y.Foff = P.Foff;
  Y.recv_off.assign(P.nsup, -1);
  Y.recv_size.assign(P.nsup, 0);
  Y.store_size = P.factor_size;
  Y.scratch_size = P.scratch_size;
}

}
```

sharedmemsparselu.jl_amd/csrc/smlu.cpp:

```cpp
#include "handle.hpp"

namespace smlu {
thread_local std::string g_last_error;
}

static int check_device(smlu_handle* h) {
  int cnt = 0;
  hipError_t e = hipGetDeviceCount(&cnt);
  if (e != hipSuccess || cnt <= 0)
    return fail(h, SMLU_ERR_NODEVICE, "no HIP device visible (libsmlu has no CPU fallback)");
  if (h->opts.device < 0 || h->opts.device >= cnt)
    return fail(h, SMLU_ERR_NODEVICE, "opts.device out of range");
  hipDeviceProp_t prop;
  if (hipGetDeviceProperties(&prop, h->opts.device) != hipSuccess)
    return fail(h, SMLU_ERR_NODEVICE, "hipGetDeviceProperties failed");
  if (std::strncmp(prop.gcnArchName, "gfx950", 6) != 0)
    return fail(h, SMLU_ERR_NODEVICE, std::string("device is ") + prop.gcnArchName + ", libsmlu is built for gfx950 only");
  h->device = h->opts.device;
  return SMLU_OK;
}

std::vector<int64_t> diagonal_match(int64_t n, const int64_t* colptr, const int64_t* rowval,
                                    const double* a, int64_t base) {
  bool need = false;
  for (int64_t j = 0; j < n && !need; ++j) {
    bool has = false;
    for (int64_t e = colptr[j] - base; e < colptr[j + 1] - base; ++e)
      if (rowval[e] - base == j) has = a[e] != 0.0;
    need = !has;
  }
  if (!need) return {};
  const int64_t nnz = colptr[n] - base;
  std::vector<int64_t> cp(n + 1);
  std::vector<int32_t> ri((size_t)std::max<int64_t>(nnz, 1));
  for (int64_t j = 0; j <= n; ++j) cp[j] = colptr[j] - base;
  for (int64_t e = 0; e < nnz; ++e) ri[e] = (int32_t)(rowval[e] - base);
  std::vector<int64_t> m = zero_free_diagonal(n, cp.data(), ri.data(), a);
  bool ident = true;
  for (int64_t j = 0; j < (int64_t)m.size() && ident; ++j) ident = m[j] == j;
  if (ident) m.clear();
  return m;
}

int create_impl(int64_t n, const int64_t* colptr, const int64_t* rowval, const double* nzval,
                const int64_t* p, const int64_t* q, const double* Rs, const smlu_opts* opts,
                smlu_handle** out, int rank, int nranks, const smlu_transport* tr, RcclState* rccl,
                const std::vector<int64_t>* preorder) {
  std::unique_ptr<RcclState> rccl_own(rccl);
  if (!out) return fail(nullptr, SMLU_ERR_ARG, "out is NULL");
  *out = nullptr;
  if (n <= 0 || !colptr || (!rowval && n > 0) || !nzval)
    return fail(nullptr, SMLU_ERR_ARG, "invalid matrix arguments");
  std::unique_ptr<smlu_handle> h(new (std::nothrow) smlu_handle());
  if (!h) return fail(nullptr, SMLU_ERR_ALLOC, "allocation failed");
  h->rccl = rccl_own.release();
  if (tr) h->tr = *tr;
  if (opts) h->opts = *opts;
  else smlu_default_opts(&h->opts);
  if (!valid_opts(&h->opts)) return fail(nullptr, SMLU_ERR_ARG, "index_base must be 0 or 1");
  if (h->opts.chunk_size <= 0 || h->opts.chunk_size > n) h->opts.chunk_size = std::min<int64_t>(8, n);
  int rc = check_device(h.get());
  if (rc != SMLU_OK) return rc;
  std::string e;
  try {
    std::vector<int64_t> match;
    if (!p && h->opts.ordering != SMLU_ORDER_GIVEN)
      match = diagonal_match(n, colptr, rowval, nzval, h->opts.index_base);
    PlanOptions po = plan_opts(h->opts);
    if (preorder) po.preorder = *preorder;
    e = h->plan.build(n, colptr, rowval, h->opts.index_base, po, p, q,
                      match.empty() ? nullptr : match.data());
  } catch (const std::bad_alloc&) {
    return fail(nullptr, SMLU_ERR_ALLOC, "host allocation failed during analysis");
  }
  if (!e.empty()) return fail(nullptr, SMLU_ERR_ARG, e);
  h->rank = rank;
  h->nranks = nranks;
  h->cpair = preorder != nullptr && !h->plan.matched;
  if (!p && !h->plan.matched) h->dominant = diagonally_dominant(n, colptr, rowval, nzval, h->opts.index_base);
  if (nranks > 1) {
    if (tune().ob > 0) h->sch.ob = tune().ob;
    h->plan.compute_owners(nranks, h->sch.ob);
    h->opts.profile = 0;
  }
  rc = setup_device(h.get());
  if (rc != SMLU_OK) { g_last_error = h->err; return rc; }
  if (h->rccl) {
    static_cast<RcclState*>(h->rccl)->stream = h->stream;
    static_cast<RcclState*>(h->rccl)->dbuf = h->d_red.p;
  }
  hipStream_t st = h->stream;
  {
    smlu_handle* hp = h.get();
    smlu_handle* h = hp;
    HIPCHK(hipMemcpyAsync(h->A.p, nzval, sizeof(double) * h->plan.nnzA, hipMemcpyHostToDevice, st));
    if (Rs) {
      HIPCHK(hipMemcpyAsync(h->Rs.p, Rs, sizeof(double) * n, hipMemcpyHostToDevice, st));
      h->given_Rs = true;
    }
  }
  rc = run_factor(h.get());
  *out = h.release();
  return rc;
}


void smlu_default_opts(smlu_opts* o) {
  if (!o) return;
  std::memset(o, 0, sizeof(*o));
  o->chunk_size = 8;
  o->index_base = 1;
  o->ordering = SMLU_ORDER_AUTO;
  o->scale = 1;
  o->relax = 1;
  o->pivot_tol = 0.1;
  o->diag_pivot_tol = 0.001;
  o->device = 0;
  o->profile = 0;
  o->leaf_size = 64;
  o->use_mfma = 1;
  o->refine = -1;
  o->vendor_gemm = 0;
}

int smlu_create(int64_t n, const int64_t* colptr, const int64_t* rowval, const double* nzval,
                const smlu_opts* opts, smlu_handle** out) {
  return create_impl(n, colptr, rowval, nzval, nullptr, nullptr, nullptr, opts, out);
}

int smlu_create_i32(int64_t n, const int32_t* colptr, const int32_t* rowval, const double* nzval,
                    const smlu_opts* opts, smlu_handle** out) {
  if (!out || !colptr || n <= 0) return fail(nullptr, SMLU_ERR_ARG, "invalid matrix arguments");
  const int64_t base = opts ? opts->index_base : 1;
  const int64_t nnz = (int64_t)colptr[n] - base;
  if (nnz < 0 || (nnz > 0 && !rowval)) return fail(nullptr, SMLU_ERR_ARG, "invalid matrix arguments");
  std::vector<int64_t> cp(colptr, colptr + n + 1), rv(rowval, rowval + nnz);
  return smlu_create(n, cp.data(), rv.data(), nzval, opts, out);
}

void smlu_destroy(smlu_handle* h) { delete h; }

const char* smlu_last_error_string(const smlu_handle* h) {
  if (h) return h->err.c_str();
  return g_last_error.c_str();
}

int64_t smlu_last_error_col(const smlu_handle* h) {
  if (!h) return -1;
  return (h->zc && h->errcol >= 0) ? h->errcol / 2 : h->errcol;
}

static double plan_stat(const Plan& P, const std::string& k) {
  if (k.rfind("phase_ms", 0) == 0) {
    const int i = std::atoi(k.c_str() + 8);
    return i >= 0 && i < 12 ? P.phase_ms[i] : std::numeric_limits<double>::quiet_NaN();
  }
  if (k == "n") return (double)P.n;
  if (k == "nnzA") return (double)P.nnzA;
  if (k == "nsuper") return (double)P.nsup;
  if (k == "ntsuper") return (double)P.ntsup;
  if (k == "nlevels") return (double)P.nlevels;
  if (k == "nnzL") return P.nnzL;
  if (k == "nnzU") return P.nnzU;
  if (k == "nnzLU") return P.nnzL + P.nnzU - (double)P.n;
  if (k == "upd") return P.upd;
  if (k == "dense_flops") return P.flops;
  if (k == "stored") return P.stored;
  if (k == "front_max") return (double)P.front_max;
  if (k == "ns_max") return (double)P.ns_max;
  if (k == "nu_max") return (double)P.nu_max;
  if (k == "factor_bytes") return 8.0 * (double)P.factor_size;
  if (k == "scratch_bytes") return 8.0 * (double)P.scratch_size;
  if (k == "analysis_ms") return P.analysis_ms;
  if (k == "extadd_entries") {
    double t = 0;
    for (int64_t s = 0; s < P.nsup; ++s)
      if (P.s_parent[s] >= 0) t += (double)P.nu(s) * (double)P.nu(s);
    return t;
  }
  return std::numeric_limits<double>::quiet_NaN();
}

double smlu_stat(const smlu_handle* h, const char* key) {
  if (!h || !key) return std::numeric_limits<double>::quiet_NaN();
  std::string k(key);
  if (k == "complex") return h->zc ? 1.0 : 0.0;
  if (k == "cpair") return h->cpair ? 1.0 : 0.0;
  if (k == "launches") return (double)h->sch.nlaunch;
  if (k == "refactor_ms_last") return h->refactor_ms;
  if (k == "solve_ms_last") return h->solve_ms;
  if (k == "growth_max") return h->growth_max;
  if (k == "weak") return (double)h->weak;
  if (k == "dominant") return h->dominant ? 1.0 : 0.0;
  if (k == "pivmode") return (double)h->pivmode;
  if (k == "matched") return h->plan.matched ? 1.0 : 0.0;
  if (k == "nranks") return (double)h->nranks;
  if (k == "owned_blocks") return (double)h->lay.blocks.size();
  if (k == "comm_steps") return (double)h->sch.comm.size();
  if (k == "comm_calls") return (double)h->comm_calls;
  if (k == "comm_bytes_sent") return h->comm_sent;
  if (k == "comm_bytes_recv") return h->comm_recv;
  if (k == "comm_bytes_sent_refactor") return h->comm_sent_fac;
  if (k == "comm_bytes_recv_refactor") return h->comm_recv_fac;
  if (k == "rccl_nranks") return h->rccl ? (double)static_cast<const RcclState*>(h->rccl)->comm_count : 0.0;
  if (k == "store_bytes_rank") return 8.0 * (double)h->lay.store_size;
  if (k == "scratch_bytes_rank") return 8.0 * (double)h->lay.scratch_size;
  if (k == "shared_fronts") {
    double c = 0;
    for (int64_t s = 0; s < h->plan.nsup && h->nranks > 1; ++s)
      if (h->plan.dist(s) && std::binary_search(h->plan.group[s].begin(), h->plan.group[s].end(), h->rank)) ++c;
    return c;
  }
  if (k == "repivots") return (double)h->repivots;
  if (k == "mode_refactors") return (double)h->mode_refactors;
  if (k == "repivot_node") return (double)h->repivot_node;
  if (k == "repivot_info") return (double)h->repivot_info;
  if (k == "repivot_growth") return h->repivot_growth;
  if (k == "repivot_node_mode" || k == "repivot_node_ns" || k == "repivot_node_nu") {
    if (h->repivot_node < 0) return -1;
    const SNode& r = h->repivot_sn;
    return k == "repivot_node_mode" ? r.mode : k == "repivot_node_ns" ? r.ns : r.nu;
  }
  if (k == "pivot_tol") return h->opts.pivot_tol;
  if (k == "diag_pivot_tol") return h->plan.given_order ? 0.0 : h->opts.diag_pivot_tol;
  if (k == "sweep_timeouts") {
    return (double)h->sweep_timeouts;
  }
  if (k == "sweep_status") {
    int32_t v = 0;
    if (h->sstatus.p && hipMemcpy(&v, h->sstatus.p, sizeof v, hipMemcpyDeviceToHost) != hipSuccess) return -1;
    return v;
  }
  if (k == "solve_sweeps") {
    int64_t c = 0;
    for (const Launch& L : h->sch.fwd) c += L.kind == K_SWEEPF;
    for (const Launch& L : h->sch.bwd) c += L.kind == K_SWEEPB;
    return (double)c;
  }
  if (k.rfind("launches_", 0) == 0) {
    const std::string v = k.substr(9);
    double c = 0;
    for (const Launch& L : h->sch.fac) {
      const bool gemm = L.kind == K_GEMM || L.kind == K_GEMMU || L.kind == K_GEMMO || L.kind == K_GEMM22;
      const bool trsm = L.kind == K_TRSML;
      const bool mfma = L.aux == 131 || L.aux == 135;
      if (v == "mfma128" && gemm && mfma) ++c;
      else if (v == "mfma128_trsm" && trsm && mfma) ++c;
      else if (v == "k64" && gemm && L.aux == 65) ++c;
      else if (v == "k64_trsm" && trsm && L.aux == 65) ++c;
      else if (v == "valu64" && gemm && L.aux == 64) ++c;
      else if (v == "mfma64" && gemm && L.aux == 66) ++c;
      else if (v == "valu64_trsm" && trsm && L.aux == 64) ++c;
      else if (v == "tri_inv" && L.kind == K_TRIINV) ++c;
      else if (v == "panel_tall" && L.kind == K_PANEL && L.nwg > 512) ++c;
    }
    return c;
  }
  if (k.rfind("fronts_mode", 0) == 0) {
    const int m = std::atoi(k.c_str() + 11);
    double c = 0;
    for (const SNode& r : h->sch.hsn) c += r.mode == m ? 1 : 0;
    return c;
  }
  if (k == "pattern_dropped") return (double)h->pattern_dropped;
  if (k == "given_pattern") return h->given_pattern ? 1.0 : 0.0;
  if (k == "status_copy_retries") return (double)h->status_copy_retries;
  if (k == "bad_info_count") return (double)h->bad_info_count;
  if (k == "bad_info_node") return (double)h->bad_info_node;
  if (k == "bad_info_word") return (double)h->bad_info_word;
  if (k == "refine_steps") return (double)h->refine_steps;
  if (k == "refine_residual") return h->refine_resid;
  if (k == "refine_berr") return h->refine_berr;
  if (k == "gemm_flops") return h->sch.gemm_flops;
  if (k == "gemm22_flops") return h->sch.gemm22_flops;
  if (k == "gemm_launches") return (double)h->sch.gemm_launches;
  if (k == "gemm_bytes") return h->sch.gemm_bytes;
  if (k == "gemm128_launches") return (double)h->sch.gemm128_launches;
  if (k == "vendor_calls") return 0.0;
  if (k.rfind("ms_", 0) == 0) {
    std::string name = k.substr(3);
    double t = 0;
    bool found = false;
    for (int i = 0; i < K_NKIND; ++i)
      if (name == kKindName[i]) { t += h->kind_ms[i]; found = true; }
    return found ? t : std::numeric_limits<double>::quiet_NaN();
  }
  return plan_stat(h->plan, k);
}

int smlu_plan_create(int64_t n, const int64_t* colptr, const int64_t* rowval, const smlu_opts* opts,
                     smlu_plan** out) {
  if (!out || !colptr || n <= 0) return fail(nullptr, SMLU_ERR_ARG, "invalid arguments");
  smlu_opts o;
  if (opts) o = *opts;
  else smlu_default_opts(&o);
  if (!valid_opts(&o)) return fail(nullptr, SMLU_ERR_ARG, "index_base must be 0 or 1");
  std::unique_ptr<smlu_plan> p(new smlu_plan());
  std::string e = p->plan.build(n, colptr, rowval, o.index_base, plan_opts(o));
  if (!e.empty()) return fail(nullptr, SMLU_ERR_ARG, e);
  *out = p.release();
  return SMLU_OK;
}

double smlu_plan_stat(const smlu_plan* plan, const char* key) {
  if (!plan || !key) return std::numeric_limits<double>::quiet_NaN();
  return plan_stat(plan->plan, key);
}

int smlu_plan_pattern(const smlu_plan* pl, int64_t* q, int64_t* Lcolptr, int64_t* Lrowval) {
  if (!pl) return SMLU_ERR_ARG;
  const Plan& P = pl->plan;
  if (q) for (int64_t i = 0; i < P.n; ++i) q[i] = P.q[i];
  if (Lcolptr || Lrowval) {
    int64_t o = 0;
    if (Lcolptr) Lcolptr[0] = 0;
    for (int64_t j = 0; j < P.n; ++j) {
      int64_t t = P.col2t[j], last = P.t_first[t + 1] - 1;
      if (Lrowval) {
        for (int64_t i = j; i <= last; ++i) Lrowval[o++] = i;
        for (int64_t e = P.t_rowptr[t]; e < P.t_rowptr[t + 1]; ++e) Lrowval[o++] = P.t_rows[e];
      } else {
        o += last - j + 1 + P.t_rowptr[t + 1] - P.t_rowptr[t];
      }
      if (Lcolptr) Lcolptr[j + 1] = o;
    }
  }
  return SMLU_OK;
}

int smlu_plan_supernodes(const smlu_plan* pl, int64_t* first, int64_t* parent, int64_t* level) {
  if (!pl) return SMLU_ERR_ARG;
  const Plan& P = pl->plan;
  for (int64_t s = 0; s <= P.nsup; ++s)
    if (first) first[s] = P.s_first[s];
  for (int64_t s = 0; s < P.nsup; ++s) {
    if (parent) parent[s] = P.s_parent[s];
    if (level) level[s] = P.s_level[s];
  }
  return SMLU_OK;
}

static void fronts_of(const Plan& P, int64_t* first, int64_t* parent, int64_t* rowptr, int64_t* rows,
                      int64_t* p0) {
  for (int64_t s = 0; s <= P.nsup; ++s) {
    if (first) first[s] = P.s_first[s];
    if (rowptr) rowptr[s] = P.s_rowptr[s];
  }
  for (int64_t s = 0; s < P.nsup; ++s)
    if (parent) parent[s] = P.s_parent[s];
  if (rows)
    for (int64_t e = 0; e < P.s_rowptr[P.nsup]; ++e) rows[e] = P.s_rows[e];
  if (p0)
    for (int64_t i = 0; i < P.n; ++i) p0[i] = P.p0[i];
}

int smlu_plan_fronts(const smlu_plan* pl, int64_t* rowptr, int64_t* rows, int64_t* p0) {
  if (!pl) return SMLU_ERR_ARG;
  fronts_of(pl->plan, nullptr, nullptr, rowptr, rows, p0);
  return SMLU_OK;
}

int smlu_get_fronts(smlu_handle* h, int64_t* first, int64_t* parent, int64_t* rowptr, int64_t* rows,
                    int64_t* p0, int32_t* mode) {
  if (!h) return fail(h, SMLU_ERR_ARG, "NULL handle");
  fronts_of(h->plan, first, parent, rowptr, rows, p0);
  if (mode)
    for (int64_t s = 0; s < h->plan.nsup; ++s) mode[s] = h->sch.hsn[s].mode;
  return SMLU_OK;
}

void smlu_plan_destroy(smlu_plan* p) { delete p; }

const char* smlu_version(void) { return "smlu 0.1.0 (gfx950, fp64, multifrontal)"; }
```

sharedmemsparselu.jl_amd/csrc/tune.cpp:

```cpp
#include <algorithm>
#include <cstdlib>

#include "plan.hpp"

namespace smlu {

Tune tune() {
  Tune v;
  {
    if (const char* e = std::getenv("SMLU_OB")) v.ob = std::max(64, (std::atoi(e) / 64) * 64);
    if (const char* e = std::getenv("SMLU_T128MIN")) v.t128_min = std::atoll(e);
    if (const char* e = std::getenv("SMLU_SMALLK")) v.small_k = std::atoi(e) != 0;
    if (const char* e = std::getenv("SMLU_FULLPIV_NS")) v.fullpiv_ns = std::atoll(e);
    if (const char* e = std::getenv("SMLU_SWEEP_SPIN")) v.sweep_spin = std::atoi(e);
    if (const char* e = std::getenv("SMLU_SOLVE_STEPS")) v.solve_steps = std::atoi(e) == 1;
    v.no_graph = std::getenv("SMLU_NO_GRAPH") != nullptr;
    v.debug_sync = std::getenv("SMLU_DEBUG_SYNC") != nullptr;
    v.no_repivot = std::getenv("SMLU_NO_REPIVOT") != nullptr;
    if (const char* e = std::getenv("OMP_NUM_THREADS")) v.host_threads = std::atoi(e);
  }
  return v;
}

}
```

Measured before the change: 6.358 billion.

## Fuse child F22 extend-add gather into Schur-complement GEMM accumulator init

For large blocked fronts with few children, the F22 Schur update GEMM now starts its accumulators by gathering the children's contribution blocks through inverse row maps, instead of loading a C block that an earlier extend-add pass had to write. The extend-add kernel is told to skip the F22 region of those columns and handle only the L/U part. This removes one full write and re-read of the F22 block through HBM. The cost is irregular per-element gathered loads and extra index tables in the GEMM prologue, plus a host-side check that the gather never reads a block the same launch writes. It is enabled by default only on a single rank without cpair and with MFMA.

```diff
diff --git a/sharedmemsparselu.jl_amd/csrc/device.hpp b/sharedmemsparselu.jl_amd/csrc/device.hpp
--- a/sharedmemsparselu.jl_amd/csrc/device.hpp
+++ b/sharedmemsparselu.jl_amd/csrc/device.hpp
@@ -25,6 +25,17 @@
   int32_t tiles_m;
   int32_t gsid = -1;
   int64_t tile0;
+};
+
+struct F22Gather {
+  int32_t beg, cnt;
+};
+struct F22Child {
+  int64_t foff;
+  int64_t inv;
+  int32_t nu;
+  int32_t lo, hi;
+  int32_t pad;
 };
 
 constexpr int kUrowsCols = 32;
@@ -57,6 +68,7 @@
   int64_t n4;
 };
 
+constexpr int32_t kXColNoF22 = 1 << 30;
 struct XCol {
   int32_t p, tj;
   int64_t off;
diff --git a/sharedmemsparselu.jl_amd/csrc/factor.cpp b/sharedmemsparselu.jl_amd/csrc/factor.cpp
--- a/sharedmemsparselu.jl_amd/csrc/factor.cpp
+++ b/sharedmemsparselu.jl_amd/csrc/factor.cpp
@@ -28,6 +28,9 @@
     case K_GEMMU:
     case K_GEMMO:
     case K_GEMM22:
+      if (L.aux == 143)
+        return launch_gemm_gather(st, L.nwg, h->gtasks.p + L.off, (int)L.cnt, h->f22tasks.p + L.off2, h->f22ch.p,
+                                  h->f22inv.p, h->scratch.p);
       return launch_gemm(st, L.nwg, h->gtasks.p + L.off, (int)L.cnt, (int)L.aux, 0);
     case K_TRSML:
       return launch_gemm_g(st, L.nwg, h->gtasks.p + L.off, (int)L.cnt, (int)L.aux, 0, h->info.p,
diff --git a/sharedmemsparselu.jl_amd/csrc/handle.hpp b/sharedmemsparselu.jl_amd/csrc/handle.hpp
--- a/sharedmemsparselu.jl_amd/csrc/handle.hpp
+++ b/sharedmemsparselu.jl_amd/csrc/handle.hpp
@@ -41,6 +41,8 @@
                          double*, const int32_t*, int64_t);
 hipError_t launch_gemm(hipStream_t, int64_t, const GemmTask*, int, int, int64_t);
 hipError_t launch_gemm_g(hipStream_t, int64_t, const GemmTask*, int, int, int64_t, int32_t*, double*, double);
+hipError_t launch_gemm_gather(hipStream_t, int64_t, const GemmTask*, int, const F22Gather*, const F22Child*,
+                              const int32_t*, const double*);
 hipError_t launch_tri_inv(hipStream_t, int, int, const int32_t*, const SNode*, double*, double*, double*);
 hipError_t launch_urows(hipStream_t, int, const URowTask*, const SNode*, double*, const double*);
 hipError_t launch_fwd_tiny(hipStream_t, int, const int32_t*, const SNode*, const int32_t*, const int32_t*,
@@ -195,6 +197,9 @@
   DBuf<unsigned long long> stick;
   DBuf<double> sxh;
   DBuf<GemmTask> gtasks;
+  DBuf<F22Gather> f22tasks;
+  DBuf<F22Child> f22ch;
+  DBuf<int32_t> f22inv;
   DBuf<SwapTask> stasks;
   DBuf<URowTask> urtasks;
   DBuf<XCol> xcols;
@@ -283,6 +288,9 @@
     stick.free();
     sxh.free();
     gtasks.free();
+    f22tasks.free();
+    f22ch.free();
+    f22inv.free();
     stasks.free();
     urtasks.free();
     xcols.free();
diff --git a/sharedmemsparselu.jl_amd/csrc/kernels_front.hip b/sharedmemsparselu.jl_amd/csrc/kernels_front.hip
--- a/sharedmemsparselu.jl_amd/csrc/kernels_front.hip
+++ b/sharedmemsparselu.jl_amd/csrc/kernels_front.hip
@@ -53,8 +53,8 @@
   const XCol t = cols[w];
   const SNode p = sn[t.p];
   FrontPtrs P = front_ptrs(p, store, scratch);
-  const int64_t len = P.M;
-  const int64_t tj = t.tj;
+  const int64_t len = (t.tj & kXColNoF22) ? P.ns : P.M;
+  const int64_t tj = t.tj & ~kXColNoF22;
   gdbl* colL = tj < P.ns ? P.L + tj * P.M : nullptr;
   gdbl* colU = tj < P.ns ? nullptr : P.U + (tj - P.ns) * P.ns;
   gdbl* colF = (tj < P.ns || P.nu == 0) ? nullptr : P.F + (tj - P.ns) * P.nu - P.ns;
diff --git a/sharedmemsparselu.jl_amd/csrc/kernels_gemm.hip b/sharedmemsparselu.jl_amd/csrc/kernels_gemm.hip
--- a/sharedmemsparselu.jl_amd/csrc/kernels_gemm.hip
+++ b/sharedmemsparselu.jl_amd/csrc/kernels_gemm.hip
@@ -312,10 +312,43 @@
 #define HBM_ 128
 #define HBK_ 16
 #define HLDB_ (HBM_ + 2)
-template <bool TRSM, bool FULL>
+__device__ __forceinline__ double sel0(bool c, double x) {
+  return __longlong_as_double(__double_as_longlong(x) & (c ? -1LL : 0LL));
+}
+struct GatherArgs {
+  const F22Gather* tg;
+  const F22Child* ch;
+  const int32_t* inv;
+  const double* scratch;
+};
+struct F22Tile {
+  const F22Child* ch;
+  const int32_t* inv;
+  const double* scratch;
+  int cnt;
+};
+__device__ __forceinline__ double f22_child_val(const char* src, int nuc, int ri, int cj) {
+  const bool ok = (ri | cj) >= 0;
+  const uint32_t off = ok ? ((uint32_t)cj * (uint32_t)nuc + (uint32_t)ri) * 8u : 0u;
+  return sel0(ok, *(const gdbl*)(src + off));
+}
+__device__ __forceinline__ void f22_child_add(v4d (&acc)[4][4], int j, const char* src, int nuc, const int (&ri)[4],
+                                              const int (&cj)[4]) {
+  double v[4][4];
+#pragma unroll
+  for (int r = 0; r < 4; ++r)
+#pragma unroll
+    for (int i = 0; i < 4; ++i) v[i][r] = f22_child_val(src, nuc, ri[i], cj[r]);
+#pragma unroll
+  for (int r = 0; r < 4; ++r)
+#pragma unroll
+    for (int i = 0; i < 4; ++i) acc[i][j][r] += v[i][r];
+  __builtin_amdgcn_sched_barrier(0);
+}
+template <bool TRSM, bool FULL, bool GATHER = false>
 __device__ __forceinline__ void gemm128_mfma_body(const GemmTask& t, int m0, int n0,
                                                 double (&As)[2][HBK_][HBM_], double (&Bs)[2][HBK_][HLDB_],
-                                                const GrowthArgs& ga) {
+                                                const GrowthArgs& ga, const F22Tile& fg = F22Tile{}) {
   const gdbl* gA = gbl(t.A);
   const gdbl* gB = gbl(t.B);
   gdbl* gC = gbl(t.C);
@@ -323,16 +356,48 @@
   const int wr = (wv & 1) * 64, wc = (wv >> 1) * 64;
   const int li = lane & 15, lk = lane >> 4;
   v4d acc[4][4];
-#pragma unroll
-  for (int i = 0; i < 4; ++i) {
-    const int row = m0 + wr + 16 * i + li;
-#pragma unroll
-    for (int j = 0; j < 4; ++j)
-#pragma unroll
-      for (int r = 0; r < 4; ++r) {
-        const int col = n0 + wc + 16 * j + lk + 4 * r;
-        acc[i][j][r] = (FULL || (row < t.m && col < t.n)) ? gC[(int64_t)col * t.ldc + row] : 0.0;
-      }
+  if (GATHER && fg.cnt >= 0) {
+#pragma unroll
+    for (int i = 0; i < 4; ++i)
+#pragma unroll
+      for (int j = 0; j < 4; ++j) acc[i][j] = v4d{0.0, 0.0, 0.0, 0.0};
+#pragma unroll 1
+    for (int d = 0; d < fg.cnt; ++d) {
+      const F22Child c = fg.ch[d];
+      if (c.hi < m0 + wr || c.lo >= m0 + wr + 64 || c.hi < n0 + wc || c.lo >= n0 + wc + 64) continue;
+      const int32_t* inv = fg.inv + c.inv;
+      const char* src = reinterpret_cast<const char*>(fg.scratch + c.foff);
+      int ri[4], cj[4][4];
+#pragma unroll
+      for (int i = 0; i < 4; ++i) {
+        const int row = m0 + wr + 16 * i + li;
+        const int v = inv[min(row, t.m - 1)];
+        ri[i] = row < t.m ? v : -1;
+      }
+#pragma unroll
+      for (int j = 0; j < 4; ++j)
+#pragma unroll
+        for (int r = 0; r < 4; ++r) {
+          const int col = n0 + wc + 16 * j + lk + 4 * r;
+          const int v = inv[min(col, t.n - 1)];
+          cj[j][r] = col < t.n ? v : -1;
+        }
+      __builtin_amdgcn_sched_barrier(0);
+#pragma unroll
+      for (int j = 0; j < 4; ++j) f22_child_add(acc, j, src, c.nu, ri, cj[j]);
+    }
+  } else {
+#pragma unroll
+    for (int i = 0; i < 4; ++i) {
+      const int row = m0 + wr + 16 * i + li;
+#pragma unroll
+      for (int j = 0; j < 4; ++j)
+#pragma unroll
+        for (int r = 0; r < 4; ++r) {
+          const int col = n0 + wc + 16 * j + lk + 4 * r;
+          acc[i][j][r] = (FULL || (row < t.m && col < t.n)) ? gC[(int64_t)col * t.ldc + row] : 0.0;
+        }
+    }
   }
   const int ar = tid & 127, ak = tid >> 7;
   const int bk = tid & 15, bc = tid >> 4;
@@ -425,9 +490,9 @@
 }
 
 
-template <bool TRSM, bool EB>
+template <bool TRSM, bool EB, bool GATHER = false>
 __device__ __forceinline__ void gemm128_mfma3_interior(const GemmTask& t, int m0, int n0, Mfma3Lds& S,
-                                                       const GrowthArgs& ga) {
+                                                       const GrowthArgs& ga, const F22Tile& fg = F22Tile{}) {
   const int tid = threadIdx.x, lane = tid & 63;
   const int wv = __builtin_amdgcn_readfirstlane(tid >> 6);
   const int wr = (wv & 1) * 64, wc = (wv >> 1) * 64;
@@ -463,16 +528,43 @@
     }
   };
   v4d acc[4][4];
-#pragma unroll
-  for (int ip = 0; ip < 2; ++ip)
-#pragma unroll
-    for (int j = 0; j < 4; ++j)
-#pragma unroll
-      for (int r = 0; r < 4; ++r) {
-        const v2d c = ldu2(cbase(ip, j, r), c_lo);
-        acc[2 * ip][j][r] = c.x;
-        acc[2 * ip + 1][j][r] = c.y;
-      }
+  if (GATHER && fg.cnt >= 0) {
+#pragma unroll
+    for (int i = 0; i < 4; ++i)
+#pragma unroll
+      for (int j = 0; j < 4; ++j) acc[i][j] = v4d{0.0, 0.0, 0.0, 0.0};
+#pragma unroll 1
+    for (int d = 0; d < fg.cnt; ++d) {
+      const F22Child c = fg.ch[d];
+      if (c.hi < m0 + wr || c.lo >= m0 + wr + 64 || c.hi < n0 + wc || c.lo >= n0 + wc + 64) continue;
+      const int32_t* inv = fg.inv + c.inv;
+      const char* src = reinterpret_cast<const char*>(fg.scratch + c.foff);
+      int ri[4], cj[4][4];
+#pragma unroll
+      for (int ip = 0; ip < 2; ++ip) {
+        ri[2 * ip] = inv[m0 + wr + 32 * ip + 2 * li];
+        ri[2 * ip + 1] = inv[m0 + wr + 32 * ip + 2 * li + 1];
+      }
+#pragma unroll
+      for (int j = 0; j < 4; ++j)
+#pragma unroll
+        for (int r = 0; r < 4; ++r) cj[j][r] = inv[n0 + wc + 16 * j + lk + 4 * r];
+      __builtin_amdgcn_sched_barrier(0);
+#pragma unroll
+      for (int j = 0; j < 4; ++j) f22_child_add(acc, j, src, c.nu, ri, cj[j]);
+    }
+  } else {
+#pragma unroll
+    for (int ip = 0; ip < 2; ++ip)
+#pragma unroll
+      for (int j = 0; j < 4; ++j)
+#pragma unroll
+        for (int r = 0; r < 4; ++r) {
+          const v2d c = ldu2(cbase(ip, j, r), c_lo);
+          acc[2 * ip][j][r] = c.x;
+          acc[2 * ip + 1][j][r] = c.y;
+        }
+  }
   const int a_off = (lk * HBM_ + wr + 2 * li);
   int b_off[4];
 #pragma unroll
@@ -574,24 +666,30 @@
   }
 };
 #endif
-template <bool TRSM, bool EB = false>
+template <bool TRSM, bool EB = false, bool GATHER = false>
 __global__ __launch_bounds__(256, 2) void k_gemm128_mfma3(const GemmTask* __restrict__ tasks, int ntask,
-                                                          GrowthArgs ga) {
+                                                          GrowthArgs ga, GatherArgs gx) {
 #ifdef SMLU_CLOCK_PROBE
   const ClockMark mark;
 #endif
   __shared__ __attribute__((aligned(16))) double lds[sizeof(Mfma3Lds) / sizeof(double)];
   const int64_t b = xcd_window_remap(blockIdx.x, gridDim.x);
-  const GemmTask t = tasks[find_gemm_task(tasks, ntask, b)];
+  const int ti = find_gemm_task(tasks, ntask, b);
+  const GemmTask t = tasks[ti];
+  F22Tile fg{nullptr, nullptr, nullptr, -1};
+  if (GATHER) {
+    const F22Gather g = gx.tg[ti];
+    fg = F22Tile{gx.ch + g.beg, gx.inv, gx.scratch, g.cnt};
+  }
   int tm, tn;
   tile_rc<HBM_>(t, b - t.tile0, tm, tn);
   const int m0 = tm * HBM_, n0 = tn * HBM_;
   if (m0 + HBM_ <= t.m && n0 + HBM_ <= t.n) {
-    gemm128_mfma3_interior<TRSM, EB>(t, m0, n0, *reinterpret_cast<Mfma3Lds*>(lds), ga);
+    gemm128_mfma3_interior<TRSM, EB, GATHER>(t, m0, n0, *reinterpret_cast<Mfma3Lds*>(lds), ga, fg);
   } else {
     auto& As = *reinterpret_cast<double(*)[2][HBK_][HBM_]>(lds);
     auto& Bs = *reinterpret_cast<double(*)[2][HBK_][HLDB_]>(lds + 2 * HBK_ * HBM_);
-    gemm128_mfma_body<TRSM, false>(t, m0, n0, As, Bs, ga);
+    gemm128_mfma_body<TRSM, false, GATHER>(t, m0, n0, As, Bs, ga, fg);
   }
 #ifdef SMLU_CLOCK_PROBE
   mark.done(EB ? 0 : 1);
@@ -601,9 +699,6 @@
 #define UR_NC 32
 #define UR_RB 6
 #define UR_LD 36
-__device__ __forceinline__ double sel0(bool c, double x) {
-  return __longlong_as_double(__double_as_longlong(x) & (c ? -1LL : 0LL));
-}
 __global__ __launch_bounds__(256, 2) void k_urows(const URowTask* __restrict__ tasks, const SNode* __restrict__ sn,
                                                   double* __restrict__ store, const double* __restrict__ tinv) {
   __shared__ double Bs[64 * UR_LD];
@@ -809,11 +904,13 @@
                          int64_t maxwg, int32_t* info, double* growth, double piv_tol) {
   if (ntiles <= 0) return hipSuccess;
   const GrowthArgs ga{info, growth, piv_tol};
+  const GatherArgs gx{nullptr, nullptr, nullptr, nullptr};
   const bool trsm = info != nullptr;
-  if (tile == 135 && trsm) k_gemm128_mfma3<true, true><<<(unsigned)ntiles, 256, 0, st>>>(tasks, ntask, ga);
-  else if (tile == 135) k_gemm128_mfma3<false, true><<<(unsigned)ntiles, 256, 0, st>>>(tasks, ntask, ga);
-  else if (tile == 131 && trsm) k_gemm128_mfma3<true><<<(unsigned)ntiles, 256, 0, st>>>(tasks, ntask, ga);
-  else if (tile == 131) k_gemm128_mfma3<false><<<(unsigned)ntiles, 256, 0, st>>>(tasks, ntask, ga);
+  if (tile == 143) return hipErrorInvalidValue;
+  if (tile == 135 && trsm) k_gemm128_mfma3<true, true><<<(unsigned)ntiles, 256, 0, st>>>(tasks, ntask, ga, gx);
+  else if (tile == 135) k_gemm128_mfma3<false, true><<<(unsigned)ntiles, 256, 0, st>>>(tasks, ntask, ga, gx);
+  else if (tile == 131 && trsm) k_gemm128_mfma3<true><<<(unsigned)ntiles, 256, 0, st>>>(tasks, ntask, ga, gx);
+  else if (tile == 131) k_gemm128_mfma3<false><<<(unsigned)ntiles, 256, 0, st>>>(tasks, ntask, ga, gx);
   else if (tile == 65 && trsm) k_gemm_k64<true><<<(unsigned)ntiles, 256, 0, st>>>(tasks, ntask, ga);
   else if (tile == 65) k_gemm_k64<false><<<(unsigned)ntiles, 256, 0, st>>>(tasks, ntask, ga);
   else if (tile == 66 && trsm) k_gemm64_mfma<true><<<(unsigned)ntiles, 256, 0, st>>>(tasks, ntask, ga);
@@ -826,6 +923,15 @@
                        int64_t maxwg) {
   return launch_gemm_g(st, ntiles, tasks, ntask, tile, maxwg, nullptr, nullptr, 1.0);
 }
+hipError_t launch_gemm_gather(hipStream_t st, int64_t ntiles, const GemmTask* tasks, int ntask, const F22Gather* tg,
+                              const F22Child* ch, const int32_t* inv, const double* scratch) {
+  if (ntiles <= 0) return hipSuccess;
+  if (!tg || !scratch) return hipErrorInvalidValue;
+  const GrowthArgs ga{nullptr, nullptr, 1.0};
+  const GatherArgs gx{tg, ch, inv, scratch};
+  k_gemm128_mfma3<false, true, true><<<(unsigned)ntiles, 256, 0, st>>>(tasks, ntask, ga, gx);
+  return hipGetLastError();
+}
 hipError_t launch_urows(hipStream_t st, int cnt, const URowTask* tasks, const SNode* sn, double* store,
                         const double* tinv) {
   if (cnt <= 0) return hipSuccess;
diff --git a/sharedmemsparselu.jl_amd/csrc/plan.hpp b/sharedmemsparselu.jl_amd/csrc/plan.hpp
--- a/sharedmemsparselu.jl_amd/csrc/plan.hpp
+++ b/sharedmemsparselu.jl_amd/csrc/plan.hpp
@@ -11,6 +11,8 @@
   int64_t t128_min = 512;
   bool small_k = true;
   int64_t fullpiv_ns = -1;
+  int64_t f22_gather_nu = 512;
+  int64_t f22_gather_ch = 8;
   int sweep_spin = 1 << 22;
   bool solve_steps = false;
   bool no_graph = false;
diff --git a/sharedmemsparselu.jl_amd/csrc/schedule.cpp b/sharedmemsparselu.jl_amd/csrc/schedule.cpp
--- a/sharedmemsparselu.jl_amd/csrc/schedule.cpp
+++ b/sharedmemsparselu.jl_amd/csrc/schedule.cpp
@@ -83,6 +83,11 @@
     }
   }
   HIPCHK(h->gtasks.upload(gt.data(), gt.size(), st));
+  if (!S.g22.empty()) {
+    HIPCHK(h->f22tasks.upload(S.g22.data(), S.g22.size(), st));
+    HIPCHK(h->f22ch.upload(S.g22ch.data(), S.g22ch.size(), st));
+    HIPCHK(h->f22inv.upload(S.g22inv.data(), S.g22inv.size(), st));
+  }
   HIPCHK(h->stasks.upload(S.st_tasks.data(), S.st_tasks.size(), st));
   HIPCHK(h->urtasks.upload(S.ur_tasks.data(), S.ur_tasks.size(), st));
   HIPCHK(h->xcols.upload(S.xc.data(), S.xc.size(), st));
@@ -116,7 +121,7 @@
   }
   HIPCHK(hipStreamSynchronize(st));
   S.ilist = {}; S.xt = {}; S.ae = {}; S.xc = {}; S.ft = {}; S.gptr = {}; S.gent = {};
-  S.gt = {}; S.st_tasks = {}; S.ur_tasks = {};
+  S.gt = {}; S.st_tasks = {}; S.ur_tasks = {}; S.g22 = {}; S.g22ch = {}; S.g22inv = {};
   return SMLU_OK;
 }
 
@@ -135,6 +140,8 @@
   out[0] = out[1] + out[2] + 8.0 * nnzA + 8.0 * n * 3 + 8.0 + 8.0 * (n + 1) + 4.0 * nnzA * 2 + 8.0 * n * 3 +
            4.0 * (double)(P.s_rows.size() + P.relmap.size() + P.ch_list.size()) + 4.0 * n * 2 + 4.0 * (double)nnodes +
            8.0 * (16 + 5 * 512) + out[3];
+  out[0] += sizeof(F22Gather) * (double)S.g22.size() + sizeof(F22Child) * (double)S.g22ch.size() +
+            4.0 * S.g22inv.size();
   out[0] += sizeof(SNode) * (double)S.hsn.size() + 4.0 * S.ilist.size() + sizeof(XContrib) * (double)S.xt.size() +
             sizeof(AEnt) * (double)S.ae.size() + sizeof(FrontTile) * (double)S.ft.size() +
             4.0 * (S.gptr.size() + S.gent.size()) + 4.0 * S.ssync_n + 8.0 * S.ntick +
@@ -224,6 +231,9 @@
   h->stick.free();
   h->sxh.free();
   h->gtasks.free();
+  h->f22tasks.free();
+  h->f22ch.free();
+  h->f22inv.free();
   h->stasks.free();
   h->urtasks.free();
   h->xcols.free();
diff --git a/sharedmemsparselu.jl_amd/csrc/schedule.hpp b/sharedmemsparselu.jl_amd/csrc/schedule.hpp
--- a/sharedmemsparselu.jl_amd/csrc/schedule.hpp
+++ b/sharedmemsparselu.jl_amd/csrc/schedule.hpp
@@ -87,6 +87,7 @@
   int32_t tiles_m = 0;
   int32_t gsid = -1;
   int64_t tile0 = 0;
+  int32_t front = -1;
 };
 
 struct ScheduleInput {
@@ -120,6 +121,11 @@
   std::vector<GemmRec> gt;
   std::vector<SwapTask> st_tasks;
   std::vector<URowTask> ur_tasks;
+  std::vector<F22Gather> g22;
+  std::vector<F22Child> g22ch;
+  std::vector<int32_t> g22inv;
+  int64_t f22_gather_fronts = 0;
+  double f22_gather_entries = 0;
   double gemm_flops = 0, gemm22_flops = 0;
   double gemm_bytes = 0;
   int64_t gemm_launches = 0, gemm128_launches = 0;
diff --git a/sharedmemsparselu.jl_amd/csrc/schedule_build.cpp b/sharedmemsparselu.jl_amd/csrc/schedule_build.cpp
--- a/sharedmemsparselu.jl_amd/csrc/schedule_build.cpp
+++ b/sharedmemsparselu.jl_amd/csrc/schedule_build.cpp
@@ -33,6 +33,7 @@
 }
 
 constexpr int kMfmaTile = 131;
+constexpr int kMfmaGatherTile = 143;
 constexpr bool kDistLookahead = false;
 
 struct Builder {
@@ -57,6 +58,7 @@
   std::vector<int64_t> bidx;
   std::vector<int32_t> col_cnt, col_pos;
   std::vector<std::vector<Launch>> bwd_levels;
+  std::vector<char> f22g;
 
   Builder(const ScheduleInput& i, Schedule& s)
       : in(i), P(*i.plan), Y(*i.lay), S(s), rank(i.rank), nranks(i.nranks) {}
@@ -126,6 +128,7 @@
     if (step < 0)
       std::stable_sort(cand.begin(), cand.end(), [](const GemmRec& a, const GemmRec& b) { return a.k > b.k; });
     Launch L = launch(step < 0 ? K_GEMM22 : kind, step, S.gt.size());
+    if (step < 0 && !f22_gather(cand, tile, L)) return;
     L.aux = tile;
     int64_t tiles = 0;
     const int ts = tile >= 128 ? 128 : 64;
@@ -146,6 +149,97 @@
     ++S.gemm_launches;
     if (tile >= 128) ++S.gemm128_launches;
     if (step < 0) S.gemm22_flops += fl;
+  }
+
+  void choose_f22_gather(int l) {
+    if (nranks > 1 || in.cpair || !in.use_mfma || in.tn.f22_gather_nu <= 0) return;
+    int64_t t128 = 0;
+    for (int64_t k = LP[l]; k < LP[l + 1]; ++k) {
+      const SNode& r = S.hsn[LS[k]];
+      if (r.mode != 0 && r.nu > 0 && r.ns > 0) t128 += (int64_t)((r.nu + 127) / 128) * ((r.nu + 127) / 128);
+    }
+    if (t128 < S.t128_min) return;
+    for (int64_t k = LP[l]; k < LP[l + 1]; ++k) {
+      const int64_t s = LS[k];
+      const SNode& r = S.hsn[s];
+      if (r.mode == 0 || r.ns <= 0 || r.nu < in.tn.f22_gather_nu) continue;
+      int64_t nch = 0, numax = 0;
+      for (int64_t e = P.ch_ptr[s]; e < P.ch_ptr[s + 1]; ++e) {
+        nch += P.nu(P.ch_list[e]) > 0;
+        numax = std::max(numax, P.nu(P.ch_list[e]));
+      }
+      if (nch <= in.tn.f22_gather_ch && numax <= 23170) f22g[s] = 1;
+    }
+  }
+  bool f22_gather(const std::vector<GemmRec>& cand, int& tile, Launch& L) {
+    bool any = false;
+    for (const GemmRec& g : cand) any = any || (g.front >= 0 && f22g[g.front]);
+    if (!any) return true;
+    if (tile != 135) {
+      fail(kSchedErrState, "internal: F22 gather chosen for a launch off the 128 MFMA tile");
+      return false;
+    }
+    tile = kMfmaGatherTile;
+    L.off2 = (int64_t)S.g22.size();
+    std::vector<std::pair<int64_t, int64_t>> wr, rd;
+    for (const GemmRec& g : cand) {
+      wr.push_back({g.C.off, g.C.off + (int64_t)g.ldc * (g.n - 1) + g.m});
+      if (g.front < 0 || !f22g[g.front]) {
+        S.g22.push_back(F22Gather{0, -1});
+        continue;
+      }
+      const int64_t s = g.front, ns = P.ns(s), nu = P.nu(s);
+      F22Gather G{(int32_t)S.g22ch.size(), 0};
+      for (int64_t e = P.ch_ptr[s]; e < P.ch_ptr[s + 1]; ++e) {
+        const int64_t c = P.ch_list[e], nuc = P.nu(c);
+        if (nuc <= 0) continue;
+        const int32_t* rm = P.relmap.data() + S.hsn[c].rowptr;
+        const int64_t inv0 = (int64_t)S.g22inv.size();
+        S.g22inv.resize(inv0 + nu, -1);
+        int32_t* inv = S.g22inv.data() + inv0;
+        int64_t lo = nu, hi = -1, want = 0, have = 0;
+        for (int64_t jc = 0; jc < nuc; ++jc) {
+          const int64_t i = (int64_t)rm[jc] - ns;
+          if (i < 0) continue;
+          if (i >= nu) {
+            fail(kSchedErrState, "internal: a child's row map leaves its parent front");
+            return false;
+          }
+          inv[i] = (int32_t)jc;
+          lo = std::min(lo, i);
+          hi = std::max(hi, i);
+          ++want;
+        }
+        for (int64_t i = 0; i < nu; ++i) have += inv[i] >= 0;
+        bool ok = have == want;
+        for (int64_t jc = 0; jc < nuc && ok; ++jc)
+          if (rm[jc] >= ns) ok = inv[rm[jc] - ns] == jc;
+        if (!ok) {
+          fail(kSchedErrState, "internal: an F22 gather map does not invert its row map");
+          return false;
+        }
+        if (want == 0) {
+          S.g22inv.resize(inv0);
+          continue;
+        }
+        S.g22ch.push_back(F22Child{S.hsn[c].Foff, inv0, (int32_t)nuc, (int32_t)lo, (int32_t)hi, 0});
+        rd.push_back({S.hsn[c].Foff, S.hsn[c].Foff + nuc * nuc});
+        ++G.cnt;
+      }
+      S.g22.push_back(G);
+      ++S.f22_gather_fronts;
+      S.f22_gather_entries += (double)nu * (double)nu;
+    }
+    std::sort(wr.begin(), wr.end());
+    for (size_t i = 1; i < wr.size(); ++i) wr[i].second = std::max(wr[i].second, wr[i - 1].second);
+    for (const auto& r : rd) {
+      auto it = std::upper_bound(wr.begin(), wr.end(), std::make_pair(r.second, (int64_t)-1));
+      if (it != wr.begin() && std::prev(it)->second > r.first) {
+        fail(kSchedErrState, "internal: an F22 launch writes a child's F22 block it gathers from");
+        return false;
+      }
+    }
+    return true;
   }
 
   void nodes() {
@@ -335,7 +429,8 @@
           S.ae.push_back(AEnt{fr_ent[ea], P.A_li[fr_ent[ea]]});
           ++ea;
         }
-        S.xc.push_back(XCol{nodes[ri], (int32_t)tj, base + cnt[tj], cnt[tj + 1] - cnt[tj],
+        const int32_t tjf = (int32_t)tj | (f22g[s] && tj >= P.ns(s) ? kXColNoF22 : 0);
+        S.xc.push_back(XCol{nodes[ri], tjf, base + cnt[tj], cnt[tj + 1] - cnt[tj],
                             (int32_t)((int64_t)S.ae.size() - a0), a0});
       }
   }
@@ -442,8 +537,10 @@
     double fl = 0;
     for (auto s : big) {
       const SNode& r = S.hsn[s];
+      const size_t had = cand.size();
       update(cand, fl, kStore + r.Loff + r.ns, kStore + r.Uoff, kScratch + r.Foff, r.nu, r.nu, r.ns,
              (int64_t)r.ns + r.nu, r.ns, r.nu);
+      if (cand.size() > had) cand.back().front = (int32_t)s;
     }
     add_gemm_launch(cand, fl, -1);
   }
@@ -1197,7 +1294,9 @@
     nodes();
     group_entries();
     levels();
+    f22g.assign(P.nsup, 0);
     for (int l = 0; l < P.nlevels && err.empty(); ++l) {
+      choose_f22_gather(l);
       assembly(l, f22_exchange(l));
       small_fronts(l);
       if (err.empty()) blocked_fronts(l);
diff --git a/sharedmemsparselu.jl_amd/csrc/smlu.cpp b/sharedmemsparselu.jl_amd/csrc/smlu.cpp
--- a/sharedmemsparselu.jl_amd/csrc/smlu.cpp
+++ b/sharedmemsparselu.jl_amd/csrc/smlu.cpp
@@ -243,8 +243,9 @@
     for (const Launch& L : h->sch.fac) {
       const bool gemm = L.kind == K_GEMM || L.kind == K_GEMMU || L.kind == K_GEMMO || L.kind == K_GEMM22;
       const bool trsm = L.kind == K_TRSML;
-      const bool mfma = L.aux == 131 || L.aux == 135;
+      const bool mfma = L.aux == 131 || L.aux == 135 || L.aux == 143;
       if (v == "mfma128" && gemm && mfma) ++c;
+      else if (v == "mfma128_gather" && gemm && L.aux == 143) ++c;
       else if (v == "mfma128_trsm" && trsm && mfma) ++c;
       else if (v == "k64" && gemm && L.aux == 65) ++c;
       else if (v == "k64_trsm" && trsm && L.aux == 65) ++c;
@@ -275,6 +276,8 @@
   if (k == "gemm22_flops") return h->sch.gemm22_flops;
   if (k == "gemm_launches") return (double)h->sch.gemm_launches;
   if (k == "gemm_bytes") return h->sch.gemm_bytes;
+  if (k == "f22_gather_fronts") return (double)h->sch.f22_gather_fronts;
+  if (k == "f22_gather_entries") return h->sch.f22_gather_entries;
   if (k == "gemm128_launches") return (double)h->sch.gemm128_launches;
   if (k == "vendor_calls") return 0.0;
   if (k.rfind("ms_", 0) == 0) {
diff --git a/sharedmemsparselu.jl_amd/csrc/tune.cpp b/sharedmemsparselu.jl_amd/csrc/tune.cpp
--- a/sharedmemsparselu.jl_amd/csrc/tune.cpp
+++ b/sharedmemsparselu.jl_amd/csrc/tune.cpp
@@ -12,6 +12,8 @@
     if (const char* e = std::getenv("SMLU_T128MIN")) v.t128_min = std::atoll(e);
     if (const char* e = std::getenv("SMLU_SMALLK")) v.small_k = std::atoi(e) != 0;
     if (const char* e = std::getenv("SMLU_FULLPIV_NS")) v.fullpiv_ns = std::atoll(e);
+    if (const char* e = std::getenv("SMLU_F22_GATHER_NU")) v.f22_gather_nu = std::atoll(e);
+    if (const char* e = std::getenv("SMLU_F22_GATHER_CH")) v.f22_gather_ch = std::atoll(e);
     if (const char* e = std::getenv("SMLU_SWEEP_SPIN")) v.sweep_spin = std::atoi(e);
     if (const char* e = std::getenv("SMLU_SOLVE_STEPS")) v.solve_steps = std::atoi(e) == 1;
     v.no_graph = std::getenv("SMLU_NO_GRAPH") != nullptr;
```

After: 6.563 billion, median of 6. 3.2% higher.
